# scheckmedia/centernet-uda

Hardware: AMD Instinct MI355X
Metric: images/sec CenterNet DLA-34 512x512 UDA step (entropy minimisation) (higher is better)
Workload: dtype f32; 1 GPU; configs[2]: DLA-34 + DCNv2, 512x512, per-GPU batch 16 source + 16 target, uda=entropy_minimization, Adam(lr 5e-5), random-init weights; global_batch=16, parallelism=dp1

## Files before the change

centernet-uda_amd/_ext.py:

```python
import torch

import hip_runtime as hr


def _shapes(input, weight, offset, mask, kh, kw, dg):
    if input.dim() != 4 or weight.dim() != 4:
        raise RuntimeError("dcn_v2: input and weight must be 4-D")
    B, C, H, W = input.shape
    Co, Ck, wkh, wkw = weight.shape
    if (wkh, wkw) != (kh, kw):
        raise RuntimeError("Input shape and kernel shape wont match: (%d x %d vs %d x %d)." % (kh, kw, wkh, wkw))
    if Ck != C:
        raise RuntimeError("Input shape and kernel channels wont match: (%d vs %d)." % (C, Ck))
    return B, C, H, W, Co


def _out_hw(H, W, kh, kw, sh, sw, ph, pw, dh, dw):
    return ((H + 2 * ph - (dh * (kh - 1) + 1)) // sh + 1, (W + 2 * pw - (dw * (kw - 1) + 1)) // sw + 1)


def _forward(who, input, weight, bias, offset, mask, om, geom, Ho, Wo, want_columns, act_slope, pack_token, pack_version,
             stats_box):
    B, C, H, W, Co, kh, kw = geom[:7]
    dg = geom[13]
    out = torch.empty((B, Co, Ho, Wo), dtype=torch.float32, device=input.device)
    cols = None
    if want_columns and W >= 2:
        cols = torch.empty((B, kh * kw * C, Ho * Wo), dtype=torch.float32, device=input.device)
    L = hr.lib()
    ws = hr.workspace(L.cnuda_dcn_v2_workspace_bytes(*geom), input.device)
    if dg == 1 and W >= 2:
        hr.prof_arm('dcn_fwd', B, C, H, W, Co, kh, kw, Ho, Wo)
    stats, blk, rows = None, 0, 0
    if stats_box is not None and act_slope < 0:
        rec = hr.stats_side_output(stats_box, L.cnuda_dcn_v2_stats_block, geom, Ho * Wo, input.device)
        if rec is not None:
            stats, blk, rows = rec[:3]
    tail = (*geom, hr.ptr(ws), ws.numel(), hr.stream())
    with hr.pack_stamp(pack_token, weight, pack_version):
        if om is not None:
            rc = L.cnuda_dcn_v2_forward_om(hr.ptr(input), hr.ptr(weight), hr.ptr(bias), hr.ptr(om), hr.ptr(out), hr.ptr(cols),
                                           hr.ptr(stats), blk, rows, float(act_slope), *tail)
        elif stats is not None:
            who += '_stats'
            rc = L.cnuda_dcn_v2_forward_stats(hr.ptr(input), hr.ptr(weight), hr.ptr(bias), hr.ptr(offset), hr.ptr(mask),
                                              hr.ptr(out), hr.ptr(cols), hr.ptr(stats), blk, rows, *tail)
        else:
            rc = L.cnuda_dcn_v2_forward_act(hr.ptr(input), hr.ptr(weight), hr.ptr(bias), hr.ptr(offset), hr.ptr(mask),
                                            hr.ptr(out), hr.ptr(cols), float(act_slope), *tail)
        hr.check(rc, who)
    return out, cols


def _backward(who, input, weight, bias, offset, mask, om, grad_output, geom, columns, grad_weight, grad_bias, grad_input):
    B, C, H, W, Co, kh, kw = geom[:7]
    g_in = grad_input if grad_input is not None else torch.empty_like(input)
    g_om = [torch.empty_like(om)] if om is not None else [torch.empty_like(offset), torch.empty_like(mask)]
    g_wb = [grad_weight if grad_weight is not None else torch.empty_like(weight),
            grad_bias if grad_bias is not None else torch.empty_like(bias)]
    L = hr.lib()
    ws = hr.workspace(L.cnuda_dcn_v2_workspace_bytes(*geom), input.device)
    if geom[13] == 1:
        hr.prof_arm('dcn_bwd', B, C, H, W, Co, kh, kw, grad_output.shape[2], grad_output.shape[3])
    fn = L.cnuda_dcn_v2_backward_acc if om is None else L.cnuda_dcn_v2_backward_om
    hr.check(fn(hr.ptr(input), hr.ptr(weight), hr.ptr(bias), *[hr.ptr(t) for t in ((offset, mask) if om is None else (om,))],
                hr.ptr(grad_output), hr.ptr(columns), hr.ptr(g_in), 1 if grad_input is not None else 0,
                *[hr.ptr(g) for g in g_om + g_wb], *geom, hr.ptr(ws), ws.numel(), hr.stream()), who)
    return [g_in] + g_om + g_wb


def dcn_v2_forward(input, weight, bias, offset, mask, kernel_h, kernel_w, stride_h, stride_w,
                   pad_h, pad_w, dilation_h, dilation_w, deformable_group, _want_columns=False, _act_slope=-1.0,
                   _pack_token=0, _pack_version=None, _stats_box=None):
    hr.require_gpu(input, weight, bias, offset, mask)
    input, weight, bias, offset, mask = [hr.f32c(t) for t in (input, weight, bias, offset, mask)]
    B, C, H, W, Co = _shapes(input, weight, offset, mask, kernel_h, kernel_w, deformable_group)
    Ho, Wo = _out_hw(H, W, kernel_h, kernel_w, stride_h, stride_w, pad_h, pad_w, dilation_h, dilation_w)
    T = kernel_h * kernel_w
    if tuple(offset.shape) != (B, 2 * T * deformable_group, Ho, Wo) or \
            tuple(mask.shape) != (B, T * deformable_group, Ho, Wo):
        raise RuntimeError("dcn_v2_forward: offset %s / mask %s do not match output %dx%d"
                           % (tuple(offset.shape), tuple(mask.shape), Ho, Wo))
    geom = (B, C, H, W, Co, kernel_h, kernel_w, stride_h, stride_w, pad_h, pad_w,
            dilation_h, dilation_w, deformable_group)
    out, cols = _forward('dcn_v2_forward', input, weight, bias, offset, mask, None, geom, Ho, Wo, _want_columns, _act_slope,
                         _pack_token, _pack_version, _stats_box)
    return (out, cols) if _want_columns else out


def dcn_v2_backward(input, weight, bias, offset, mask, grad_output, kernel_h, kernel_w, stride_h, stride_w,
                    pad_h, pad_w, dilation_h, dilation_w, deformable_group, _columns=None, _grad_weight=None,
                    _grad_bias=None, _grad_input=None):
    hr.require_gpu(input, weight, bias, offset, mask, grad_output)
    input, weight, bias, offset, mask, grad_output = [
        hr.f32c(t) for t in (input, weight, bias, offset, mask, grad_output)]
    B, C, H, W, Co = _shapes(input, weight, offset, mask, kernel_h, kernel_w, deformable_group)
    geom = (B, C, H, W, Co, kernel_h, kernel_w, stride_h, stride_w, pad_h, pad_w,
            dilation_h, dilation_w, deformable_group)
    return _backward('dcn_v2_backward', input, weight, bias, offset, mask, None, grad_output, geom, _columns, _grad_weight,
                     _grad_bias, _grad_input)


def dcn_v2_forward_om(input, weight, bias, om, kernel_h, kernel_w, stride_h, stride_w, pad_h, pad_w, dilation_h, dilation_w,
                      _want_columns=False, _pack_token=0, _stats_box=None, _act_slope=-1.0, _pack_version=None):
    hr.require_gpu(input, weight, bias, om)
    input, weight, bias, om = [hr.f32c(t) for t in (input, weight, bias, om)]
    B, C, H, W = input.shape
    Co = weight.shape[0]
    if weight.shape[1] != C or tuple(weight.shape[2:]) != (kernel_h, kernel_w):
        raise RuntimeError("dcn_v2_forward_om: weight %s does not match %d input channels / a %dx%d kernel"
                           % (tuple(weight.shape), C, kernel_h, kernel_w))
    Ho, Wo = _out_hw(H, W, kernel_h, kernel_w, stride_h, stride_w, pad_h, pad_w, dilation_h, dilation_w)
    T = kernel_h * kernel_w
    if tuple(om.shape) != (B, 3 * T, Ho, Wo):
        raise RuntimeError("dcn_v2_forward_om: om %s does not match [%d, %d, %d, %d]" % (tuple(om.shape), B, 3 * T, Ho, Wo))
    geom = (B, C, H, W, Co, kernel_h, kernel_w, stride_h, stride_w, pad_h, pad_w, dilation_h, dilation_w, 1)
    return _forward('dcn_v2_forward_om', input, weight, bias, None, None, om, geom, Ho, Wo, _want_columns, _act_slope,
                    _pack_token, _pack_version, _stats_box)


def dcn_v2_backward_om(input, weight, bias, om, grad_output, kernel_h, kernel_w, stride_h, stride_w, pad_h, pad_w,
                       dilation_h, dilation_w, _columns=None, _grad_weight=None, _grad_bias=None, _grad_input=None):
    hr.require_gpu(input, weight, bias, om, grad_output)
    input, weight, bias, om, grad_output = [hr.f32c(t) for t in (input, weight, bias, om, grad_output)]
    B, C, H, W = input.shape
    geom = (B, C, H, W, weight.shape[0], kernel_h, kernel_w, stride_h, stride_w, pad_h, pad_w, dilation_h, dilation_w, 1)
    return _backward('dcn_v2_backward_om', input, weight, bias, None, None, om, grad_output, geom, _columns, _grad_weight,
                     _grad_bias, _grad_input)


def _psroi_geom(input, rois, offset, no_trans, spatial_scale, output_dim, group_size, pooled_size, part_size,
                sample_per_part, trans_std):
    if input.dim() != 4:
        raise RuntimeError("dcn_v2_psroi_pooling: input must be 4-D")
    if rois.dim() != 2 or rois.shape[1] != 5:
        raise RuntimeError("dcn_v2_psroi_pooling: rois must be [N, 5] (batch index, x1, y1, x2, y2), got %s"
                           % (tuple(rois.shape),))
    B, C, H, W = input.shape
    N = rois.shape[0]
    if C != output_dim * group_size * group_size:
        raise RuntimeError("dcn_v2_psroi_pooling: input has %d channels, output_dim * group_size^2 = %d"
                           % (C, output_dim * group_size * group_size))
    if no_trans:
        num_classes = 1
    else:
        if offset.dim() != 4 or offset.shape[0] != N or offset.shape[1] % 2 or offset.shape[1] == 0 or \
                tuple(offset.shape[2:]) != (part_size, part_size):
            raise RuntimeError("dcn_v2_psroi_pooling: offset %s does not match [%d, 2 * num_classes, %d, %d]"
                               % (tuple(offset.shape), N, part_size, part_size))
        num_classes = offset.shape[1] // 2
        if output_dim % num_classes:
            raise RuntimeError("dcn_v2_psroi_pooling: output_dim %d is not a multiple of the offset's %d classes"
                               % (output_dim, num_classes))
    return (B, C, H, W, N, 1 if no_trans else 0, float(spatial_scale), int(output_dim), int(group_size),
            int(pooled_size), int(part_size), int(sample_per_part), float(trans_std), num_classes)


def dcn_v2_psroi_pooling_forward(input, rois, offset, no_trans, spatial_scale, output_dim, group_size, pooled_size,
                                 part_size, sample_per_part, trans_std):
    hr.require_gpu(input, rois, offset)
    input, rois = hr.f32c(input), hr.f32c(rois)
    geom = _psroi_geom(input, rois, offset, no_trans, spatial_scale, output_dim, group_size, pooled_size, part_size,
                       sample_per_part, trans_std)
    offset = None if no_trans else hr.f32c(offset)
    shape = (rois.shape[0], output_dim, pooled_size, pooled_size)
    out = torch.empty(shape, dtype=torch.float32, device=input.device)
    count = torch.empty(shape, dtype=torch.float32, device=input.device)
    hr.check(hr.lib().cnuda_dcn_v2_psroi_pooling_forward(hr.ptr(input), hr.ptr(rois), hr.ptr(offset), hr.ptr(out),
                                                         hr.ptr(count), *geom, hr.stream()),
             'dcn_v2_psroi_pooling_forward')
    return out, count


def dcn_v2_psroi_pooling_backward(grad_output, input, rois, offset, output_count, no_trans, spatial_scale, output_dim,
                                  group_size, pooled_size, part_size, sample_per_part, trans_std, _grad_input=None):
    hr.require_gpu(grad_output, input, rois, offset, output_count)
    grad_output, input, rois, output_count = [hr.f32c(t) for t in (grad_output, input, rois, output_count)]
    geom = _psroi_geom(input, rois, offset, no_trans, spatial_scale, output_dim, group_size, pooled_size, part_size,
                       sample_per_part, trans_std)
    shape = (rois.shape[0], output_dim, pooled_size, pooled_size)
    if tuple(grad_output.shape) != shape or tuple(output_count.shape) != shape:
        raise RuntimeError("dcn_v2_psroi_pooling_backward: grad_output %s / output_count %s do not match %s"
                           % (tuple(grad_output.shape), tuple(output_count.shape), shape))
    offset = None if no_trans else hr.f32c(offset)
    if _grad_input is not None and (_grad_input.shape != input.shape or _grad_input.dtype != torch.float32 or
                                    not _grad_input.is_contiguous() or not _grad_input.is_cuda):
        raise RuntimeError("dcn_v2_psroi_pooling_backward: _grad_input must be a contiguous fp32 GPU tensor like input")
    grad_input = _grad_input if _grad_input is not None else torch.empty_like(input)
    grad_offset = torch.empty(0, dtype=torch.float32, device=input.device) if no_trans else torch.empty_like(offset)
    L = hr.lib()
    ws = hr.workspace(L.cnuda_dcn_v2_psroi_pooling_workspace_bytes(geom[0], geom[4], geom[7], geom[9]), input.device)
    hr.check(L.cnuda_dcn_v2_psroi_pooling_backward(hr.ptr(grad_output), hr.ptr(input), hr.ptr(rois), hr.ptr(offset),
                                                   hr.ptr(output_count), hr.ptr(grad_input),
                                                   1 if _grad_input is not None else 0,
                                                   None if no_trans else hr.ptr(grad_offset), *geom, hr.ptr(ws),
                                                   ws.numel(), hr.stream()),
             'dcn_v2_psroi_pooling_backward')
    return grad_input, grad_offset
```

centernet-uda_amd/csrc/dcn.hip:

```cpp
#include <algorithm>
#include "igemm.cuh"
#include "igemm_host.h"

namespace cnuda {
namespace {

struct DcnGeom {
    int B, C, H, W, Co, kh, kw, sh, sw, ph, pw, dh, dw, dg, Ho, Wo;
    int off_bs, mask_bs, goff_bs, gmask_bs, gmask_logit;
};

struct Tap {
    int o00, o01, o10, o11;
    int h0, w0;
    float lh, lw, hh, hw;
    float mask;
    bool inside, c00, c01, c10, c11;
};

struct TapRaw { float dy, dx, mask; };
__device__ __forceinline__ TapRaw load_tap_raw(const DcnGeom& g, const float* __restrict__ off_b,
                                               const float* __restrict__ mask_b, int grp, int tap, int p) {
    const int T = g.kh * g.kw, HoWo = g.Ho * g.Wo;
    TapRaw r;
    r.dy = off_b[((size_t)grp * 2 * T + 2 * tap) * HoWo + p];
    r.dx = off_b[((size_t)grp * 2 * T + 2 * tap + 1) * HoWo + p];
    r.mask = mask_b[((size_t)grp * T + tap) * HoWo + p];
    return r;
}
__device__ __forceinline__ Tap tap_from_raw(const DcnGeom& g, const TapRaw& raw, int tap, int oy, int ox);
__device__ __forceinline__ Tap make_tap(const DcnGeom& g, const float* __restrict__ off_b,
                                        const float* __restrict__ mask_b, int grp, int tap, int oy, int ox) {
    return tap_from_raw(g, load_tap_raw(g, off_b, mask_b, grp, tap, oy * g.Wo + ox), tap, oy, ox);
}
__device__ __forceinline__ Tap tap_from_raw(const DcnGeom& g, const TapRaw& raw, int tap, int oy, int ox) {
    const int i = tap / g.kw, j = tap - i * g.kw;
    const float dy = raw.dy, dx = raw.dx;
    Tap t;
    t.mask = raw.mask;
    const float h = (float)(oy * g.sh - g.ph + i * g.dh) + dy;
    const float w = (float)(ox * g.sw - g.pw + j * g.dw) + dx;
    t.inside = (h > -1.0f) && (w > -1.0f) && (h < (float)g.H) && (w < (float)g.W);
    const float hf = floorf(h), wf = floorf(w);
    const int h0 = (int)hf, w0 = (int)wf;
    t.h0 = h0;
    t.w0 = w0;
    t.lh = h - hf;
    t.lw = w - wf;
    t.hh = 1.0f - t.lh;
    t.hw = 1.0f - t.lw;
    const bool top = h0 >= 0, bot = h0 + 1 <= g.H - 1, lef = w0 >= 0, rig = w0 + 1 <= g.W - 1;
    t.c00 = t.inside && top && lef;
    t.c01 = t.inside && top && rig;
    t.c10 = t.inside && bot && lef;
    t.c11 = t.inside && bot && rig;
    const int base = h0 * g.W + w0;
    t.o00 = t.c00 ? base : 0;
    t.o01 = t.c01 ? base + 1 : 0;
    t.o10 = t.c10 ? base + g.W : 0;
    t.o11 = t.c11 ? base + g.W + 1 : 0;
    return t;
}

__device__ __forceinline__ void tap_corners(const Tap& t, const float* __restrict__ plane, float& v00, float& v01,
                                            float& v10, float& v11) {
    v00 = t.c00 ? plane[t.o00] : 0.0f;
    v01 = t.c01 ? plane[t.o01] : 0.0f;
    v10 = t.c10 ? plane[t.o10] : 0.0f;
    v11 = t.c11 ? plane[t.o11] : 0.0f;
}
__device__ __forceinline__ float tap_sample(const Tap& t, float v00, float v01, float v10, float v11) {
    return t.hh * t.hw * v00 + t.hh * t.lw * v01 + t.lh * t.hw * v10 + t.lh * t.lw * v11;
}
struct __attribute__((packed, aligned(4))) Pair { float l, r; };

struct DcnFwdParams {
    DcnGeom g;
    const float *in, *off, *mask, *bias;
    float act_slope;
    float* out;
    float* col;
    float* stats;
    int stats_mp;
};

template <bool BUF>
struct DcnFwdLoaderT {
    using Params = DcnFwdParams;
    static const char* name() { return "DcnFwdLoader"; }
    static constexpr bool kHasSideOutput = true;
    const DcnGeom& g;
    const float *in_b, *off_b, *mask_b;
    buf_rsrc rin;
    float* col_base = nullptr;
    unsigned in_boff = 0, col_voff = IG_BUF_OOB;
    bool col_on = false;
    int oy, ox, K;
    bool valid;
    int cur;
    int ck0 = 0, ctap = 0, cc0 = 0;
    int qT, qB;
    float m00, m01, m10, m11;
    float* col_n;
    int col_stride;
    __device__ __forceinline__ void disable_col() { col_n = nullptr; col_on = false; }
    __device__ DcnFwdLoaderT(const Params& p, long long n, bool n_valid) : g(p.g), valid(n_valid), cur(-1) {
        const int HoWo = g.Ho * g.Wo;
        const int nn = n_valid ? (int)n : 0;
        const int b = nn / HoWo, pp = nn - b * HoWo;
        oy = pp / g.Wo;
        ox = pp - oy * g.Wo;
        const int T = g.kh * g.kw;
        in_b = p.in + (size_t)b * g.C * g.H * g.W;
        off_b = p.off + (size_t)b * g.off_bs;
        mask_b = p.mask + (size_t)b * g.mask_bs;
        K = T * g.C;
        col_n = (p.col && n_valid) ? p.col + (size_t)b * K * HoWo + pp : nullptr;
        col_stride = HoWo;
        if constexpr (BUF) {
            rin = ig_make_rsrc(p.in, (unsigned)((size_t)g.B * g.C * g.H * g.W * sizeof(float)));
            col_base = p.col;
            in_boff = (unsigned)(b * g.C * g.H * g.W) * (unsigned)sizeof(float);
            col_on = p.col != nullptr;
            col_voff = (p.col && n_valid) ? (unsigned)(b * K * HoWo + pp) * (unsigned)sizeof(float) : IG_BUF_OOB;
        }
    }
    __device__ __forceinline__ void set_tap(int tap) {
        const Tap t = make_tap(g, off_b, mask_b, 0, tap, oy, ox);
        const float mk = (valid && t.inside) ? t.mask : 0.0f;
        const float w00 = t.c00 ? t.hh * t.hw * mk : 0.0f, w01 = t.c01 ? t.hh * t.lw * mk : 0.0f;
        const float w10 = t.c10 ? t.lh * t.hw * mk : 0.0f, w11 = t.c11 ? t.lh * t.lw * mk : 0.0f;
        const bool inside = valid && t.inside;
        const int w0 = inside ? t.w0 : 0, h0 = inside ? t.h0 : 0;
        const int wa = w0 < 0 ? 0 : (w0 > g.W - 2 ? g.W - 2 : w0);
        const bool ledge = w0 < 0, redge = w0 > g.W - 2;
        m00 = ledge ? w01 : (redge ? 0.0f : w00);
        m01 = ledge ? 0.0f : (redge ? w00 : w01);
        m10 = ledge ? w11 : (redge ? 0.0f : w10);
        m11 = ledge ? 0.0f : (redge ? w10 : w11);
        const int ht = h0 < 0 ? 0 : h0, hb = h0 + 1 > g.H - 1 ? g.H - 1 : h0 + 1;
        qT = ht * g.W + wa;
        qB = hb * g.W + wa;
        cur = tap;
    }
    __device__ __forceinline__ float sample(const float* __restrict__ pl) const {
        const Pair a = *reinterpret_cast<const Pair*>(pl + qT), b = *reinterpret_cast<const Pair*>(pl + qB);
        return m00 * a.l + m01 * a.r + m10 * b.l + m11 * b.r;
    }
    struct Raw {
        Pair t[8], b[8];
        int k0;
        bool live, eager;
    };
    __device__ __forceinline__ void load_raw(int k0, int ksub, Raw& r) {
        const int HW = g.H * g.W;
        r.k0 = k0 + ksub;
        r.live = k0 < K;
        r.eager = g.C % IG_BK != 0;
        if (!r.eager) {
            if (!r.live) return;
            while (ck0 < k0) {
                ck0 += IG_BK;
                cc0 += IG_BK;
                if (cc0 >= g.C) { cc0 -= g.C; ++ctap; }
            }
            const int tap = ctap, c0 = cc0 + ksub;
            if (tap != cur) set_tap(tap);
            if constexpr (BUF) {
                const unsigned vT = in_boff + (unsigned)qT * 4u, vB = in_boff + (unsigned)qB * 4u;
                const int c0s = cc0 + __builtin_amdgcn_readfirstlane(ksub);
#pragma unroll
                for (int j = 0; j < 8; ++j) {
                    const unsigned soff = (unsigned)((c0s + 2 * j) * HW) * 4u;
                    r.t[j] = __builtin_bit_cast(Pair, __builtin_amdgcn_raw_buffer_load_b64(rin, (int)vT, (int)soff, 0));
                    r.b[j] = __builtin_bit_cast(Pair, __builtin_amdgcn_raw_buffer_load_b64(rin, (int)vB, (int)soff, 0));
                }
                return;
            }
            const float* plane = in_b + (size_t)c0 * HW;
#pragma unroll
            for (int j = 0; j < 8; ++j) {
                const float* pl = plane + (size_t)(2 * j) * HW;
                r.t[j] = *reinterpret_cast<const Pair*>(pl + qT);
                r.b[j] = *reinterpret_cast<const Pair*>(pl + qB);
            }
            return;
        }
#pragma unroll
        for (int j = 0; j < 8; ++j) {
            const int k = k0 + ksub + 2 * j;
            float v = 0.0f;
            if (k < K) {
                const int tap = k / g.C, c = k - tap * g.C;
                if (tap != cur) set_tap(tap);
                v = sample(in_b + (size_t)c * HW);
            }
            r.t[j].l = v;
        }
    }
    __device__ __forceinline__ void finish(const Raw& r, float (&v)[8]) {
        if (!r.eager) {
            if (!r.live) {
#pragma unroll
                for (int j = 0; j < 8; ++j) v[j] = 0.0f;
                return;
            }
#pragma unroll
            for (int j = 0; j < 8; ++j) v[j] = m00 * r.t[j].l + m01 * r.t[j].r + m10 * r.b[j].l + m11 * r.b[j].r;
            if constexpr (BUF) {
                if (col_on && col_voff != IG_BUF_OOB) {
                    const int k0s = __builtin_amdgcn_readfirstlane(r.k0);
                    const char* cbase = reinterpret_cast<const char*>(col_base);
                    unsigned voff = col_voff;
                    asm volatile("" : "+v"(voff));
#pragma unroll
                    for (int j = 0; j < 8; ++j) {
                        const size_t row = (size_t)(unsigned)((k0s + 2 * j) * col_stride) * 4u;
                        unsigned long long rbase = reinterpret_cast<unsigned long long>(cbase) + row;
                        asm volatile("" : "+s"(rbase));
                        *reinterpret_cast<__attribute__((address_space(1))) float*>(rbase + (unsigned long long)voff) = v[j];
                    }
                }
                return;
            }
            if (col_n) {
                float* cp = col_n + (size_t)r.k0 * col_stride;
                const size_t step = (size_t)2 * col_stride;
#pragma unroll
                for (int j = 0; j < 8; ++j) cp[j * step] = v[j];
            }
            return;
        }
#pragma unroll
        for (int j = 0; j < 8; ++j) {
            const int k = r.k0 + 2 * j;
            v[j] = r.t[j].l;
            if (col_n && k < K) col_n[(size_t)k * col_stride] = v[j];
        }
    }
    struct Out {
        float* base;
        int HoWo;
        __device__ Out(const Params& p, long long n) {
            HoWo = p.g.Ho * p.g.Wo;
            const int ni = (int)n, b = ni / HoWo, pp = ni - b * HoWo;
            base = p.out + (size_t)b * p.g.Co * HoWo + pp;
        }
        __device__ __forceinline__ void store(const Params& p, int m, float v) {
            v += p.bias[m];
            if (p.act_slope >= 0.0f && v < 0.0f) v *= p.act_slope;
            base[(size_t)m * HoWo] = v;
        }
        static constexpr bool kVec4 = true;
        __device__ static bool vec4_ok(const Params& p) { return ((p.g.Ho * p.g.Wo) & 3) == 0; }
        __device__ __forceinline__ void store4(const Params& p, int m, f32x4 v) {
            v += p.bias[m];
            if (p.act_slope >= 0.0f) {
#pragma unroll
                for (int e = 0; e < 4; ++e) if (v[e] < 0.0f) v[e] *= p.act_slope;
            }
            *reinterpret_cast<f32x4*>(base + (size_t)m * HoWo) = v;
        }
    };
};

using DcnFwdLoader = DcnFwdLoaderT<false>;
using DcnFwdBufLoader = DcnFwdLoaderT<true>;

constexpr int DW_MARGIN = 3;
typedef __attribute__((address_space(3))) volatile unsigned char lds_vu8;
template <int TC> struct DwTile {
    static constexpr int TR = IG_BN / TC, NR = TR + 2 + 2 * DW_MARGIN, RS = TC + 8, PL = NR * RS;
    static constexpr int CPR = TC / 4 + 2, CPP = NR * CPR, CELLS = 16 * CPP;
    static constexpr int NCELL = (CELLS + IG_THREADS - 1) / IG_THREADS;
    static constexpr int SHIFT = TC == 32 ? 5 : 4;
};
template <int TC> constexpr size_t dcnw_lds_floats(int bm) { return (size_t)16 * DwTile<TC>::PL + 2 * IG_KC * bm; }

template <int BM, int TC>
__global__ __launch_bounds__(IG_THREADS, 3) void dcnw_fwd_kernel(DcnFwdParams p, const float* __restrict__ A, int Mp, int Kp,
                                                                 int n_tiles, int tiles_x) {
    using Q = DwTile<TC>;
    constexpr int TM = BM / 32, PL = Q::PL, RS = Q::RS;
    extern __shared__ __attribute__((aligned(16))) float smem[];
    const DcnGeom& g = p.g;
    const int W = g.W, H = g.H, HW = g.H * g.W;
    float* const Hs = smem;
    float* const Asb = smem + 16 * PL;
    const int tid = threadIdx.x, lane = tid & 63, wid = tid >> 6;
    int tile = xcd_remap(blockIdx.x, n_tiles);
    const int tile_id = tile;
    const int tx = tile % tiles_x; tile /= tiles_x;
    const int tiles_y = H / Q::TR;
    const int ty = tile % tiles_y, b = tile / tiles_y;
    const int y0 = ty * Q::TR, x0 = tx * TC;
    const int yw0 = y0 - 1 - DW_MARGIN;
    const int pxl = wid * 32 + (lane & 31), kl = lane >> 5;
    const int py = y0 + (pxl >> Q::SHIFT), px = x0 + (pxl & (TC - 1)), pp = py * W + px;

    const buf_rsrc rs = ig_make_rsrc(p.in, (unsigned)((size_t)g.B * g.C * HW * sizeof(float)));
    auto cell = [&](int i, unsigned& voff, int& loff) {
        int salt = 0;
        asm volatile("" : "+v"(salt));
        const int e = tid + i * IG_THREADS + salt;
        const int c = e / Q::CPP, rem = e - c * Q::CPP;
        const int row = rem / Q::CPR, q4 = rem - row * Q::CPR;
        const int iy = yw0 + row, ix = x0 - 4 + 4 * q4;
        loff = e < Q::CELLS ? c * PL + row * RS + 4 * q4 : -1;
        voff = (e < Q::CELLS && iy >= 0 && iy < H && ix >= 0 && ix < W)
                   ? (unsigned)(((b * g.C + c) * HW + iy * W + ix) * (int)sizeof(float)) : IG_BUF_OOB;
    };

    int addr[9];
    float flh[9], flw[9], fmk[9];
    unsigned stray = 0;
    {
        const float* off_b = p.off + (size_t)b * g.off_bs + pp;
        const float* mask_b = p.mask + (size_t)b * g.mask_bs + pp;
        float dy[9], dx[9], mk[9];
#pragma unroll
        for (int t = 0; t < 9; ++t) {
            dy[t] = off_b[(size_t)(2 * t) * HW];
            dx[t] = off_b[(size_t)(2 * t + 1) * HW];
            mk[t] = mask_b[(size_t)t * HW];
        }
#pragma unroll
        for (int t = 0; t < 9; ++t) {
            const float h = (float)(py - 1 + t / 3) + dy[t], w = (float)(px - 1 + t % 3) + dx[t];
            const float hf = floorf(h), wf = floorf(w);
            const bool valid = h > -1.0f && w > -1.0f && h < (float)H && w < (float)W;
            const int h0 = valid ? (int)hf : 0, w0i = valid ? (int)wf : 0;
            const int wr = h0 - yw0, wc = w0i - x0 + 4;
            const bool inwin = valid && wr >= 0 && wr + 1 <= Q::NR - 1 && wc >= 0 && wc + 1 <= RS - 1;
            addr[t] = inwin ? wr * RS + wc : 0;
            flh[t] = h - hf;
            flw[t] = w - wf;
            fmk[t] = inwin ? mk[t] : 0.0f;
            if (valid && !inwin) stray |= 1u << t;
        }
    }
    const bool any_stray = __any(stray != 0);

    f32x16 acc[TM];
#pragma unroll
    for (int i = 0; i < TM; ++i)
#pragma unroll
        for (int r = 0; r < 16; ++r) acc[i][r] = 0.0f;

    f32x4 hreg[Q::NCELL];
    auto win_load = [&](int grp) {
        const unsigned soff = (unsigned)(grp * 16 * HW) * (unsigned)sizeof(float);
#pragma unroll
        for (int i = 0; i < Q::NCELL; ++i) {
            unsigned voff; int loff;
            cell(i, voff, loff);
            hreg[i] = ig_buf_load4(rs, voff, soff);
        }
    };
    auto win_store = [&]() {
#pragma unroll
        for (int i = 0; i < Q::NCELL; ++i) {
            unsigned voff; int loff;
            cell(i, voff, loff);
            if (loff >= 0) *reinterpret_cast<f32x4*>(Hs + loff) = hreg[i];
        }
    };
    f32x4 ra[ig_a_per<BM>()];
    const IgABuf<BM> abuf(A, Mp, Kp, 0, tid);
    const int nchunk = Kp / IG_KC, G = g.C >> 4;
    const bool col_on = p.col != nullptr;
    float* const col_l = col_on ? p.col + (size_t)b * 9 * g.C * HW + (size_t)kl * HW + pp : nullptr;

    win_load(0);
    abuf.load(0, ra);
    win_store();
    ig_store_a<BM>(Asb, tid, ra);
    if (1 < nchunk) abuf.load(IG_KC, ra);
    __syncthreads();
    int grp = 0;
    for (int c0 = 0; c0 < nchunk; c0 += 9, ++grp) {
        const bool more = grp + 1 < G;
        if (more) win_load(grp + 1);
#pragma unroll
        for (int t = 0; t < 9; ++t) {
            const int c = c0 + t;
            f32x4 ra2[ig_a_per<BM>()];
            if (c + 2 < nchunk) abuf.load((c + 2) * IG_KC, ra2);
            const float* As = Asb + (c & 1) * IG_KC * BM;
            const float* ap = As + kl * BM + (lane & 31);
            int a_t = addr[t];
            asm volatile("" : "+v"(a_t));
            const float* hb = Hs + kl * PL + a_t;
            const float lh = flh[t], lw = flw[t], hh = 1.0f - lh, hw = 1.0f - lw, mk = fmk[t];
            const float w00 = hh * hw * mk, w01 = hh * lw * mk, w10 = lh * hw * mk, w11 = lh * lw * mk;
            float v[IG_KC / 2], cr[IG_KC / 4][4];
            float* cp = nullptr;
            if (col_on) {
                unsigned long long rowoff = (unsigned long long)(unsigned)((t * g.C + grp * 16) * HW) * sizeof(float);
                asm volatile("" : "+s"(rowoff));
                cp = reinterpret_cast<float*>(reinterpret_cast<char*>(col_l) + rowoff);
            }
            auto read_half = [&](int h) {
#pragma unroll
                for (int s = 0; s < IG_KC / 4; ++s) {
                    const float* q = hb + 2 * (h * (IG_KC / 4) + s) * PL;
                    cr[s][0] = q[0]; cr[s][1] = q[1]; cr[s][2] = q[RS]; cr[s][3] = q[RS + 1];
                }
            };
            auto blend_half = [&](int h) {
#pragma unroll
                for (int s = 0; s < IG_KC / 4; ++s) {
                    float x = w00 * cr[s][0];
                    x = fmaf(w01, cr[s][1], x);
                    x = fmaf(w10, cr[s][2], x);
                    v[h * (IG_KC / 4) + s] = fmaf(w11, cr[s][3], x);
                }
                if (col_on) {
#pragma unroll
                    for (int s = 0; s < IG_KC / 4; ++s) cp[(size_t)(2 * (h * (IG_KC / 4) + s)) * HW] = v[h * (IG_KC / 4) + s];
                }
            };
            auto mma_half = [&](int h) {
#pragma unroll
                for (int s = h * (IG_KC / 4); s < (h + 1) * (IG_KC / 4); ++s) {
#pragma unroll
                    for (int i = 0; i < TM; ++i)
                        acc[i] = __builtin_amdgcn_mfma_f32_32x32x2f32(ap[2 * s * BM + i * 32], v[s], acc[i], 0, 0, 0);
                }
            };
            read_half(0);
            blend_half(0);
            read_half(1);
            __builtin_amdgcn_sched_barrier(0);
            mma_half(0);
            __builtin_amdgcn_sched_barrier(0);
            blend_half(1);
            mma_half(1);
            if (c + 1 < nchunk) ig_store_a<BM>(Asb + ((c + 1) & 1) * IG_KC * BM, tid, ra);
#pragma unroll
            for (int i = 0; i < ig_a_per<BM>(); ++i) ra[i] = ra2[i];
            __syncthreads();
            __builtin_amdgcn_sched_barrier(0);
        }
        if (any_stray) {
#pragma unroll 1
            for (int t0 = 0; t0 < 9; ++t0) {
                int t = t0;
                asm volatile("" : "+s"(t));
                if (!__any((stray >> t) & 1u)) continue;
                float sv[IG_KC / 2];
#pragma unroll
                for (int s = 0; s < IG_KC / 2; ++s) sv[s] = 0.0f;
                if ((stray >> t) & 1u) {
                    const float* off_b = p.off + (size_t)b * g.off_bs + pp;
                    const int tr = t / 3;
                    const float sh_ = (float)(py - 1 + tr) + off_b[(size_t)(2 * t) * HW];
                    const float sw_ = (float)(px - 1 + t - 3 * tr) + off_b[(size_t)(2 * t + 1) * HW];
                    const float smk = p.mask[(size_t)b * g.mask_bs + (size_t)t * HW + pp];
                    const float shf = floorf(sh_), swf = floorf(sw_);
                    const int sh0 = (int)shf, sw0 = (int)swf;
                    const float slh = sh_ - shf, slw = sw_ - swf, shh = 1.0f - slh, shw = 1.0f - slw;
                    const bool top = sh0 >= 0, bot = sh0 + 1 <= H - 1, lef = sw0 >= 0, rig = sw0 + 1 <= W - 1;
                    const float g00 = (top && lef) ? shh * shw * smk : 0.0f, g01 = (top && rig) ? shh * slw * smk : 0.0f;
                    const float g10 = (bot && lef) ? slh * shw * smk : 0.0f, g11 = (bot && rig) ? slh * slw * smk : 0.0f;
                    const int cy0 = top ? sh0 : 0, cy1 = bot ? sh0 + 1 : H - 1, cx0 = lef ? sw0 : 0, cx1 = rig ? sw0 + 1 : W - 1;
                    const float* in_c = p.in + ((size_t)b * g.C + grp * 16 + kl) * HW;
                    const int o00 = cy0 * W + cx0, o01 = cy0 * W + cx1, o10 = cy1 * W + cx0, o11 = cy1 * W + cx1;
#pragma unroll
                    for (int s = 0; s < IG_KC / 2; ++s) {
                        const float* pl = in_c + (size_t)(2 * s) * HW;
                        float x = g00 * pl[o00];
                        x = fmaf(g01, pl[o01], x);
                        x = fmaf(g10, pl[o10], x);
                        sv[s] = fmaf(g11, pl[o11], x);
                    }
                    if (col_on) {
                        float* cp = col_l + (size_t)(t * g.C + grp * 16) * HW;
#pragma unroll
                        for (int s = 0; s < IG_KC / 2; ++s) cp[(size_t)(2 * s) * HW] = sv[s];
                    }
                }
                const float* ag = A + (size_t)((c0 + t) * IG_KC + kl) * Mp + (lane & 31);
#pragma unroll
                for (int s = 0; s < IG_KC / 2; ++s) {
#pragma unroll
                    for (int i = 0; i < TM; ++i)
                        acc[i] = __builtin_amdgcn_mfma_f32_32x32x2f32(ag[(size_t)(2 * s) * Mp + i * 32], sv[s], acc[i], 0, 0, 0);
                }
            }
        }
        if (more) {
            win_store();
            __syncthreads();
        }
    }
    float* stage = smem + wid * IG_EPI_WAVE;
    const int col = lane & 31, cg = lane & 7, rsub = lane >> 3;
    const int epl = wid * 32 + 4 * cg;
    float* const obase = p.out + (size_t)b * g.Co * HW + (size_t)(y0 + (epl >> Q::SHIFT)) * W + x0 + (epl & (TC - 1));
#pragma unroll
    for (int i = 0; i < TM; ++i) {
#pragma unroll
        for (int r = 0; r < 16; ++r) stage[mfma_row(r, lane) * IG_EPI_LD + col] = acc[i][r];
        asm volatile("s_waitcnt lgkmcnt(0)" ::: "memory");
#pragma unroll
        for (int it = 0; it < 4; ++it) {
            const int row = it * 8 + rsub;
            f32x4 v4 = *reinterpret_cast<const f32x4*>(stage + row * IG_EPI_LD + 4 * cg);
            const int m = i * 32 + row;
            if (m < g.Co) {
                v4 += p.bias[m];
                if (p.act_slope >= 0.0f) {
#pragma unroll
                    for (int e = 0; e < 4; ++e) if (v4[e] < 0.0f) v4[e] *= p.act_slope;
                }
                *reinterpret_cast<f32x4*>(obase + (size_t)m * HW) = v4;
            }
            if (p.stats) {
                float s1 = (v4[0] + v4[1]) + (v4[2] + v4[3]);
                float s2 = (v4[0] * v4[0] + v4[1] * v4[1]) + (v4[2] * v4[2] + v4[3] * v4[3]);
                auto row8 = [](float v) {
                    v += __builtin_bit_cast(float, __builtin_amdgcn_update_dpp(0, __builtin_bit_cast(int, v), 0xB1, 0xf, 0xf, false));
                    v += __builtin_bit_cast(float, __builtin_amdgcn_update_dpp(0, __builtin_bit_cast(int, v), 0x4E, 0xf, 0xf, false));
                    v += __builtin_bit_cast(float, __builtin_amdgcn_update_dpp(0, __builtin_bit_cast(int, v), 0x141, 0xf, 0xf, false));
                    return v;
                };
                s1 = row8(s1);
                s2 = row8(s2);
                if (cg == 0)
                    reinterpret_cast<float2*>(p.stats)[((size_t)tile_id * 4 + wid) * p.stats_mp + m] = make_float2(s1, s2);
            }
        }
        asm volatile("s_waitcnt lgkmcnt(0)" ::: "memory");
    }
}

struct DcnSampleParams {
    DcnGeom g;
    const float *in, *off, *mask;
    float* col;
};
__global__ __launch_bounds__(1024) void dcn_sample_kernel(DcnSampleParams p, int tiles_per_image) {
    const DcnGeom& g = p.g;
    const int T = g.kh * g.kw, HoWo = g.Ho * g.Wo, HW = g.H * g.W;
    const int b = blockIdx.x / tiles_per_image, tile = blockIdx.x - b * tiles_per_image;
    const int px = tile * 64 + threadIdx.x;
    if (px >= HoWo) return;
    const int oy = px / g.Wo, ox = px - oy * g.Wo;
    const float* in_b = p.in + (size_t)b * g.C * HW;
    for (int tap = threadIdx.y; tap < T; tap += blockDim.y) {
        const Tap t = make_tap(g, p.off + (size_t)b * g.off_bs, p.mask + (size_t)b * g.mask_bs, 0, tap, oy, ox);
        const float mk = t.inside ? t.mask : 0.0f;
        const float w00 = t.c00 ? t.hh * t.hw * mk : 0.0f, w01 = t.c01 ? t.hh * t.lw * mk : 0.0f;
        const float w10 = t.c10 ? t.lh * t.hw * mk : 0.0f, w11 = t.c11 ? t.lh * t.lw * mk : 0.0f;
        float* dst = p.col + ((size_t)b * T + tap) * g.C * HoWo + px;
        const bool paired = g.W >= 2;
        const bool ledge = t.w0 < 0, redge = t.w0 > g.W - 2;
        const int wa = ledge ? 0 : (redge ? g.W - 2 : t.w0);
        const int ht = t.h0 < 0 ? 0 : t.h0, hb = t.h0 + 1 > g.H - 1 ? g.H - 1 : t.h0 + 1;
        const int qT = t.inside ? ht * g.W + wa : 0, qB = t.inside ? hb * g.W + wa : 0;
        for (int c0 = 0; c0 < g.C; c0 += 8) {
            float e00[8], e01[8], e10[8], e11[8];
            if (paired) {
                Pair pt[8], pb[8];
#pragma unroll
                for (int u = 0; u < 8; ++u) {
                    const float* plane = in_b + (size_t)(c0 + u < g.C ? c0 + u : g.C - 1) * HW;
                    pt[u] = *reinterpret_cast<const Pair*>(plane + qT);
                    pb[u] = *reinterpret_cast<const Pair*>(plane + qB);
                }
#pragma unroll
                for (int u = 0; u < 8; ++u) {
                    e00[u] = redge ? pt[u].r : pt[u].l; e01[u] = ledge ? pt[u].l : pt[u].r;
                    e10[u] = redge ? pb[u].r : pb[u].l; e11[u] = ledge ? pb[u].l : pb[u].r;
                }
            } else {
#pragma unroll
                for (int u = 0; u < 8; ++u) {
                    const float* plane = in_b + (size_t)(c0 + u < g.C ? c0 + u : g.C - 1) * HW;
                    e00[u] = plane[t.o00]; e01[u] = plane[t.o01]; e10[u] = plane[t.o10]; e11[u] = plane[t.o11];
                }
            }
#pragma unroll
            for (int u = 0; u < 8; ++u)
                if (c0 + u < g.C)
                    dst[(size_t)(c0 + u) * HoWo] = w00 * e00[u] + w01 * e01[u] + w10 * e10[u] + w11 * e11[u];
        }
    }
}

struct DcnColsParams {
    DcnGeom g;
    const float *col, *bias;
    float act_slope;
    float* out;
    float* stats;
    int stats_mp;
};
struct DcnColsLoader {
    using Params = DcnColsParams;
    static const char* name() { return "DcnColsLoader"; }
    static constexpr bool kHasSideOutput = false;
    const float* base;
    int K, HoWo;
    bool valid;
    __device__ DcnColsLoader(const Params& p, long long n, bool n_valid) : valid(n_valid) {
        HoWo = p.g.Ho * p.g.Wo;
        K = p.g.kh * p.g.kw * p.g.C;
        const int nn = n_valid ? (int)n : 0;
        const int b = nn / HoWo, pp = nn - b * HoWo;
        base = p.col + (size_t)b * K * HoWo + pp;
    }
    __device__ __forceinline__ void load(int k0, int ksub, float (&v)[8]) {
#pragma unroll
        for (int j = 0; j < 8; ++j) {
            const int k = k0 + ksub + 2 * j;
            v[j] = (valid && k < K) ? base[(size_t)k * HoWo] : 0.0f;
        }
    }
    struct Out {
        float* base;
        int HoWo;
        __device__ Out(const Params& p, long long n) {
            HoWo = p.g.Ho * p.g.Wo;
            const int ni = (int)n, b = ni / HoWo, pp = ni - b * HoWo;
            base = p.out + (size_t)b * p.g.Co * HoWo + pp;
        }
        __device__ __forceinline__ void store(const Params& p, int m, float v) {
            v += p.bias[m];
            if (p.act_slope >= 0.0f && v < 0.0f) v *= p.act_slope;
            base[(size_t)m * HoWo] = v;
        }
// ... 349 lines not shown
}

struct DcnPrepParams {
    DcnGeom g;
    const float *w, *off, *mask;
    float* wt;
    DcnGeo* geo;
    int wt_blocks;
    float* zero;
    long long zero_quads;
    int zero_first;
};
__global__ __launch_bounds__(256) void dcn_prep_kernel(DcnPrepParams p) {
    const DcnGeom& g = p.g;
    if (p.zero && (int)blockIdx.x >= p.zero_first) {
        const long long nb = (long long)gridDim.x - p.zero_first;
        float4* z = reinterpret_cast<float4*>(p.zero);
        for (long long i = ((long long)blockIdx.x - p.zero_first) * 256 + threadIdx.x; i < p.zero_quads; i += nb * 256)
            z[i] = make_float4(0.f, 0.f, 0.f, 0.f);
        return;
    }
    const int T = g.kh * g.kw;
    if ((int)blockIdx.x < p.wt_blocks) {
        const long long total = (long long)g.Co * g.C * T;
        for (long long i = (long long)blockIdx.x * 256 + threadIdx.x; i < total; i += (long long)p.wt_blocks * 256) {
            const int o = (int)(i % g.Co);
            const long long r = i / g.Co;
            const int c = (int)(r % g.C), tap = (int)(r / g.C);
            p.wt[i] = p.w[((size_t)o * g.C + c) * T + tap];
        }
        return;
    }
    if (!p.geo) return;
    const int HoWo = g.Ho * g.Wo;
    const long long total = (long long)g.B * T * HoWo;
    const long long nb = (long long)(p.zero ? p.zero_first : (int)gridDim.x) - p.wt_blocks;
    for (long long i = ((long long)blockIdx.x - p.wt_blocks) * 256 + threadIdx.x; i < total; i += nb * 256) {
        const int px = (int)(i % HoWo);
        const long long r = i / HoWo;
        const int tap = (int)(r % T), b = (int)(r / T);
        const int oy = px / g.Wo, ox = px - oy * g.Wo;
        p.geo[i] = dcn_geo_pack(make_tap(g, p.off + (size_t)b * g.off_bs, p.mask + (size_t)b * g.mask_bs, 0, tap, oy, ox));
    }
}

struct DcnBwdDataParams {
    DcnGeom g;
    const float *in, *dcol;
    const DcnGeo* geo;
    float *gin, *goff, *gmask;
    DcnWalkTile tile;
    int nsplit;
};
template <bool QUADS>
__global__ __launch_bounds__(512, 6) void dcn_bwd_data_kernel(DcnBwdDataParams p, int n_wg) {
    extern __shared__ __align__(16) float win[];
    const DcnGeom& g = p.g;
    const int T = g.kh * g.kw, HoWo = g.Ho * g.Wo, HW = g.H * g.W;
    const int tid = threadIdx.x & 255, lane = tid & 63, wid = __builtin_amdgcn_readfirstlane(tid >> 6);
    int id = xcd_remap(blockIdx.x, n_wg);
    const int part = id % p.nsplit; id /= p.nsplit;
    const DcnWalkTile& tile = p.tile;
    const int tx = id % tile.tiles_x; id /= tile.tiles_x;
    const int ty = id % tile.tiles_y;
    const int b = id / tile.tiles_y;
    const int y0 = ty * tile.TR, x0 = tx * tile.TC;
    const DcnGeo* geo_b = p.geo + (size_t)b * T * HoWo;
    const float* dcol_b = p.dcol + (size_t)b * T * g.C * HoWo;
    auto pixel_of = [&](int grp, bool& valid) {
        const int i = grp * 64 + lane;
        const int oy = y0 + (i >> tile.tc_shift), ox = x0 + (i & (tile.TC - 1));
        valid = oy < g.Ho && ox < g.Wo;
        return valid ? oy * g.Wo + ox : 0;
    };
#ifdef DCN_ABLATE
    if ((DCN_ABLATE == 1) == (threadIdx.x >= 256)) return;
#endif
    if (threadIdx.x >= 256) {
        bool valid;
        const int px = pixel_of(wid, valid);
        if (!valid) return;
        const float* in_b = p.in + (size_t)b * g.C * HW;
#pragma unroll 1
        for (int tap = part; tap < T; tap += p.nsplit) {
            const DcnGeoTap t = dcn_geo_unpack(geo_b[(size_t)tap * HoWo + px]);
            const float* dc = dcol_b + (size_t)tap * g.C * HoWo + (QUADS ? (size_t)px * 4 : (size_t)px);
            DcnCoordSums s{0.f, 0.f, 0.f};
            if (t.inside) s = dcn_coord_tap<QUADS>(g, t, in_b, dc, HoWo);
            dcn_coord_store(g, p.gmask, p.goff, b, tap, px, HoWo, t.mask, s);
        }
        return;
    }
    const DcnScatterCtx x = dcn_scatter_ctx(win, tile, g, y0, x0, wid, tid);
    float* gin_b = p.gin + (size_t)b * g.C * HW;
    const int cg_end = (part + 1) * tile.ncg / p.nsplit;
#pragma unroll 1
    for (int cg = part * tile.ncg / p.nsplit; cg < cg_end; ++cg)
        dcn_scatter_group<QUADS>(x, g, geo_b, dcol_b, gin_b, cg * CI_CG + wid * 4, lane);
}

struct DcnWParams {
    DcnGeom g;
    const float *in, *off, *mask, *gout;
};
struct DcnWLoader {
    using Params = DcnWParams;
    const Params& p;
    IgPixelCursor c;
    __device__ DcnWLoader(const Params& pp, long long n, long long n_end) : p(pp) {
        c.init(n, n_end, p.g.Ho * p.g.Wo, p.g.Wo);
    }
    __device__ __forceinline__ void advance() { c.advance(p.g.Ho * p.g.Wo, p.g.Wo); }
    template <int NV, int STEP>
    __device__ __forceinline__ void load_g(int m0, int msub, float (&v)[NV]) {
        const DcnGeom& g = p.g;
        const int HoWo = g.Ho * g.Wo;
        const float* base = p.gout + (size_t)c.b_ * g.Co * HoWo + c.pp_;
#pragma unroll
        for (int i = 0; i < NV; ++i) {
            const int m = m0 + msub + STEP * i;
            v[i] = (c.valid_ && m < g.Co) ? base[(size_t)m * HoWo] : 0.0f;
        }
    }
    template <int NV, int STEP>
    __device__ __forceinline__ void load_b(int j0, int jsub, float (&v)[NV]) {
        const DcnGeom& g = p.g;
        const int HW = g.H * g.W, T = g.kh * g.kw, K = T * g.C;
        const float* in_b = p.in + (size_t)c.b_ * g.C * HW;
        const float* off_b = p.off + (size_t)c.b_ * g.off_bs;
        const float* mask_b = p.mask + (size_t)c.b_ * g.mask_bs;
        int cur = -1;
        Tap t;
#pragma unroll
        for (int i = 0; i < NV; ++i) {
            const int k = j0 + jsub + STEP * i;
            float r = 0.0f;
            if (c.valid_ && k < K) {
                const int tap = k / g.C, ch = k - tap * g.C;
                if (tap != cur) { t = make_tap(g, off_b, mask_b, 0, tap, c.oy_, c.ox_); cur = tap; }
                if (t.inside) {
                    float v00, v01, v10, v11;
                    tap_corners(t, in_b + (size_t)ch * HW, v00, v01, v10, v11);
                    r = tap_sample(t, v00, v01, v10, v11) * t.mask;
                }
            }
            v[i] = r;
        }
    }
};

struct DcnColWParams {
    DcnGeom g;
    const float *col, *gout;
};
struct DcnColWLoader {
    using Params = DcnColWParams;
    const Params& p;
    IgPixelCursor c;
    __device__ DcnColWLoader(const Params& pp, long long n, long long n_end) : p(pp) {
        c.init(n, n_end, p.g.Ho * p.g.Wo, p.g.Wo);
    }
    __device__ __forceinline__ void advance() { c.advance(p.g.Ho * p.g.Wo, p.g.Wo); }
    template <int NV, int STEP>
    __device__ __forceinline__ void load_g(int m0, int msub, float (&v)[NV]) {
        const DcnGeom& g = p.g;
        const int HoWo = g.Ho * g.Wo;
        const float* base = p.gout + (size_t)c.b_ * g.Co * HoWo + c.pp_;
#pragma unroll
        for (int i = 0; i < NV; ++i) {
            const int m = m0 + msub + STEP * i;
            v[i] = (c.valid_ && m < g.Co) ? base[(size_t)m * HoWo] : 0.0f;
        }
    }
    template <int NV, int STEP>
    __device__ __forceinline__ void load_b(int j0, int jsub, float (&v)[NV]) {
        const DcnGeom& g = p.g;
        const int HoWo = g.Ho * g.Wo, K = g.kh * g.kw * g.C;
        const float* base = p.col + (size_t)c.b_ * K * HoWo + c.pp_;
#pragma unroll
        for (int i = 0; i < NV; ++i) {
            const int k = j0 + jsub + STEP * i;
            v[i] = (c.valid_ && k < K) ? base[(size_t)k * HoWo] : 0.0f;
        }
    }
};

struct DcnColWBufLoader {
    using Params = DcnColWParams;
    const Params& p;
    buf_rsrc rg, rc;
    IgPixelCursor c;
    unsigned gimg, cimg;
    __device__ DcnColWBufLoader(const Params& pp, long long n, long long n_end) : p(pp) {
        const DcnGeom& g = p.g;
        const size_t px = (size_t)g.B * g.Ho * g.Wo;
        rg = ig_make_rsrc(p.gout, (unsigned)(px * g.Co * sizeof(float)));
        rc = ig_make_rsrc(p.col, (unsigned)(px * g.kh * g.kw * g.C * sizeof(float)));
        c.init(n, n_end, g.Ho * g.Wo, g.Wo);
        gimg = (unsigned)(c.b_ * g.Co * g.Ho * g.Wo) * 4u;
        cimg = (unsigned)(c.b_ * g.kh * g.kw * g.C * g.Ho * g.Wo) * 4u;
    }
    __device__ __forceinline__ void advance() {
        const DcnGeom& g = p.g;
        c.advance(g.Ho * g.Wo, g.Wo);
        if (c.crossed_) {
            gimg += (unsigned)(c.crossed_ * g.Co * g.Ho * g.Wo) * 4u;
            cimg += (unsigned)(c.crossed_ * g.kh * g.kw * g.C * g.Ho * g.Wo) * 4u;
        }
    }
    template <int NV, int STEP>
    __device__ __forceinline__ void load_g(int m0, int msub, float (&v)[NV]) {
        ig_buf_rows<NV, STEP>(rg, c, gimg, p.g.Ho * p.g.Wo, m0, msub, v);
    }
    template <int NV, int STEP>
    __device__ __forceinline__ void load_b(int j0, int jsub, float (&v)[NV]) {
        ig_buf_rows<NV, STEP>(rc, c, cimg, p.g.Ho * p.g.Wo, j0, jsub, v);
    }
};

struct DcnNaiveParams {
    DcnGeom g;
    const float *in, *weight, *bias, *off, *mask, *gout;
    float *out, *gin, *goff, *gmask, *gw;
};

__global__ void dcn_naive_fwd_kernel(DcnNaiveParams p) {
    const DcnGeom& g = p.g;
    const int T = g.kh * g.kw, HoWo = g.Ho * g.Wo, HW = g.H * g.W, cpg = g.C / g.dg;
    const long long total = (long long)g.B * g.Co * HoWo;
    for (long long i = (long long)blockIdx.x * blockDim.x + threadIdx.x; i < total;
         i += (long long)gridDim.x * blockDim.x) {
        const int pp = (int)(i % HoWo), o = (int)((i / HoWo) % g.Co), b = (int)(i / ((long long)HoWo * g.Co));
        const int oy = pp / g.Wo, ox = pp - oy * g.Wo;
        float s = p.bias[o];
        for (int grp = 0; grp < g.dg; ++grp)
            for (int tap = 0; tap < T; ++tap) {
                const Tap t = make_tap(g, p.off + (size_t)b * g.off_bs,
                                       p.mask + (size_t)b * g.mask_bs, grp, tap, oy, ox);
                if (!t.inside) continue;
                for (int cc = 0; cc < cpg; ++cc) {
                    const int c = grp * cpg + cc;
                    float v00, v01, v10, v11;
                    tap_corners(t, p.in + ((size_t)b * g.C + c) * HW, v00, v01, v10, v11);
                    s += p.weight[((size_t)o * g.C + c) * T + tap] * (tap_sample(t, v00, v01, v10, v11) * t.mask);
                }
            }
        p.out[i] = s;
    }
}

__global__ void dcn_naive_bwd_kernel(DcnNaiveParams p) {
    const DcnGeom& g = p.g;
    const int T = g.kh * g.kw, HoWo = g.Ho * g.Wo, HW = g.H * g.W, cpg = g.C / g.dg;
    const long long total = (long long)g.B * g.C * T * HoWo;
    for (long long i = (long long)blockIdx.x * blockDim.x + threadIdx.x; i < total;
         i += (long long)gridDim.x * blockDim.x) {
        const int pp = (int)(i % HoWo), tap = (int)((i / HoWo) % T), c = (int)((i / ((long long)HoWo * T)) % g.C);
        const int b = (int)(i / ((long long)HoWo * T * g.C));
        const int oy = pp / g.Wo, ox = pp - oy * g.Wo, grp = c / cpg;
        const Tap t = make_tap(g, p.off + (size_t)b * g.off_bs, p.mask + (size_t)b * g.mask_bs, grp,
                               tap, oy, ox);
        if (!t.inside) continue;
        float v00, v01, v10, v11;
        tap_corners(t, p.in + ((size_t)b * g.C + c) * HW, v00, v01, v10, v11);
        const float smp = tap_sample(t, v00, v01, v10, v11);
        const float* go = p.gout + (size_t)b * g.Co * HoWo + pp;
        float d = 0.0f;
        for (int o = 0; o < g.Co; ++o) {
            const float gv = go[(size_t)o * HoWo];
            d += p.weight[((size_t)o * g.C + c) * T + tap] * gv;
            atomicAdd(p.gw + ((size_t)o * g.C + c) * T + tap, gv * (smp * t.mask));
        }
        const float dm = d * t.mask;
        atomicAdd(p.gmask + ((size_t)(b * g.dg + grp) * T + tap) * HoWo + pp, d * smp);
        atomicAdd(p.goff + ((size_t)(b * g.dg + grp) * 2 * T + 2 * tap) * HoWo + pp,
                  (-t.hw * v00 - t.lw * v01 + t.hw * v10 + t.lw * v11) * dm);
        atomicAdd(p.goff + ((size_t)(b * g.dg + grp) * 2 * T + 2 * tap + 1) * HoWo + pp,
                  (-t.hh * v00 + t.hh * v01 - t.lh * v10 + t.lh * v11) * dm);
        float* gplane = p.gin + ((size_t)b * g.C + c) * HW;
        if (t.c00) atomicAdd(gplane + t.o00, t.hh * t.hw * dm);
        if (t.c01) atomicAdd(gplane + t.o01, t.hh * t.lw * dm);
        if (t.c10) atomicAdd(gplane + t.o10, t.lh * t.hw * dm);
        if (t.c11) atomicAdd(gplane + t.o11, t.lh * t.lw * dm);
    }
}

int fill_geom(DcnGeom& g, int B, int C, int H, int W, int Co, int kh, int kw, int sh, int sw, int ph, int pw, int dh,
              int dw, int dg, const char* who) {
    CNUDA_REQUIRE(B > 0 && C > 0 && H > 0 && W > 0 && Co > 0, "%s: empty tensor", who);
    CNUDA_REQUIRE(kh > 0 && kw > 0 && sh > 0 && sw > 0 && dh > 0 && dw > 0 && ph >= 0 && pw >= 0,
                  "%s: bad kernel geometry", who);
    CNUDA_REQUIRE(dg > 0 && C % dg == 0, "%s: channels (%d) not divisible by deformable_group (%d)", who, C, dg);
    g = DcnGeom{B, C, H, W, Co, kh, kw, sh, sw, ph, pw, dh, dw, dg,
                (H + 2 * ph - (dh * (kh - 1) + 1)) / sh + 1, (W + 2 * pw - (dw * (kw - 1) + 1)) / sw + 1, 0, 0, 0, 0, 0};
    CNUDA_REQUIRE(g.Ho > 0 && g.Wo > 0, "%s: kernel larger than padded input", who);
    CNUDA_REQUIRE((long long)dg * 3 * kh * kw * g.Ho * g.Wo < (1ll << 31), "%s: offset planes of an image exceed 2^31 elements", who);
    g.off_bs = g.goff_bs = dg * 2 * kh * kw * g.Ho * g.Wo;
    g.mask_bs = g.gmask_bs = dg * kh * kw * g.Ho * g.Wo;
    return 0;
}

constexpr int kDcnMinTiles = 512;
int dcn_pick_bm(int M, long long N) {
    int bm = M > 64 ? 128 : (M > 32 ? 64 : 32);
    const long long n_tiles = (N + IG_BN - 1) / IG_BN;
    while (bm > 32 && n_tiles * ((M + bm - 1) / bm) < kDcnMinTiles) bm >>= 1;
    return bm;
}

constexpr int kFusedMinTilesDefault = 512;
int g_fused_min_tiles = kFusedMinTilesDefault;
int g_scatter_margin = 0;
int g_walk_tc = 0;
int g_offset_regime = 0;


int dcnw_tile_cols(int W) { return W % 32 == 0 ? 32 : 16; }
bool dcnw_takes(const DcnGeom& g) {
    static const bool dcnw_on = !(getenv("CNUDA_DCNW") && getenv("CNUDA_DCNW")[0] == '0');
    return dcnw_on && (g_offset_regime & 2) == 0 && matrix_mode() == 0 && g.kh == 3 && g.kw == 3 && g.sh == 1 && g.sw == 1 && g.ph == 1 && g.pw == 1 &&
           g.dh == 1 && g.dw == 1 && g.dg == 1 && g.C % 16 == 0 && g.Co <= 64 &&
           g.W % 16 == 0 && g.H % (IG_BN / dcnw_tile_cols(g.W)) == 0 &&
           (size_t)g.B * g.C * g.H * g.W * sizeof(float) < IG_BUF_OOB;
}

#ifndef DCN_COLS_WS
#define DCN_COLS_WS 1
#endif
#ifndef DCN_COLW_WS
#define DCN_COLW_WS 1
#endif
enum class DcnFwdPath { Naive, Composed, Window, SampleThenGemm, Gather };
struct DcnPlan {
    DcnFwdPath fwd;
    bool fwd_buf;
    bool fwd_ws;
    bool colw_buf, colw_ws;
    bool dcol_quads;
    int T, K, Kp, bm, Mp;
    WgradShape wg;
    long long N;
    size_t fwd_bytes, bwd_bytes;
    bool fwd_two_kernels;
    size_t gemm_bytes;
    DcnWalkTile tile;
    size_t col2im_lds;
    bool fused_consumers;
    int fused_split;
};
DcnPlan make_plan(const DcnGeom& g) {
    DcnPlan q;
    q.T = g.kh * g.kw;
    q.K = q.T * g.C;
    q.Kp = round_up(q.K, IG_KC);
    q.N = (long long)g.B * g.Ho * g.Wo;
    q.bm = dcn_pick_bm(g.Co, q.N);
    q.Mp = round_up(g.Co, q.bm);
    q.wg = make_wgrad_shape(g.Co, q.K, q.N, WG_BM, round_up(q.K, WG_BJ) % 128 == 0 ? 128 : WG_BJ, WG_BP);
    q.fwd_two_kernels = q.Mp / q.bm > 1;
    q.fwd_bytes = carve_bytes((size_t)q.Kp * q.Mp, 4) + 256 +
                  (q.fwd_two_kernels ? carve_bytes((size_t)g.B * q.K * g.Ho * g.Wo, 4) : 0);
    if (g.Co <= 64) {
        const size_t wb = carve_bytes((size_t)q.Kp * 64, 4) + 256;
        if (wb > q.fwd_bytes) q.fwd_bytes = wb;
    }
    q.gemm_bytes = cnuda_conv2d_workspace_bytes(g.B, g.Co, g.Ho, g.Wo, q.T * g.C, 1, 1, 1, 1, 0, 0);
    q.bwd_bytes = carve_bytes((size_t)q.wg.Z * q.wg.Mpw * q.wg.Jp, 4) +
                  carve_bytes(std::max((size_t)g.Co * g.B, (size_t)q.wg.Z * q.wg.Mpw), 4) +
                  carve_bytes((size_t)12 * g.C * (g.Co < 64 ? 64 : g.Co), 4) +
                  carve_bytes((size_t)g.B * q.T * g.C * g.Ho * g.Wo, 4) +
                  carve_bytes((size_t)g.B * q.T * g.Ho * g.Wo, sizeof(DcnGeo)) + carve_bytes(q.gemm_bytes, 1) + 256;
    DcnWalkTile& w = q.tile;
    w.TC = 64;
    while (w.TC > 16 && w.TC / 2 >= g.Wo) w.TC >>= 1;
    if (w.TC == 64 && round_up(g.Wo, 32) < round_up(g.Wo, 64)) w.TC = 32;
    if (g_walk_tc == 16 || g_walk_tc == 32 || g_walk_tc == 64) w.TC = g_walk_tc;
    w.TR = 256 / w.TC;
    w.tc_shift = w.TC == 64 ? 6 : (w.TC == 32 ? 5 : 4);
    w.tiles_y = ceil_div(g.Ho, w.TR);
    w.tiles_x = ceil_div(g.Wo, w.TC);
    w.ncg = ceil_div(g.C, CI_CG);
    w.margin = g_scatter_margin > 0 ? g_scatter_margin : ((g_offset_regime & 1) ? 4 : CI_MARGIN);
    const int wr = (w.TR - 1) * g.sh + (g.kh - 1) * g.dh + 2 * w.margin + 1;
    const int wc = (w.TC - 1) * g.sw + (g.kw - 1) * g.dw + 2 * w.margin + 1;
    w.WSZmax = wr * wc;
    w.claim_sz = ((wr + 1) * (wc + 1) + 15) / 16 * 16;
    if ((size_t)CI_CG * w.WSZmax * 4 + 4096 + 4 * (size_t)w.claim_sz > (w.margin > CI_MARGIN ? 80 : 53) * 1024) { w.WSZmax = 0; w.claim_sz = 16; }
    q.col2im_lds = ((size_t)CI_CG * w.WSZmax + 4 * 256) * sizeof(float) + 4 * (size_t)w.claim_sz;
    q.fused_consumers = w.WSZmax > 0 && g.W >= 2 && (long long)g.B * w.tiles_y * w.tiles_x >= g_fused_min_tiles;
    q.fused_split = 4;
    if (q.fused_split > w.ncg) q.fused_split = w.ncg;

    const size_t HoWo = (size_t)g.Ho * g.Wo;
    q.fwd = (g.dg > 1 && g.W >= 2) ? DcnFwdPath::Composed
          : (g.dg != 1 || g.W < 2) ? DcnFwdPath::Naive
          : dcnw_takes(g) ? DcnFwdPath::Window
          : q.fwd_two_kernels ? DcnFwdPath::SampleThenGemm : DcnFwdPath::Gather;
    q.fwd_buf = buffer_addressing() && g.C % IG_BK == 0 && (size_t)g.B * g.C * g.H * g.W * sizeof(float) < IG_BUF_OOB &&
                (size_t)g.B * q.K * HoWo * sizeof(float) < IG_BUF_OOB;
    q.fwd_ws = DCN_COLS_WS && q.fwd_buf && q.bm >= 64 && wave_specialised() && matrix_mode() == 0;
    q.colw_buf = buffer_addressing() && (size_t)g.B * q.K * HoWo * sizeof(float) < IG_BUF_OOB &&
                 (size_t)g.B * g.Co * HoWo * sizeof(float) < IG_BUF_OOB && HoWo < (1 << 23);
    q.colw_ws = DCN_COLW_WS && q.colw_buf && wave_specialised() && matrix_mode() == 0;
    static const bool quads_on = !(getenv("CNUDA_DCOL_QUADS") && getenv("CNUDA_DCOL_QUADS")[0] == '0');
    q.dcol_quads = quads_on && g.C % 4 == 0 && HoWo < (1 << 26) &&
                   cnuda_conv2d_rowquads_supported(g.B, g.Co, g.Ho, g.Wo, q.T * g.C, 1, 1, 1, 1, 0, 0);
    return q;
}

int plan_stats_block(const DcnGeom& g, const DcnPlan& q, int* rows) {
    if (q.fwd == DcnFwdPath::Naive || q.fwd == DcnFwdPath::Composed || ((g.Ho * g.Wo) & 3) != 0) return 0;
    if (q.fwd == DcnFwdPath::Window) { if (rows) *rows = 64; return 32; }
    if (rows) *rows = q.Mp;
    return q.bm == 32 ? 32 : 64;
}

struct DcnCall {
    DcnGeom g;
    const float *input, *weight, *bias, *offset, *mask;
    void* workspace;
    size_t workspace_bytes;
    cnuda_stream_t stream;
};
struct DcnFwdCall : DcnCall {
    float *output, *columns, *stats;
    float act_slope;
};
struct DcnBwdCall : DcnCall {
    const float *grad_output, *columns;
    float *grad_input, *grad_offset, *grad_mask, *grad_weight, *grad_bias;
    int accumulate_input;
};

template <class F>
auto with_quads(bool quads, F&& f) {
    return quads ? f(std::true_type{}) : f(std::false_type{});
}

template <class Loader, bool WS = false, class P>
bool launch_dcn_fwd(const DcnPlan& q, const P& p, const float* A, int Cout, hipStream_t st) {
    const int n_tiles = ceil_div(q.N, IG_BN), m_tiles = q.Mp / q.bm;
    const dim3 grid(n_tiles * m_tiles);
    if constexpr (WS)
        return with_tile<64, 128>(q.bm, [&](auto BM) {
            CNUDA_LAUNCH((igemm_fwd_ws_kernel<BM(), Loader>), grid, dim3(2 * IG_THREADS), 0, st, p, A, q.Mp, q.Kp, Cout, q.N, n_tiles, m_tiles);
        });
    else
        return with_tile<32, 64, 128>(q.bm, [&](auto BM) {
            CNUDA_LAUNCH((igemm_fwd_kernel<BM(), Loader>), grid, dim3(IG_THREADS), 0, st, p, A, q.Mp, q.Kp, Cout, q.N, n_tiles, m_tiles);
        });
}

}
}

using namespace cnuda;

extern "C" int cnuda_dcn_set_scatter_margin(int margin) {
    const int prev = g_scatter_margin;
    g_scatter_margin = margin < 1 ? 0 : (margin > 8 ? 8 : margin);
    return prev;
}
extern "C" int cnuda_dcn_set_walk_tile(int tile_cols) {
    const int prev = g_walk_tc;
    g_walk_tc = tile_cols;
    return prev;
}
extern "C" int cnuda_dcn_set_offset_regime(int regime) {
    const int prev = g_offset_regime;
    g_offset_regime = regime & 3;
    return prev;
}

namespace cnuda {
namespace {
__global__ __launch_bounds__(256) void dcn_offset_census_kernel(const float* __restrict__ offset, long long n_pairs, long long HW,
                                                                unsigned* __restrict__ counts) {
    unsigned c2 = 0, c3 = 0;
    for (long long i = (long long)blockIdx.x * 256 + threadIdx.x; i < n_pairs; i += (long long)gridDim.x * 256) {
        const long long plane = i / HW, px = i - plane * HW;
        const float dy = fabsf(offset[(2 * plane) * HW + px]), dx = fabsf(offset[(2 * plane + 1) * HW + px]);
        const float d = dy > dx ? dy : dx;
        c2 += d >= 2.0f;
        c3 += d >= 3.0f;
    }
    __shared__ unsigned s2, s3;
    if (threadIdx.x == 0) { s2 = 0; s3 = 0; }
    __syncthreads();
    if (c2) atomicAdd(&s2, c2);
    if (c3) atomicAdd(&s3, c3);
    __syncthreads();
    if (threadIdx.x == 0) {
        if (s2) atomicAdd(counts, s2);
        if (s3) atomicAdd(counts + 1, s3);
    }
}
}
}
extern "C" int cnuda_dcn_offset_census(const float* offset, int B, int taps, long long HW, unsigned* counts,
                                       cnuda_stream_t stream) {
    CNUDA_REQUIRE(offset && counts && B > 0 && taps > 0 && HW > 0, "cnuda_dcn_offset_census: bad arguments");
    const long long n = (long long)B * taps * HW;
    CNUDA_LAUNCH(cnuda::dcn_offset_census_kernel, dim3(stream_grid(n, 256)), dim3(256), 0, (hipStream_t)stream, offset, n, HW,
                 counts);
    return check_launch("cnuda_dcn_offset_census");
}
extern "C" int cnuda_dcn_set_fused_min_tiles(int min_tiles) {
    const int prev = g_fused_min_tiles;
    g_fused_min_tiles = min_tiles < 1 ? kFusedMinTilesDefault : min_tiles;
    return prev;
}

extern "C" size_t cnuda_dcn_v2_workspace_bytes(int B, int C, int H, int W, int Cout, int kh, int kw, int sh, int sw,
                                               int ph, int pw, int dh, int dw, int dg) {
    DcnGeom g;
    if (fill_geom(g, B, C, H, W, Cout, kh, kw, sh, sw, ph, pw, dh, dw, dg, "cnuda_dcn_v2_workspace_bytes")) return 0;
    const DcnPlan q = make_plan(g);
    if (q.fwd == DcnFwdPath::Composed) {
        const int Cg = C / dg, T = kh * kw;
        const size_t inner = cnuda_dcn_v2_workspace_bytes(B, Cg, H, W, Cout, kh, kw, sh, sw, ph, pw, dh, dw, 1);
        return 2 * carve_bytes((size_t)B * Cg * H * W, 4) + 2 * carve_bytes((size_t)Cout * Cg * T, 4) +
               carve_bytes((size_t)B * Cout * g.Ho * g.Wo, 4) + 2 * carve_bytes((size_t)Cout, 4) + carve_bytes(inner, 1) + 512;
    }
    return q.fwd_bytes > q.bwd_bytes ? q.fwd_bytes : q.bwd_bytes;
}

extern "C" int cnuda_dcn_v2_forward(const float* input, const float* weight, const float* bias, const float* offset,
                                    const float* mask, float* output, int B, int C, int H, int W, int Cout, int kh,
                                    int kw, int sh, int sw, int ph, int pw, int dh, int dw, int dg, void* workspace,
                                    size_t workspace_bytes, cnuda_stream_t stream) {
    return cnuda_dcn_v2_forward_cols(input, weight, bias, offset, mask, output, nullptr, B, C, H, W, Cout, kh, kw, sh,
                                     sw, ph, pw, dh, dw, dg, workspace, workspace_bytes, stream);
}

extern "C" int cnuda_dcn_v2_forward_cols(const float* input, const float* weight, const float* bias,
                                         const float* offset, const float* mask, float* output, float* columns, int B,
                                         int C, int H, int W, int Cout, int kh, int kw, int sh, int sw, int ph, int pw,
                                         int dh, int dw, int dg, void* workspace, size_t workspace_bytes,
                                         cnuda_stream_t stream) {
    return cnuda_dcn_v2_forward_act(input, weight, bias, offset, mask, output, columns, -1.0f, B, C, H, W, Cout, kh, kw,
                                    sh, sw, ph, pw, dh, dw, dg, workspace, workspace_bytes, stream);
}

extern "C" int cnuda_dcn_v2_stats_block(int B, int C, int H, int W, int Cout, int kh, int kw, int sh, int sw, int ph, int pw,
                                        int dh, int dw, int dg, int* rows) {
    DcnGeom g;
    if (fill_geom(g, B, C, H, W, Cout, kh, kw, sh, sw, ph, pw, dh, dw, dg, "cnuda_dcn_v2_stats_block")) return 0;
    return plan_stats_block(g, make_plan(g), rows);
}

static int dcn_forward_impl(const DcnFwdCall& c, const DcnPlan& q) {
    const DcnGeom& g = c.g;
    CNUDA_REQUIRE(c.input && c.weight && c.bias && c.offset && c.mask && c.output, "cnuda_dcn_v2_forward: null pointer");
    CNUDA_REQUIRE(!c.columns || g.W >= 2, "cnuda_dcn_v2_forward_cols: columns output needs width >= 2");
    hipStream_t st = (hipStream_t)c.stream;
    CNUDA_REQUIRE(c.act_slope < 0.0f || (g.dg == 1 && g.W >= 2), "cnuda_dcn_v2_forward_act: fused activation needs deformable_group == 1 and width >= 2");
    if (q.fwd == DcnFwdPath::Composed) {
        const int Cg = g.C / g.dg, T = q.T, HoWo = g.Ho * g.Wo;
        const long long HW = (long long)g.H * g.W;
        const size_t inner = cnuda_dcn_v2_workspace_bytes(g.B, Cg, g.H, g.W, g.Co, g.kh, g.kw, g.sh, g.sw, g.ph, g.pw, g.dh, g.dw, 1);
        Carver cv(c.workspace, c.workspace_bytes);
        float* xg = cv.take<float>((size_t)g.B * Cg * HW);
        float* wg = cv.take<float>((size_t)g.Co * Cg * T);
        float* tmp = cv.take<float>((size_t)g.B * g.Co * HoWo);
        float* zero = cv.take<float>((size_t)g.Co);
        void* iws = cv.take<char>(inner);
        CNUDA_REQUIRE(c.workspace && cv.cur <= cv.end, "cnuda_dcn_v2_forward: workspace too small");
        if (hipMemsetAsync(zero, 0, (size_t)g.Co * sizeof(float), st) != hipSuccess) return check_launch("cnuda_dcn_v2_forward(dg>1)");
        DcnFwdCall gc = c;
        gc.g.C = Cg; gc.g.dg = 1;
        gc.input = xg; gc.weight = wg;
        gc.workspace = iws; gc.workspace_bytes = inner;
        const DcnPlan gq = make_plan(gc.g);
        const PackStampSuspend uncached;
        for (int grp = 0; grp < g.dg; ++grp) {
            if (int rc = cnuda_copy_channels(c.input, xg, g.B, Cg, HW, g.C, grp * Cg, Cg, 0, c.stream)) return rc;
            if (int rc = cnuda_copy_channels(c.weight, wg, g.Co, Cg, T, g.C, grp * Cg, Cg, 0, c.stream)) return rc;
            gc.bias = grp == 0 ? c.bias : zero;
            gc.offset = c.offset + (size_t)grp * 2 * T * HoWo;
            gc.mask = c.mask + (size_t)grp * T * HoWo;
            gc.output = grp == 0 ? c.output : tmp;
            gc.columns = c.columns ? c.columns + (size_t)grp * g.B * T * Cg * HoWo : nullptr;
            if (int rc = dcn_forward_impl(gc, gq)) return rc;
            if (grp > 0)
                if (int rc = cnuda_add(c.output, tmp, c.output, (long long)g.B * g.Co * HoWo, c.stream)) return rc;
        }
        return check_launch("cnuda_dcn_v2_forward(dg>1)");
    }
    if (q.fwd == DcnFwdPath::Naive) {
        DcnNaiveParams p{g, c.input, c.weight, c.bias, c.offset, c.mask, nullptr, c.output, nullptr, nullptr, nullptr, nullptr};
        CNUDA_LAUNCH(dcn_naive_fwd_kernel, dim3(stream_grid((long long)g.B * g.Co * g.Ho * g.Wo, 256)), dim3(256),
                           0, st, p);
        return check_launch("cnuda_dcn_v2_forward(dg>1)");
    }
    CNUDA_REQUIRE(q.N < (1ll << 31) - IG_BN, "cnuda_dcn_v2_forward: more than 2^31 pixels per call");
    CNUDA_REQUIRE(c.workspace && c.workspace_bytes >= q.fwd_bytes, "cnuda_dcn_v2_forward: workspace too small");
    Carver cv(c.workspace, c.workspace_bytes);
    if (q.fwd == DcnFwdPath::Window) {
        const int bm = 64;
        const float* Aw = launch_pack(c.weight, cv.take<float>((size_t)q.Kp * bm), (size_t)q.Kp * bm * sizeof(float), g.Co, g.C,
                                      q.T, PACK_HALO_FWD, q.Kp, bm, 0, st);
        DcnFwdParams p{g, c.input, c.offset, c.mask, c.bias, c.act_slope, c.output, c.columns, c.stats, 64};
        ProfScope prof(st);
        prof.name("dcnw_fwd_kernel<%d>%s", bm, c.columns ? " (+ column side output)" : "");
        const int tiles_x = g.W / dcnw_tile_cols(g.W), n_tiles = (int)(q.N / IG_BN);
        bool lds_ok = true;
        const bool found = with_tiles<Tile<64, 32>, Tile<64, 16>>(bm, dcnw_tile_cols(g.W), [&](auto BM, auto TC) {
            const size_t fl = dcnw_lds_floats<TC()>(BM());
            const size_t lds = (fl < (size_t)4 * IG_EPI_WAVE ? (size_t)4 * IG_EPI_WAVE : fl) * sizeof(float);
            lds_ok = raise_dynamic_lds(reinterpret_cast<const void*>(&dcnw_fwd_kernel<BM(), TC()>), lds);
            if (lds_ok) CNUDA_LAUNCH((dcnw_fwd_kernel<BM(), TC()>), dim3(n_tiles), dim3(IG_THREADS), lds, st, p, Aw, bm, q.Kp, n_tiles, tiles_x);
        });
        CNUDA_REQUIRE(lds_ok, "cnuda_dcn_v2_forward: dynamic LDS");
        CNUDA_REQUIRE(found, "cnuda_dcn_v2_forward: no dcnw_fwd_kernel instance for %d-column tiles", dcnw_tile_cols(g.W));
        return check_launch("cnuda_dcn_v2_forward(window)");
    }
    const float* A = launch_pack(c.weight, cv.take<float>((size_t)q.Kp * q.Mp), (size_t)q.Kp * q.Mp * sizeof(float), g.Co,
                                 g.C, q.T, PACK_FWD, q.Kp, q.Mp, 0, st);
    if (q.fwd == DcnFwdPath::SampleThenGemm) {
        float* cols = c.columns ? c.columns : cv.take<float>((size_t)g.B * q.K * g.Ho * g.Wo);
        ProfScope prof(st);
        prof.name("dcn_sample_kernel + igemm_fwd_kernel<%d, DcnColsLoader>", q.bm);
        {
            DcnSampleParams sp{g, c.input, c.offset, c.mask, cols};
            const int tiles = ceil_div(g.Ho * g.Wo, 64), tw = q.T < 16 ? q.T : 16;
            CNUDA_LAUNCH(dcn_sample_kernel, dim3(g.B * tiles), dim3(64, tw), 0, st, sp, tiles);
        }
        DcnColsParams p{g, cols, c.bias, c.act_slope, c.output, c.stats, q.Mp};
        const bool found = q.fwd_ws    ? launch_dcn_fwd<DcnColsBufLoader, true>(q, p, A, g.Co, st)
                           : q.fwd_buf ? launch_dcn_fwd<DcnColsBufLoader>(q, p, A, g.Co, st)
                                       : launch_dcn_fwd<DcnColsLoader>(q, p, A, g.Co, st);
        CNUDA_REQUIRE(found, "cnuda_dcn_v2_forward: no GEMM instance for a %d-row tile", q.bm);
        return check_launch("cnuda_dcn_v2_forward(columns + GEMM)");
    }
    DcnFwdParams p{g, c.input, c.offset, c.mask, c.bias, c.act_slope, c.output, c.columns, c.stats, q.Mp};
    ProfScope prof(st);
    prof.name("igemm_fwd_kernel<%d, DcnFwdLoader>%s", q.bm, c.columns ? " (+ column side output)" : "");
    const bool found = q.fwd_buf ? launch_dcn_fwd<DcnFwdBufLoader>(q, p, A, g.Co, st) : launch_dcn_fwd<DcnFwdLoader>(q, p, A, g.Co, st);
    CNUDA_REQUIRE(found, "cnuda_dcn_v2_forward: no GEMM instance for a %d-row tile", q.bm);
    return check_launch("cnuda_dcn_v2_forward");
}

extern "C" int cnuda_dcn_v2_forward_act(const float* input, const float* weight, const float* bias,
                                        const float* offset, const float* mask, float* output, float* columns,
                                        float act_slope, int B, int C, int H, int W, int Cout, int kh, int kw, int sh,
                                        int sw, int ph, int pw, int dh, int dw, int dg, void* workspace,
                                        size_t workspace_bytes, cnuda_stream_t stream) {
    DcnFwdCall c{};
    if (int rc = fill_geom(c.g, B, C, H, W, Cout, kh, kw, sh, sw, ph, pw, dh, dw, dg, "cnuda_dcn_v2_forward")) return rc;
    c.input = input; c.weight = weight; c.bias = bias; c.offset = offset; c.mask = mask;
    c.output = output; c.columns = columns; c.act_slope = act_slope;
    c.workspace = workspace; c.workspace_bytes = workspace_bytes; c.stream = stream;
    return dcn_forward_impl(c, make_plan(c.g));
}

extern "C" int cnuda_dcn_v2_forward_stats(const float* input, const float* weight, const float* bias,
                                          const float* offset, const float* mask, float* output, float* columns,
                                          float* stats, int stats_block, int stats_rows, int B, int C, int H, int W,
                                          int Cout, int kh, int kw, int sh,
                                          int sw, int ph, int pw, int dh, int dw, int dg, void* workspace,
                                          size_t workspace_bytes, cnuda_stream_t stream) {
    DcnFwdCall c{};
    if (int rc = fill_geom(c.g, B, C, H, W, Cout, kh, kw, sh, sw, ph, pw, dh, dw, dg, "cnuda_dcn_v2_forward")) return rc;
    const DcnPlan q = make_plan(c.g);
    if (stats) {
        int rows = 0;
        const int blk = plan_stats_block(c.g, q, &rows);
        CNUDA_REQUIRE(blk != 0, "cnuda_dcn_v2_forward_stats: no statistics for this call (cnuda_dcn_v2_stats_block says which)");
        CNUDA_REQUIRE(blk == stats_block && rows == stats_rows,
                      "cnuda_dcn_v2_forward_stats: the statistics buffer was sized for blocks of %d pixels x %d rows, this call "
                      "writes %d x %d (did the offset regime change between cnuda_dcn_v2_stats_block and the call?)",
                      stats_block, stats_rows, blk, rows);
    }
    c.input = input; c.weight = weight; c.bias = bias; c.offset = offset; c.mask = mask;
    c.output = output; c.columns = columns; c.stats = stats; c.act_slope = -1.0f;
    c.workspace = workspace; c.workspace_bytes = workspace_bytes; c.stream = stream;
    return dcn_forward_impl(c, q);
}

extern "C" int cnuda_dcn_v2_forward_om(const float* input, const float* weight, const float* bias, const float* om,
                                       float* output, float* columns, float* stats, int stats_block, int stats_rows,
                                       float act_slope, int B,
                                       int C, int H, int W, int Cout, int kh, int kw, int sh, int sw, int ph, int pw, int dh,
                                       int dw, int dg, void* workspace, size_t workspace_bytes, cnuda_stream_t stream) {
    CNUDA_REQUIRE(om && dg == 1 && W >= 2, "cnuda_dcn_v2_forward_om: needs deformable_group == 1 and width >= 2");
    DcnFwdCall c{};
    if (int rc = fill_geom(c.g, B, C, H, W, Cout, kh, kw, sh, sw, ph, pw, dh, dw, dg, "cnuda_dcn_v2_forward_om")) return rc;
    const DcnPlan q = make_plan(c.g);
    if (stats) {
        int rows = 0;
        const int blk = plan_stats_block(c.g, q, &rows);
        CNUDA_REQUIRE(blk != 0 && blk == stats_block && rows == stats_rows,
                      "cnuda_dcn_v2_forward_om: the statistics buffer was sized for blocks of %d pixels x %d rows, this call "
                      "writes %d x %d", stats_block, stats_rows, blk, rows);
    }
    CNUDA_REQUIRE(!stats || act_slope < 0.0f, "cnuda_dcn_v2_forward_om: statistics are those of the output before an activation");
    c.g.off_bs = c.g.mask_bs = 3 * q.T * c.g.Ho * c.g.Wo;
    c.input = input; c.weight = weight; c.bias = bias; c.offset = om; c.mask = om + (size_t)2 * q.T * c.g.Ho * c.g.Wo;
    c.output = output; c.columns = columns; c.stats = stats; c.act_slope = act_slope;
    c.workspace = workspace; c.workspace_bytes = workspace_bytes; c.stream = stream;
    return dcn_forward_impl(c, q);
}

static int dcn_backward_impl(const DcnBwdCall& c, const DcnPlan& q) {
    const DcnGeom& g = c.g;
    CNUDA_REQUIRE(!c.columns || g.W >= 2, "cnuda_dcn_v2_backward_cols: columns input needs width >= 2");
    CNUDA_REQUIRE(c.input && c.weight && c.offset && c.mask && c.grad_output && c.grad_input && c.grad_offset && c.grad_mask &&
                      c.grad_weight && c.grad_bias,
                  "cnuda_dcn_v2_backward: null pointer");
    hipStream_t st = (hipStream_t)c.stream;
    const int T = q.T, HoWo = g.Ho * g.Wo;
    if (q.fwd == DcnFwdPath::Composed) {
        const int Cg = g.C / g.dg;
        const long long HW = (long long)g.H * g.W;
        const size_t inner = cnuda_dcn_v2_workspace_bytes(g.B, Cg, g.H, g.W, g.Co, g.kh, g.kw, g.sh, g.sw, g.ph, g.pw, g.dh, g.dw, 1);
        Carver cv(c.workspace, c.workspace_bytes);
        float* xg = cv.take<float>((size_t)g.B * Cg * HW);
        float* wg = cv.take<float>((size_t)g.Co * Cg * T);
        float* ging = cv.take<float>((size_t)g.B * Cg * HW);
        float* gwg = cv.take<float>((size_t)g.Co * Cg * T);
        float* gbt = cv.take<float>((size_t)g.Co);
        void* iws = cv.take<char>(inner);
        CNUDA_REQUIRE(c.workspace && cv.cur <= cv.end, "cnuda_dcn_v2_backward: workspace too small");
        DcnBwdCall gc = c;
        gc.g.C = Cg; gc.g.dg = 1;
        gc.input = xg; gc.weight = wg; gc.grad_input = ging; gc.grad_weight = gwg;
        gc.workspace = iws; gc.workspace_bytes = inner;
        const DcnPlan gq = make_plan(gc.g);
        const PackStampSuspend uncached;
        for (int grp = 0; grp < g.dg; ++grp) {
            if (int rc = cnuda_copy_channels(c.input, xg, g.B, Cg, HW, g.C, grp * Cg, Cg, 0, c.stream)) return rc;
            if (int rc = cnuda_copy_channels(c.weight, wg, g.Co, Cg, T, g.C, grp * Cg, Cg, 0, c.stream)) return rc;
            if (c.accumulate_input)
                if (int rc = cnuda_copy_channels(c.grad_input, ging, g.B, Cg, HW, g.C, grp * Cg, Cg, 0, c.stream)) return rc;
            gc.offset = c.offset + (size_t)grp * 2 * T * HoWo;
            gc.mask = c.mask + (size_t)grp * T * HoWo;
            gc.columns = c.columns ? c.columns + (size_t)grp * g.B * T * Cg * HoWo : nullptr;
            gc.grad_offset = c.grad_offset + (size_t)grp * 2 * T * HoWo;
            gc.grad_mask = c.grad_mask + (size_t)grp * T * HoWo;
            gc.grad_bias = grp == 0 ? c.grad_bias : gbt;
            if (int rc = dcn_backward_impl(gc, gq)) return rc;
            if (int rc = cnuda_copy_channels(ging, c.grad_input, g.B, Cg, HW, Cg, 0, g.C, grp * Cg, c.stream)) return rc;
            if (int rc = cnuda_copy_channels(gwg, c.grad_weight, g.Co, Cg, T, Cg, 0, g.C, grp * Cg, c.stream)) return rc;
        }
        return check_launch("cnuda_dcn_v2_backward(dg>1)");
    }
    const long long gin_elems = (long long)g.B * g.C * g.H * g.W;
    const bool zero_in_prep = !c.accumulate_input && g.dg == 1 && (gin_elems & 3) == 0 && (reinterpret_cast<uintptr_t>(c.grad_input) & 15) == 0;
    if (!c.accumulate_input && !zero_in_prep &&
        hipMemsetAsync(c.grad_input, 0, (size_t)gin_elems * sizeof(float), st) != hipSuccess)
        return check_launch("cnuda_dcn_v2_backward(memset)");
    if (g.dg != 1) {
        launch_channel_sum(c.grad_output, c.grad_bias, g.B, g.Co, HoWo, st);
        (void)hipMemsetAsync(c.grad_offset, 0, (size_t)g.B * g.dg * 2 * T * HoWo * sizeof(float), st);
        (void)hipMemsetAsync(c.grad_mask, 0, (size_t)g.B * g.dg * T * HoWo * sizeof(float), st);
        (void)hipMemsetAsync(c.grad_weight, 0, (size_t)g.Co * g.C * T * sizeof(float), st);
        DcnNaiveParams p{g, c.input, c.weight, nullptr, c.offset, c.mask, c.grad_output, nullptr,
                         c.grad_input, c.grad_offset, c.grad_mask, c.grad_weight};
        CNUDA_LAUNCH(dcn_naive_bwd_kernel, dim3(stream_grid((long long)g.B * g.C * T * HoWo, 256)), dim3(256), 0, st,
                           p);
        return check_launch("cnuda_dcn_v2_backward(dg>1)");
    }
    CNUDA_REQUIRE(c.workspace && c.workspace_bytes >= q.bwd_bytes, "cnuda_dcn_v2_backward: workspace too small");
    Carver cv(c.workspace, c.workspace_bytes);
    ProfGroup prof;
    if (int rc = wgrad_then_reduce(
            q.wg, cv, std::max((size_t)g.Co * g.B, (size_t)q.wg.Z * q.wg.Mpw), c.grad_weight, c.grad_bias, g.Co, g.C, q.T, st, 4,
            "cnuda_dcn_v2_backward(weight)", "cnuda_dcn_v2_backward(weight reduce)", [&](ProfScope& wscope, float* slabs, float* bsl) -> int {
                bool found;
                if (c.columns) {
                    DcnColWParams p{g, c.columns, c.grad_output};
                    wscope.name(q.colw_ws ? "igemm_wgrad_ws_kernel<%s, 64, %d>" : "igemm_wgrad_kernel<%s, 64, %d>",
                                q.colw_buf ? "DcnColWBufLoader" : "DcnColWLoader", q.wg.bj);
                    found = q.colw_ws    ? launch_wgrad<DcnColWBufLoader, true, Tile<64, 64>, Tile<64, 128>>(q.wg, p, slabs, bsl, st)
                            : q.colw_buf ? launch_wgrad<DcnColWBufLoader, false, Tile<64, 64>, Tile<64, 128>>(q.wg, p, slabs, bsl, st)
                                         : launch_wgrad<DcnColWLoader, false, Tile<64, 64>, Tile<64, 128>>(q.wg, p, slabs, bsl, st);
                } else {
                    DcnWParams p{g, c.input, c.offset, c.mask, c.grad_output};
                    wscope.name("igemm_wgrad_kernel<DcnWLoader, 64, 64>");
                    WgradShape s = q.wg;  s.bj = WG_BJ;
                    found = launch_wgrad<DcnWLoader, false, Tile<64, 64>>(s, p, slabs, bsl, st);
                }
                CNUDA_REQUIRE(found, "cnuda_dcn_v2_backward: no weight-gradient instance for %d-column tiles", q.wg.bj);
                return 0;
            }))
        return rc;
    float* wt = cv.take<float>((size_t)12 * g.C * (g.Co < 64 ? 64 : g.Co));
    float* dcol = cv.take<float>((size_t)g.B * q.T * g.C * HoWo);
    DcnGeo* geo = cv.take<DcnGeo>((size_t)g.B * q.T * HoWo);
    void* gemm_ws = cv.take<char>(q.gemm_bytes);
    {
        {
            const int wt_blocks = stream_grid((long long)q.T * g.C * g.Co, 256);
            const int geo_blocks = q.fused_consumers ? stream_grid((long long)g.B * q.T * HoWo, 256) : 0;
            const int zero_blocks = zero_in_prep ? stream_grid(gin_elems / 4, 256) : 0;
            DcnPrepParams pp{g, c.weight, c.offset, c.mask, wt, q.fused_consumers ? geo : nullptr, wt_blocks,
                             zero_in_prep ? c.grad_input : nullptr, gin_elems / 4, wt_blocks + geo_blocks};
            CNUDA_LAUNCH(dcn_prep_kernel, dim3(wt_blocks + geo_blocks + zero_blocks), dim3(256), 0, st, pp);
        }
        const bool quads = q.dcol_quads;
        if (int rc = quads ? cnuda_conv2d_forward_rowquads(c.grad_output, wt, dcol, g.B, g.Co, g.Ho, g.Wo, q.T * g.C, 1, 1, 1, 1, 0, 0,
                                                           gemm_ws, q.gemm_bytes, c.stream)
                           : cnuda_conv2d_forward(c.grad_output, wt, nullptr, dcol, g.B, g.Co, g.Ho, g.Wo, q.T * g.C, 1, 1, 1, 1, 0,
                                                  0, -1.0f, gemm_ws, q.gemm_bytes, c.stream))
            return rc;
        if (q.fused_consumers) {
            DcnBwdDataParams p{g, c.input, dcol, geo, c.grad_input, c.grad_offset, c.grad_mask, q.tile, q.fused_split};
            const int n_wg = g.B * q.tile.tiles_y * q.tile.tiles_x * q.fused_split;
            ProfScope scope(st, 3);
            scope.name("dcn_bwd_data_kernel");
            if (int rc = with_quads(quads, [&](auto Q) -> int {
                    CNUDA_REQUIRE(raise_dynamic_lds(reinterpret_cast<const void*>(&dcn_bwd_data_kernel<Q()>), q.col2im_lds),
                                  "cnuda_dcn_v2_backward: dynamic LDS");
                    CNUDA_LAUNCH((dcn_bwd_data_kernel<Q()>), dim3(n_wg), dim3(512), q.col2im_lds, st, p, n_wg);
                    return 0;
                }))
                return rc;
        } else {
            {
                DcnCoordParams p{g, c.input, c.offset, c.mask, dcol, c.grad_offset, c.grad_mask, geo};
                const int tiles = ceil_div(HoWo, 64), tw = q.T < 16 ? q.T : 16;
                ProfScope scope(st, 1);
                scope.name("dcn_coord_grad_kernel");
                with_quads(quads, [&](auto Q) {
                    CNUDA_LAUNCH((dcn_coord_grad_kernel<Q()>), dim3(g.B * tiles), dim3(64, tw), 0, st, p, tiles);
                });
            }
            {
                DcnCol2imParams p{g, dcol, geo, c.grad_input, q.tile};
                const int n_wg = g.B * q.tile.tiles_y * q.tile.tiles_x * q.tile.ncg;
                ProfScope scope(st, 2);
                scope.name("dcn_col2im_kernel");
                if (int rc = with_quads(quads, [&](auto Q) -> int {
                        CNUDA_REQUIRE(raise_dynamic_lds(reinterpret_cast<const void*>(&dcn_col2im_kernel<Q()>), q.col2im_lds),
                                      "cnuda_dcn_v2_backward: dynamic LDS");
                        CNUDA_LAUNCH((dcn_col2im_kernel<Q()>), dim3(n_wg), dim3(256), q.col2im_lds, st, p, n_wg);
                        return 0;
                    }))
                    return rc;
            }
        }
        if (int rc = check_launch("cnuda_dcn_v2_backward(data)")) return rc;
    }
    return check_launch("cnuda_dcn_v2_backward");
}

extern "C" int cnuda_dcn_v2_backward(const float* input, const float* weight, const float* bias, const float* offset,
                                     const float* mask, const float* grad_output, float* grad_input,
                                     float* grad_offset, float* grad_mask, float* grad_weight, float* grad_bias, int B,
                                     int C, int H, int W, int Cout, int kh, int kw, int sh, int sw, int ph, int pw,
                                     int dh, int dw, int dg, void* workspace, size_t workspace_bytes,
                                     cnuda_stream_t stream) {
    return cnuda_dcn_v2_backward_cols(input, weight, bias, offset, mask, grad_output, nullptr, grad_input, grad_offset,
                                      grad_mask, grad_weight, grad_bias, B, C, H, W, Cout, kh, kw, sh, sw, ph, pw, dh,
                                      dw, dg, workspace, workspace_bytes, stream);
}

extern "C" int cnuda_dcn_v2_backward_cols(const float* input, const float* weight, const float* bias,
                                          const float* offset, const float* mask, const float* grad_output,
                                          const float* columns, float* grad_input, float* grad_offset,
                                          float* grad_mask, float* grad_weight, float* grad_bias, int B, int C, int H,
                                          int W, int Cout, int kh, int kw, int sh, int sw, int ph, int pw, int dh,
                                          int dw, int dg, void* workspace, size_t workspace_bytes,
                                          cnuda_stream_t stream) {
    return cnuda_dcn_v2_backward_acc(input, weight, bias, offset, mask, grad_output, columns, grad_input, 0, grad_offset,
                                     grad_mask, grad_weight, grad_bias, B, C, H, W, Cout, kh, kw, sh, sw, ph, pw, dh, dw, dg,
                                     workspace, workspace_bytes, stream);
}

extern "C" int cnuda_dcn_v2_backward_acc(const float* input, const float* weight, const float* bias,
                                         const float* offset, const float* mask, const float* grad_output,
                                         const float* columns, float* grad_input, int accumulate_input,
                                         float* grad_offset, float* grad_mask, float* grad_weight, float* grad_bias, int B,
                                         int C, int H, int W, int Cout, int kh, int kw, int sh, int sw, int ph, int pw,
                                         int dh, int dw, int dg, void* workspace, size_t workspace_bytes,
                                         cnuda_stream_t stream) {
    DcnBwdCall c{};
    if (int rc = fill_geom(c.g, B, C, H, W, Cout, kh, kw, sh, sw, ph, pw, dh, dw, dg, "cnuda_dcn_v2_backward")) return rc;
    c.input = input; c.weight = weight; c.bias = bias; c.offset = offset; c.mask = mask;
    c.grad_output = grad_output; c.columns = columns; c.grad_input = grad_input; c.accumulate_input = accumulate_input;
    c.grad_offset = grad_offset; c.grad_mask = grad_mask; c.grad_weight = grad_weight; c.grad_bias = grad_bias;
    c.workspace = workspace; c.workspace_bytes = workspace_bytes; c.stream = stream;
    return dcn_backward_impl(c, make_plan(c.g));
}

extern "C" int cnuda_dcn_v2_backward_om(const float* input, const float* weight, const float* bias, const float* om,
                                        const float* grad_output, const float* columns, float* grad_input,
                                        int accumulate_input, float* grad_om, float* grad_weight, float* grad_bias, int B,
                                        int C, int H, int W, int Cout, int kh, int kw, int sh, int sw, int ph, int pw, int dh,
                                        int dw, int dg, void* workspace, size_t workspace_bytes, cnuda_stream_t stream) {
    CNUDA_REQUIRE(om && grad_om && dg == 1 && W >= 2, "cnuda_dcn_v2_backward_om: needs deformable_group == 1 and width >= 2");
    DcnBwdCall c{};
    if (int rc = fill_geom(c.g, B, C, H, W, Cout, kh, kw, sh, sw, ph, pw, dh, dw, dg, "cnuda_dcn_v2_backward_om")) return rc;
    DcnGeom& g = c.g;
    const size_t mo = (size_t)2 * kh * kw * g.Ho * g.Wo;
    g.off_bs = g.mask_bs = g.goff_bs = g.gmask_bs = 3 * kh * kw * g.Ho * g.Wo;
    g.gmask_logit = 1;
    c.input = input; c.weight = weight; c.bias = bias; c.offset = om; c.mask = om + mo;
    c.grad_output = grad_output; c.columns = columns; c.grad_input = grad_input; c.accumulate_input = accumulate_input;
    c.grad_offset = grad_om; c.grad_mask = grad_om + mo; c.grad_weight = grad_weight; c.grad_bias = grad_bias;
    c.workspace = workspace; c.workspace_bytes = workspace_bytes; c.stream = stream;
    return dcn_backward_impl(c, make_plan(c.g));
}
```

centernet-uda_amd/csrc/igemm.cuh:

```cuda
#pragma once
#include <type_traits>
#include <utility>
#include "common.h"
#include "igemm_host.h"

namespace cnuda {

using f32x16 = __attribute__((ext_vector_type(16))) float;

constexpr int IG_BN = 128;
constexpr int IG_BK = 16;
constexpr int IG_KC = 16;
constexpr int IG_THREADS = 256;

template <int BM> struct IgTile;
template <> struct IgTile<128> { static constexpr int WM = 2, WN = 2, TM = 2, TN = 2; };
template <> struct IgTile<64>  { static constexpr int WM = 2, WN = 2, TM = 1, TN = 2; };
template <> struct IgTile<32>  { static constexpr int WM = 1, WN = 4, TM = 1, TN = 1; };

__device__ __forceinline__ int xcd_remap(int bid, int nwg) {
    constexpr int NX = 8;
    const int per = nwg / NX, rem = nwg % NX;
    const int x = bid % NX, q = bid / NX;
    const int start = x * per + (x < rem ? x : rem);
// ... 576 lines not shown
        }
    }
#pragma unroll
    for (int j = 0; j < T::TN; ++j) {
        const long long n = n0 + wn_off + j * 32 + (lane & 31);
        if (n >= N) continue;
        typename Loader::Out out(p, n);
#pragma unroll
        for (int i = 0; i < T::TM; ++i)
#pragma unroll
            for (int r = 0; r < 16; ++r) {
                const int m = m0 + wm_off + i * 32 + mfma_row(r, lane);
                if (m < M) out.store(p, m, acc[i][j][r]);
            }
    }
}

template <int BM, class Loader, int KC = IG_KC>
__global__ __launch_bounds__(2 * IG_THREADS, (BM == 128 ? 2 : 1)) void igemm_fwd_ws_kernel(
    typename Loader::Params p, const float* __restrict__ A, int Mp, int Kp, int M, long long N,
    int n_tiles, int m_tiles) {
    igemm_fwd_ws_body<BM, Loader, KC>(p, A, Mp, Kp, M, N, n_tiles, m_tiles);
}
template <int BM, class Loader, int KC = IG_KC>
__global__ __launch_bounds__(2 * IG_THREADS, (BM == 128 ? 2 : 1)) void igemm_fwd_ws_splitk_kernel(
    typename Loader::Params p, const float* __restrict__ A, int Mp, int Kp, int M, long long N,
    int n_tiles, int m_tiles, float* __restrict__ slab, int split_k) {
    igemm_fwd_ws_body<BM, Loader, KC, true>(p, A, Mp, Kp, M, N, n_tiles, m_tiles, slab, split_k);
}

template <int BMT, int LDA, class Loader, int KP>
__device__ __forceinline__ void ig_shortk_tile(const typename Loader::Params& p, float* __restrict__ As,
                                               const float* __restrict__ Bs, int m0, long long n0, int lane, int wid, int M,
                                               long long N) {
    using T = IgTile<BMT>;
    const int wm_off = (wid / T::WN) * (T::TM * 32), wn_off = (wid % T::WN) * (T::TN * 32);
    f32x16 acc[T::TM][T::TN];
    ig_zero(acc);
#pragma unroll
    for (int c = 0; c < KP / IG_KC; ++c)
        ig_mma_chunk<BMT, IG_KC, LDA>(As + c * IG_KC * LDA, Bs + c * IG_KC * IG_BN, acc, wm_off, wn_off, lane);
    if constexpr (IgHasQuads<typename Loader::Out>::value) {
        ig_epilogue_quads<BMT, Loader>(p, acc, m0, n0, wm_off, wn_off, lane, M, N);
        return;
    }
    __syncthreads();
    if constexpr (Loader::Out::kVec4) {
        if (Loader::Out::vec4_ok(p)) {
            ig_epilogue_vec4<BMT, Loader>(p, As + wid * IG_EPI_WAVE, acc, m0, n0, wm_off, wn_off, lane, M, N);
            return;
        }
    }
#pragma unroll
    for (int j = 0; j < T::TN; ++j) {
        const long long n = n0 + wn_off + j * 32 + (lane & 31);
        if (n >= N) continue;
        typename Loader::Out out(p, n);
#pragma unroll
        for (int i = 0; i < T::TM; ++i)
#pragma unroll
            for (int r = 0; r < 16; ++r) {
                const int m = m0 + wm_off + i * 32 + mfma_row(r, lane);
                if (m < M) out.store(p, m, acc[i][j][r]);
            }
    }
}

template <int BM, class Loader, int KP>
__global__ __launch_bounds__(IG_THREADS, 2) void igemm_fwd_shortk_kernel(
    typename Loader::Params p, const float* __restrict__ A, int Mp, int Kp, int M, long long N, int n_tiles, int m_tiles) {
    static_assert(KP % IG_KC == 0 && KP * BM >= 4 * IG_EPI_WAVE, "the A buffer holds the epilogue staging tiles");
    __shared__ __attribute__((aligned(16))) float As[KP * BM];
    __shared__ __attribute__((aligned(16))) float Bs[KP * IG_BN];
    const int tid = threadIdx.x, lane = tid & 63, wid = tid >> 6;
    const long long n0 = (long long)xcd_remap(blockIdx.x, n_tiles) * IG_BN;
    {
        const int nl = tid & (IG_BN - 1), ksub = tid >> 7;
        Loader ld(p, n0 + nl, n0 + nl < N);
        float rb[KP / IG_BK][8];
#pragma unroll
        for (int c = 0; c < KP / IG_BK; ++c) ld.load(c * IG_BK, ksub, rb[c]);
#pragma unroll
        for (int c = 0; c < KP / IG_BK; ++c)
#pragma unroll
            for (int j = 0; j < 8; ++j) Bs[(c * IG_BK + ksub + 2 * j) * IG_BN + nl] = rb[c][j];
    }
    constexpr int CELLS = KP * BM / 4, PER = CELLS / IG_THREADS;
    static_assert(CELLS % IG_THREADS == 0, "whole 16-byte cells per thread");
    const buf_rsrc ra = ig_make_rsrc(A, (unsigned)((size_t)Kp * Mp * sizeof(float)));
    f32x4 cell[PER];
    auto load_a = [&](int mt) {
#pragma unroll
        for (int i = 0; i < PER; ++i) {
            const int e = tid + i * IG_THREADS, kk = e / (BM / 4), m = (e % (BM / 4)) * 4;
            cell[i] = ig_buf_load4(ra, kk < Kp ? (unsigned)((kk * Mp + m) * (int)sizeof(float)) : IG_BUF_OOB,
                                   (unsigned)(mt * BM) * (unsigned)sizeof(float));
        }
    };
    load_a(0);
    for (int mt = 0; mt < m_tiles; ++mt) {
        const int m0 = mt * BM;
        __syncthreads();
#pragma unroll
        for (int i = 0; i < PER; ++i) reinterpret_cast<f32x4*>(As)[tid + i * IG_THREADS] = cell[i];
        __syncthreads();
        if (mt + 1 < m_tiles) load_a(mt + 1);
        if constexpr (BM == 128) {
            if (M - m0 <= 64) {
                ig_shortk_tile<64, BM, Loader, KP>(p, As, Bs, m0, n0, lane, wid, M, N);
                continue;
            }
        }
        ig_shortk_tile<BM, BM, Loader, KP>(p, As, Bs, m0, n0, lane, wid, M, N);
    }
}

constexpr int WG_BM = 64, WG_BJ = 64, WG_BP = 32;

struct IgPixelCursor {
    int left_;
    int b_, pp_, oy_, ox_;
    int crossed_;
    bool valid_;
    __device__ __forceinline__ void init(long long n, long long n_end, int HoWo, int Wo) {
        const long long d = n_end - n;
        left_ = d > 0x7fffffffll ? 0x7fffffff : (d < 0 ? 0 : (int)d);
        valid_ = left_ > 0;
        const long long nn = valid_ ? n : 0;
        b_ = (int)(nn / HoWo);
        pp_ = (int)(nn - (long long)b_ * HoWo);
        oy_ = pp_ / Wo;
        ox_ = pp_ - oy_ * Wo;
        crossed_ = 0;
    }
    __device__ __forceinline__ void advance(int HoWo, int Wo) {
        left_ = left_ > WG_BP ? left_ - WG_BP : 0;
        valid_ = left_ > 0;
        pp_ += WG_BP;
        ox_ += WG_BP;
        crossed_ = 0;
        while (ox_ >= Wo) { ox_ -= Wo; ++oy_; }
        while (pp_ >= HoWo) { pp_ -= HoWo; ++b_; ++crossed_; oy_ = pp_ / Wo; ox_ = pp_ - oy_ * Wo; }
    }
};
__device__ __forceinline__ int ig_mad24(int a, int b, int c) { return __mul24(a, b) + c; }
template <int NV, int STEP>
__device__ __forceinline__ void ig_buf_rows(buf_rsrc rs, const IgPixelCursor& c, unsigned image_base, int HoWo, int row0,
                                            int sub, float (&v)[NV]) {
    const unsigned voff = c.valid_ ? image_base + (unsigned)ig_mad24(sub, HoWo, c.pp_) * 4u : IG_BUF_OOB;
#pragma unroll
    for (int i = 0; i < NV; ++i) v[i] = ig_buf_load(rs, voff, (unsigned)((row0 + STEP * i) * HoWo) * (unsigned)sizeof(float));
}

template <int NG, int STEP>
__device__ __forceinline__ void ig_wgrad_store_bias(float (&bs)[NG], float* __restrict__ dst, int pl, int sub) {
    static_assert(WG_BP == 32, "a row group's pixel lanes are one half of a wave");
#pragma unroll
    for (int i = 0; i < NG; ++i) {
        float v = bs[i];
#pragma unroll
        for (int d = 16; d >= 1; d >>= 1) v += __shfl_xor(v, d, 64);
        if (pl == 0) dst[sub + STEP * i] = v;
    }
}

template <int BM, int BJ>
struct IgWgradTile {
    static constexpr int GLD = BM + 1, BLD = BJ + 1;
    static constexpr int STEP = IG_THREADS / WG_BP;
    static constexpr int TM = (BM == 128 && BJ == 128) ? 2 : 1, TJ = (BM / 32) * (BJ / 32) / 4 / TM;
    static constexpr int WJ = BJ / 32 / TJ, NG = BM / STEP, NB = BJ / STEP;
    static_assert((BM / 32 / TM) * WJ == 4, "four waves tile the block");
};

template <class WLoader, int BM, int BJ>
struct IgWgradStager {
    using W = IgWgradTile<BM, BJ>;
    const int pl, sub, m0, j0;
    WLoader ld;
    const bool do_bias;
    float rg[W::NG], rb[W::NB], bs[W::NG];
    __device__ __forceinline__ IgWgradStager(const typename WLoader::Params& p, long long n_begin, long long n_end, int m0_,
                                             int j0_, int tid, bool do_bias_)
        : pl(tid % WG_BP), sub(tid / WG_BP), m0(m0_), j0(j0_), ld(p, n_begin + pl, n_end), do_bias(do_bias_) {
#pragma unroll
        for (int i = 0; i < W::NG; ++i) bs[i] = 0.0f;
    }
    __device__ __forceinline__ void load() {
        ld.template load_g<W::NG, W::STEP>(m0, sub, rg);
        ld.template load_b<W::NB, W::STEP>(j0, sub, rb);
    }
    __device__ __forceinline__ void advance_load() { ld.advance(); load(); }
    __device__ __forceinline__ void store(float* Gs, float* Bs) {
#pragma unroll
        for (int i = 0; i < W::NG; ++i) Gs[pl * W::GLD + sub + W::STEP * i] = rg[i];
#pragma unroll
        for (int i = 0; i < W::NB; ++i) Bs[pl * W::BLD + sub + W::STEP * i] = rb[i];
        if (do_bias) {
#pragma unroll
            for (int i = 0; i < W::NG; ++i) bs[i] += rg[i];
        }
    }
    __device__ __forceinline__ void store_bias(float* __restrict__ bslab, int Mp) {
        if (do_bias) ig_wgrad_store_bias<W::NG, W::STEP>(bs, bslab + (size_t)blockIdx.z * Mp + m0, pl, sub);
    }
};

template <int BM, int BJ>
__device__ __forceinline__ void ig_wgrad_mma_chunk(const float* Gs, const float* Bs,
                                                   f32x16 (&acc)[IgWgradTile<BM, BJ>::TM][IgWgradTile<BM, BJ>::TJ],
                                                   int wm_off, int wj_off, int lane) {
    using W = IgWgradTile<BM, BJ>;
    constexpr int TM = W::TM, TJ = W::TJ, GLD = W::GLD, BLD = W::BLD;
    const int kl = lane >> 5, il = lane & 31;
    const float* gp = Gs + kl * GLD + wm_off + il;
    const float* bp = Bs + kl * BLD + wj_off + il;
    float a[2][2][TM], b[2][2][TJ];
    auto frag = [&](int kk, float (&fa)[2][TM], float (&fb)[2][TJ]) {
#pragma unroll
        for (int i = 0; i < TM; ++i) { fa[0][i] = gp[kk * GLD + i * 32]; fa[1][i] = gp[(kk + 2) * GLD + i * 32]; }
#pragma unroll
        for (int t = 0; t < TJ; ++t) { fb[0][t] = bp[kk * BLD + t * 32]; fb[1][t] = bp[(kk + 2) * BLD + t * 32]; }
    };
    auto mma = [&](const float (&fa)[2][TM], const float (&fb)[2][TJ]) {
#pragma unroll
        for (int h = 0; h < 2; ++h)
#pragma unroll
            for (int i = 0; i < TM; ++i)
#pragma unroll
                for (int t = 0; t < TJ; ++t)
                    acc[i][t] = __builtin_amdgcn_mfma_f32_32x32x2f32(fa[h][i], fb[h][t], acc[i][t], 0, 0, 0);
    };
    frag(0, a[0], b[0]);
#pragma unroll
    for (int kk = 0; kk < WG_BP; kk += 8) {
        frag(kk + 4, a[1], b[1]);
        __builtin_amdgcn_sched_barrier(0);
        mma(a[0], b[0]);
        __builtin_amdgcn_sched_barrier(0);
        if (kk + 8 < WG_BP) frag(kk + 8, a[0], b[0]);
        __builtin_amdgcn_sched_barrier(0);
        mma(a[1], b[1]);
        __builtin_amdgcn_sched_barrier(0);
    }
}

template <int BM, int BJ>
__device__ __forceinline__ void ig_wgrad_store_slab(float* __restrict__ slabs,
                                                    const f32x16 (&acc)[IgWgradTile<BM, BJ>::TM][IgWgradTile<BM, BJ>::TJ],
                                                    int Mp, int Jp, int m0, int j0, int wm_off, int wj_off, int lane) {
    using W = IgWgradTile<BM, BJ>;
    float* slab = slabs + (size_t)blockIdx.z * Mp * Jp;
#pragma unroll
    for (int i = 0; i < W::TM; ++i)
#pragma unroll
        for (int t = 0; t < W::TJ; ++t)
#pragma unroll
            for (int r = 0; r < 16; ++r) {
                const int m = m0 + wm_off + i * 32 + mfma_row(r, lane);
                const int j = j0 + wj_off + t * 32 + (lane & 31);
                slab[(size_t)m * Jp + j] = acc[i][t][r];
            }
}

template <class WLoader, int BM, int BJ>
__global__ __launch_bounds__(IG_THREADS) void igemm_wgrad_kernel(
    typename WLoader::Params p, float* __restrict__ slabs, int Mp, int Jp, long long N, long long pix_per_split,
    float* __restrict__ bslab) {
    using W = IgWgradTile<BM, BJ>;
    __shared__ float Gs[2][WG_BP * W::GLD];
    __shared__ float Bs[2][WG_BP * W::BLD];
    const int tid = threadIdx.x, lane = tid & 63, wid = tid >> 6;
    const int j0 = blockIdx.x * BJ, m0 = blockIdx.y * BM;
    const long long n_begin = (long long)blockIdx.z * pix_per_split;
    long long n_end = n_begin + pix_per_split;
    if (n_end > N) n_end = N;
    const int wm_off = (wid / W::WJ) * 32 * W::TM, wj_off = (wid % W::WJ) * 32 * W::TJ;
    IgWgradStager<WLoader, BM, BJ> stg(p, n_begin, n_end, m0, j0, tid, bslab != nullptr && blockIdx.x == 0);
    f32x16 acc[W::TM][W::TJ];
    ig_zero(acc);
    stg.load();
    stg.store(Gs[0], Bs[0]);
    if (n_begin + WG_BP < n_end) stg.advance_load();
    __syncthreads();
    int cur = 0;
    for (long long nb = n_begin; nb < n_end; nb += WG_BP) {
        ig_wgrad_mma_chunk<BM, BJ>(Gs[cur], Bs[cur], acc, wm_off, wj_off, lane);
        if (nb + WG_BP < n_end) {
            stg.store(Gs[cur ^ 1], Bs[cur ^ 1]);
            if (nb + 2 * WG_BP < n_end) stg.advance_load();
        }
        __syncthreads();
        cur ^= 1;
    }
    ig_wgrad_store_slab<BM, BJ>(slabs, acc, Mp, Jp, m0, j0, wm_off, wj_off, lane);
    stg.store_bias(bslab, Mp);
}

template <class WLoader, int BM, int BJ>
__global__ __launch_bounds__(2 * IG_THREADS) void igemm_wgrad_ws_kernel(
    typename WLoader::Params p, float* __restrict__ slabs, int Mp, int Jp, long long N, long long pix_per_split,
    float* __restrict__ bslab) {
    using W = IgWgradTile<BM, BJ>;
    __shared__ float Gs[2][WG_BP * W::GLD];
    __shared__ float Bs[2][WG_BP * W::BLD];
    const bool producer = threadIdx.x >= IG_THREADS;
    const int tid = threadIdx.x & (IG_THREADS - 1), lane = tid & 63, wid = tid >> 6;
    const int j0 = blockIdx.x * BJ, m0 = blockIdx.y * BM;
    const long long n_begin = (long long)blockIdx.z * pix_per_split;
    long long n_end = n_begin + pix_per_split;
    if (n_end > N) n_end = N;
    if (producer) {
        IgWgradStager<WLoader, BM, BJ> stg(p, n_begin, n_end, m0, j0, tid, bslab != nullptr && blockIdx.x == 0);
        const int nchunk = (int)((n_end - n_begin + WG_BP - 1) / WG_BP);
        stg.load();
        stg.store(Gs[0], Bs[0]);
        if (1 < nchunk) stg.advance_load();
        __syncthreads();
        int cur = 0;
        for (int c = 0; c < nchunk; ++c) {
            if (c + 1 < nchunk) {
                stg.store(Gs[cur ^ 1], Bs[cur ^ 1]);
                if (c + 2 < nchunk) stg.advance_load();
            }
            __syncthreads();
            cur ^= 1;
        }
        stg.store_bias(bslab, Mp);
        return;
    }
    const int wm_off = (wid / W::WJ) * 32 * W::TM, wj_off = (wid % W::WJ) * 32 * W::TJ;
    f32x16 acc[W::TM][W::TJ];
    ig_zero(acc);
    __syncthreads();
    int cur = 0;
    for (long long nb = n_begin; nb < n_end; nb += WG_BP) {
        ig_wgrad_mma_chunk<BM, BJ>(Gs[cur], Bs[cur], acc, wm_off, wj_off, lane);
        __syncthreads();
        cur ^= 1;
    }
    ig_wgrad_store_slab<BM, BJ>(slabs, acc, Mp, Jp, m0, j0, wm_off, wj_off, lane);
}

template <class Loader, bool WS, class... Tiles, class P>
bool launch_wgrad(const WgradShape& s, const P& p, float* slabs, float* bsl, hipStream_t st) {
    const dim3 grid(s.Jp / s.bj, s.Mpw / s.bm, s.Z), blk((WS ? 2 : 1) * IG_THREADS);
    return with_tiles<Tiles...>(s.bm, s.bj, [&](auto BM, auto BJ) {
        if constexpr (WS)
            CNUDA_LAUNCH((igemm_wgrad_ws_kernel<Loader, BM(), BJ()>), grid, blk, 0, st, p, slabs, s.Mpw, s.Jp, s.N, s.pix_per_split, bsl);
        else
// ... 20 lines not shown
```

centernet-uda_amd/hip_runtime/__init__.py:

```python
import ctypes
import os
import threading
import weakref

import torch

_PKG_ROOT = os.path.dirname(os.path.dirname(os.path.abspath(__file__)))
LIB_PATH = os.path.join(_PKG_ROOT, 'libcenternet_uda_hip.so')
ABI_VERSION = 2

_lib = None
_lock = threading.Lock()
_workspaces = {}

c_int, c_size_t, c_void_p, c_float = ctypes.c_int, ctypes.c_size_t, ctypes.c_void_p, ctypes.c_float


def lib():
    global _lib
    if _lib is None:
        with _lock:
            if _lib is None:
                if not os.path.exists(LIB_PATH):
                    raise RuntimeError(
                        "%s not found: build it with `make -C centernet-uda_amd/csrc` "
                        "(or __graft_entry__.build()); there is no CPU/eager fallback" % LIB_PATH)
                l = ctypes.CDLL(LIB_PATH)
                l.cnuda_last_error.restype = ctypes.c_char_p
                l.cnuda_abi_version.restype = c_int
                if l.cnuda_abi_version() != ABI_VERSION:
                    raise RuntimeError("libcenternet_uda_hip.so ABI %d != expected %d"
                                       % (l.cnuda_abi_version(), ABI_VERSION))
                for name in dir(_Sig):
                    if name.startswith('cnuda_'):
                        restype, argtypes = getattr(_Sig, name)
                        fn = getattr(l, name)
                        fn.restype, fn.argtypes = restype, argtypes
                _lib = l
    return _lib


_I = c_int
_P = c_void_p


_LL = ctypes.c_longlong
_F = c_float
_D = ctypes.c_double
_WS = [_P, c_size_t, _P]


class _Sig:
    cnuda_decode_workspace_bytes = (c_size_t, [_I] * 5)
    cnuda_decode_set_max_bands = (_I, [_I])
    cnuda_decode_set_stage2_threads = (_I, [_I])
    cnuda_decode_detection = (_I, [_P] * 5 + [_I] * 8 + _WS)
    cnuda_nms = (_I, [_P, _P] + [_I] * 5 + [_P])
    cnuda_dcn_v2_workspace_bytes = (c_size_t, [_I] * 14)
    cnuda_dcn_v2_forward = (_I, [_P] * 6 + [_I] * 14 + _WS)
    cnuda_dcn_v2_backward = (_I, [_P] * 11 + [_I] * 14 + _WS)
    cnuda_dcn_v2_forward_cols = (_I, [_P] * 7 + [_I] * 14 + _WS)
    cnuda_dcn_v2_forward_act = (_I, [_P] * 7 + [_F] + [_I] * 14 + _WS)
    cnuda_dcn_v2_forward_stats = (_I, [_P] * 8 + [_I] * 16 + _WS)
    cnuda_dcn_v2_stats_block = (_I, [_I] * 14 + [_P])
    cnuda_dcn_v2_forward_om = (_I, [_P] * 7 + [_I] * 2 + [_F] + [_I] * 14 + _WS)
    cnuda_dcn_v2_backward_om = (_I, [_P] * 7 + [_I] + [_P] * 3 + [_I] * 14 + _WS)
    cnuda_dcn_v2_backward_cols = (_I, [_P] * 12 + [_I] * 14 + _WS)
    cnuda_dcn_v2_backward_acc = (_I, [_P] * 8 + [_I] + [_P] * 4 + [_I] * 14 + _WS)
    cnuda_dcn_v2_psroi_pooling_workspace_bytes = (c_size_t, [_I] * 4)
    cnuda_dcn_v2_psroi_pooling_forward = (_I, [_P] * 5 + [_I] * 6 + [_F] + [_I] * 5 + [_F, _I, _P])
    cnuda_dcn_v2_psroi_pooling_backward = (_I, [_P] * 6 + [_I, _P] + [_I] * 6 + [_F] + [_I] * 5 + [_F, _I] + _WS)
    cnuda_eval_workspace_bytes = (c_size_t, [_I, _I])
    cnuda_eval_box_spans = (_I, [_P, _I, _I, _I, _P, _P] + _WS)
    cnuda_eval_iou_rotated = (_I, [_P, _I, _I, _I, _LL, _P, _P, _I, _P] + _WS)
    cnuda_eval_iou_axis = (_I, [_P, _P, _P, _I, _I, _I, _LL, _P, _P])
    cnuda_eval_match = (_I, [_P, _P, _I, _P, _P, _I, _I, _LL, _P, _I, _P, _P, _P, _P])
    cnuda_eval_match_flagged = (_I, [_P, _P, _I, _P, _P, _P, _I, _I, _LL, _P, _I, _P, _P, _P, _P])
    cnuda_eval_oks = (_I, [_P] * 6 + [_I, _P, _I, _I, _I, _LL, _P, _P, _P, _P])
    cnuda_conv2d_workspace_bytes = (c_size_t, [_I] * 11)
    cnuda_conv2d_forward = (_I, [_P] * 4 + [_I] * 11 + [_F] + _WS)
    cnuda_conv2d_forward_res = (_I, [_P] * 5 + [_I] * 11 + [_F] + _WS)
    cnuda_conv2d_rowsig_supported = (_I, [_I] * 11)
    cnuda_conv2d_forward_rowsig = (_I, [_P] * 4 + [_I] * 12 + _WS)
    cnuda_conv2d_rowquads_supported = (_I, [_I] * 11)
    cnuda_conv2d_cat_supported = (_I, [_P, _I, _I, _I, _I, _I])
    cnuda_conv2d_cat_forward = (_I, [_P, _P, _I, _P, _P, _P, _P, _F, _I, _I, _I, _I] + _WS)
    cnuda_conv2d_cat_backward_data = (_I, [_P, _P, _P, _P, _P, _P, _I, _I, _I, _I, _I] + _WS)
    cnuda_conv2d_cat_backward_weight = (_I, [_P, _P, _I, _P, _P, _I, _I, _I, _I] + _WS)
    cnuda_conv2d_forward_rowquads = (_I, [_P] * 3 + [_I] * 11 + _WS)
    cnuda_conv2d_backward_data = (_I, [_P] * 3 + [_I] * 11 + _WS)
    cnuda_conv2d_backward_data_add = (_I, [_P] * 5 + [_I] * 11 + _WS)
    cnuda_conv2d_stats_block = (_I, [_I] * 11 + [_P, _P])
    cnuda_conv2d_forward_stats = (_I, [_P] * 6 + [_I] * 11 + [_F] + _WS)
    cnuda_bn_train_forward_stats = (_I, [_P, _P, _LL, _I] + [_P] * 9 + [_F, _F, _I, _I, _I, _LL, _I] + _WS)
    cnuda_conv2d_backward_weight = (_I, [_P] * 4 + [_I] * 11 + _WS)
    cnuda_conv2d_norm_input_supported = (_I, [_I] * 11)
    cnuda_conv2d_forward_norm_input = (_I, [_P] * 5 + [_I] + [_P] * 4 + [_I] * 11 + [_F] + _WS)
    cnuda_conv2d_backward_weight_norm_input = (_I, [_P] * 5 + [_I] + [_P] * 3 + [_I] * 11 + _WS)
    cnuda_bn_workspace_bytes = (c_size_t, [_I, _I, _LL])
    cnuda_bn_train_forward = (_I, [_P] * 10 + [_F, _F, _I, _I, _I, _LL, _I] + _WS)
    cnuda_bn_eval_forward = (_I, [_P] * 7 + [_F, _I, _I, _I, _LL, _P])
    cnuda_bn_backward = (_I, [_P] * 11 + [_I, _I, _I, _LL, _I] + _WS)
    cnuda_maxpool2d_forward = (_I, [_P] * 2 + [_I] * 5 + [_P])
    cnuda_maxpool2d_backward = (_I, [_P] * 3 + [_I] * 5 + [_P])
    cnuda_maxpool2d_backward_acc = (_I, [_P] * 3 + [_I] * 6 + [_P])
    cnuda_maxpool2d_window_forward = (_I, [_P] * 2 + [_I] * 7 + [_P])
    cnuda_maxpool2d_window_backward = (_I, [_P] * 3 + [_I] * 7 + [_P])
    cnuda_dwconvt2d_forward = (_I, [_P] * 3 + [_I] * 7 + [_P])
    cnuda_dwconvt2d_add_forward = (_I, [_P] * 4 + [_I] * 7 + [_P])
    cnuda_dwconvt2d_workspace_bytes = (c_size_t, [_I] * 3)
    cnuda_dwconvt2d_backward = (_I, [_P] * 5 + [_I] * 7 + _WS)
    cnuda_dwconv2d_workspace_bytes = (c_size_t, [_I] * 3)
    cnuda_dwconv2d_forward = (_I, [_P] * 3 + [_I] * 7 + [_P])
    cnuda_dwconv2d_backward = (_I, [_P] * 5 + [_I] * 7 + _WS)
    cnuda_dwconv2d_same_workspace_bytes = (c_size_t, [_I] * 3)
    cnuda_dwconv2d_same_forward = (_I, [_P] * 3 + [_I] * 10 + [_P])
    cnuda_dwconv2d_same_backward = (_I, [_P] * 5 + [_I] * 10 + _WS)
    cnuda_swish_forward = (_I, [_P] * 2 + [_LL, _P])
    cnuda_swish_backward = (_I, [_P] * 3 + [_LL, _P])
    cnuda_se_workspace_bytes = (c_size_t, [_I] * 3)
    cnuda_se_forward = (_I, [_P] * 9 + [_I] * 3 + [_LL, _P])
    cnuda_se_backward = (_I, [_P] * 12 + [_I] * 3 + [_LL] + _WS)
    cnuda_drop_connect_add = (_I, [_P] * 4 + [_I, _LL, _P])
    cnuda_pad_right_bottom = (_I, [_P] * 2 + [_LL] + [_I] * 4 + [_P])
    cnuda_add = (_I, [_P] * 3 + [_LL, _P])
    cnuda_act_backward = (_I, [_P] * 3 + [_LL, _F, _P])
    cnuda_conv1x1_backward_data_act = (_I, [_P] * 4 + [_I] * 3 + [_LL, _F, _P])
    cnuda_head_backward_sparse_supported = (_I, [_I] * 13)
    cnuda_head_backward_sparse_workspace_bytes = (c_size_t, [_I] * 9)
    cnuda_head_backward_sparse = (_I, [_P] * 12 + [_I] * 9 + [_F] + _WS)
    cnuda_copy_channels = (_I, [_P, _P, _I, _I, _LL, _I, _I, _I, _I, _P])
    cnuda_split_offset_mask = (_I, [_P] * 3 + [_I, _I, _LL, _P])
    cnuda_split_offset_mask_backward = (_I, [_P] * 4 + [_I, _I, _LL, _P])
    cnuda_loss_workspace_bytes = (c_size_t, [])
    cnuda_focal_loss_forward = (_I, [_P] * 4 + [_LL, _F] + _WS)
    cnuda_focal_loss_backward = (_I, [_P] * 5 + [_LL, _F, _P])
    cnuda_reg_l1_forward = (_I, [_P] * 5 + [_I, _I, _I, _LL, _I, _F, _F, _P])
    cnuda_reg_l1_backward = (_I, [_P] * 7 + [_I, _I, _I, _LL, _I, _F, _F, _P])
    cnuda_kps_l1_forward = (_I, [_P] * 6 + [_I, _I, _I, _LL, _I, _I, _F, _F, _P])
    cnuda_kps_l1_backward = (_I, [_P] * 8 + [_I, _I, _I, _LL, _I, _I, _F, _F, _P])
    cnuda_decode_keypoints = (_I, [_P] * 4 + [_I] * 5 + [_P])
    cnuda_softmax_loss_forward = (_I, [_P, _P, _I, _I, _LL, _I] + _WS)
    cnuda_softmax_loss_backward = (_I, [_P] * 3 + [_I, _I, _LL, _I, _P])
    cnuda_entropy_map_forward = (_I, [_P, _P, _I, _I, _LL, _P])
    cnuda_entropy_map_backward = (_I, [_P] * 3 + [_I, _I, _LL, _P])
    cnuda_entropy_eta_loss_forward = (_I, [_P, _P, _I, _I, _LL, _F] + _WS)
    cnuda_entropy_eta_loss_backward = (_I, [_P] * 3 + [_I, _I, _LL, _F, _P])
    cnuda_argmax_histogram = (_I, [_P, _P, _I, _I, _LL, _P])
    cnuda_iw_max_square_forward = (_I, [_P, _P, _F, _P, _P, _I, _I, _LL] + _WS)
    cnuda_iw_max_square_backward = (_I, [_P] * 4 + [_I, _I, _LL, _P])
    cnuda_bce_const_forward = (_I, [_P, _F, _P, _LL, _P])
    cnuda_bce_const_backward = (_I, [_P, _F, _P, _P, _LL, _P])
    cnuda_sigmoid_clamp_ = (_I, [_P, _P, _LL, _P])
    cnuda_gather_feat = (_I, [_P] * 3 + [_I, _I, _I, _LL, _P])
    cnuda_encode_targets = (_I, [_P] * 10 + [_I] * 5 + [_P])
    cnuda_encode_targets_modes = (_I, [_P] * 17 + [_I] * 6 + [_P])
    cnuda_prepare_input = (_I, [_P, _P, _I, _I, _I] + [_F] * 6 + [_P])
    cnuda_augment_color = (_I, [_P] * 3 + [_I] * 3 + [_P])
    cnuda_augment_warp = (_I, [_P] * 8 + [ctypes.c_ulonglong] + [_I] * 5 + [_P])
    cnuda_augment_points = (_I, [_P] * 3 + [_I] + [_P] * 2 + [_I] * 2 + [_P])
    cnuda_render_detections = (_I, [_P] * 6 + [_I] * 8 + [_F] * 6 + [_P])
    cnuda_meter_update = (_I, [_P, _I, _D, _P, _P, _P, _P])
    cnuda_mirror_input = (_I, [_P, _P, _LL, _I, _I, _P])
    cnuda_tta_merge = (_I, [_P] * 9 + [_I] * 6 + [_P])
    cnuda_project_detections = (_I, [_P] * 9 + [_I] * 4 + [_F, _F, _I, _I, _P])
    cnuda_predict_workspace_bytes = (c_size_t, [_I, _I])
    cnuda_soft_nms_merge = (_I, [_P] * 10 + [_I] * 5 + [_F] + _WS)
    cnuda_fda_workspace_bytes = (c_size_t, [_I] * 4)
    cnuda_fda_source_to_target = (_I, [_P] * 4 + [_I] * 4 + _WS)
    cnuda_adam_step = (_I, [_P] * 4 + [_LL] + [_F] * 5 + [_I, _P])
    cnuda_sgd_step = (_I, [_P] * 3 + [_LL] + [_D] * 4 + [_I] * 3 + [_P])
    cnuda_adamw_step = (_I, [_P] * 5 + [_LL] + [_D] * 5 + [_I] * 3 + [_P])
    cnuda_rmsprop_step = (_I, [_P] * 5 + [_LL] + [_D] * 5 + [_I, _P])
    cnuda_set_matrix_mode = (_I, [_I])
    cnuda_get_matrix_mode = (_I, [])
    cnuda_pack_cache_attach = (_I, [_P, c_size_t])
    cnuda_pack_stamp = (_I, [ctypes.c_ulonglong, ctypes.c_ulonglong])
    cnuda_pack_refresh = (_I, [_P, ctypes.c_size_t, ctypes.c_ulonglong, ctypes.c_ulonglong, _P, ctypes.c_size_t, _P])
    cnuda_pack_refresh_ranges = (_I, [_P, _P, _I, ctypes.c_ulonglong, ctypes.c_ulonglong, _P, ctypes.c_size_t, _P])
    cnuda_ema_update = (_I, [_P, _I, ctypes.c_uint, _F, _F, _P])
    cnuda_pseudo_labels = (_I, [_P] * 6 + [_I] * 6 + [_F, _P])
    cnuda_pack_cache_used = (c_size_t, [])
    cnuda_pack_cache_fills = (ctypes.c_ulonglong, [])
    cnuda_pack_cache_resets = (ctypes.c_ulonglong, [])
    cnuda_prof_enable = (_I, [_I])
    cnuda_prof_arm = (_I, [_I])
    cnuda_prof_collect = (_I, [_P, _P, _P, _I])
    cnuda_prof_name_len = (_I, [])
    cnuda_launch_log_enable = (_I, [_I])
    cnuda_launch_log_collect = (_I, [ctypes.c_char_p, c_size_t])
    cnuda_dcn_set_fused_min_tiles = (_I, [_I])
    cnuda_dcn_set_scatter_margin = (_I, [_I])
    cnuda_dcn_set_offset_regime = (_I, [_I])
    cnuda_dcn_set_walk_tile = (_I, [_I])
    cnuda_dcn_offset_census = (_I, [_P, _I, _I, _LL, _P, _P])
    cnuda_conv_set_halo_policy = (_I, [_I, _I])
    cnuda_conv_set_splitk_policy = (_I, [_I])


_PARAM_EPOCH = 0


def bump_param_epoch(rewritten=None):
    global _PARAM_EPOCH
    if rewritten is not None and not isinstance(rewritten, torch.Tensor):
        several = [t for t in rewritten if t is not None]
        if len(several) > 1:
            return _bump_several(several)
        rewritten = several[0] if several else None
    if _HELD is not None:
        _HELD.append(rewritten)
        return
    old = _PARAM_EPOCH
    _PARAM_EPOCH += 1
    if rewritten is not None and rewritten.is_cuda and _PACK['arena'] is not None and not _PACK['off']:
        if _PACK.get('table') is None or _PACK['table'].device != rewritten.device:
            _PACK['table'] = torch.empty(1 << 18, dtype=torch.uint8, device=rewritten.device)
# ... 163 lines not shown


def _stream_handle():
    if _raw_stream is not None and _cur_device is not None:
        return _raw_stream(_cur_device())
    return torch.cuda.current_stream().cuda_stream


def stream():
    return c_void_p(_stream_handle())


def require_gpu(*tensors):
    for t in tensors:
        if t is not None and not t.is_cuda:
            raise RuntimeError("centernet-uda_amd ops run on MI355X only: got a %s tensor "
                               "(there is no CPU fallback; the CPU oracle lives in oracle/ for tests)"
                               % t.device)


def f32c(t):
    if t.dtype != torch.float32:
        raise RuntimeError("expected float32, got %s" % t.dtype)
    if getattr(t, '_cnuda_deferred_bn', None) is not None:
        raise RuntimeError("this tensor is the unwritten output of a deferred BatchNorm (apply on load): only ops.conv2d "
                           "may consume it; build the BatchNorm without defer_apply for other consumers")
    return t if t.is_contiguous() else t.contiguous()


def workspace(nbytes, device):
    key = (device.index if device.index is not None else torch.cuda.current_device(), _stream_handle())
    buf = _workspaces.get(key)
    if buf is None or buf.numel() < nbytes:
        buf = torch.empty(max(int(nbytes), 1 << 20), dtype=torch.uint8, device=device)
        _workspaces[key] = buf
    return buf


def stats_side_output(box, query, geom, HoWo, device, per_image=False):
    rows, bpi = ctypes.c_int(0), ctypes.c_int(0)
    blk = query(*geom, ctypes.byref(rows), *([ctypes.byref(bpi)] if per_image else []))
    if not blk:
        return None
    nblk = geom[0] * bpi.value if bpi.value else (geom[0] * HoWo + 127) // 128 * (128 // blk)
    stats = torch.empty((nblk, rows.value, 2), dtype=torch.float32, device=device)
    box.append((stats, 0 if bpi.value else blk, rows.value, bpi.value))
    return box[-1]


class _Prof:
    enabled = False
    table = []
    shapes = []
    cap = 0


def set_matrix_mode(mode):
    check(lib().cnuda_set_matrix_mode(int(mode)), 'set_matrix_mode')


def get_matrix_mode():
    return int(lib().cnuda_get_matrix_mode())


def prof_arm(kind, B, C, H, W, Co, kh, kw, Ho, Wo):
    if not _Prof.enabled or len(_Prof.table) >= _Prof.cap:
        return
    flops = 2.0 * B * Ho * Wo * Co * C * kh * kw
    if kind == 'dcn_bwd':
        T, px = kh * kw, B * Ho * Wo
        coord_bytes = 4.0 * px * (T * C + 3 * T + 3 * T + 4 * T) + 4.0 * B * C * H * W
        col2im_bytes = 4.0 * px * T * C + 16.0 * px * T * ((C + 15) // 16) + 4.0 * B * C * H * W
        fused_bytes = 4.0 * px * T * C + 16.0 * px * T + 12.0 * px * T + 8.0 * B * C * H * W
        _Prof.table.append([(flops, 0.0), (0.0, coord_bytes), (0.0, col2im_bytes), (0.0, fused_bytes), (flops, 0.0)])
    elif kind in ('conv_fwd', 'conv_dgrad', 'conv_wgrad', 'dcn_fwd'):
        nbytes = 4.0 * B * (C * H * W + Co * Ho * Wo)
        if kind == 'dcn_fwd':
            nbytes += 4.0 * B * Ho * Wo * (3 * kh * kw + kh * kw * C)
        _Prof.table.append([(flops, nbytes)])
    else:
        raise ValueError(kind)
    _Prof.shapes.append((kind, B, C, H, W, Co, kh, kw, Ho, Wo))
    lib().cnuda_prof_arm(len(_Prof.table) - 1)


def prof_begin(max_records=16384):
    check(lib().cnuda_prof_enable(int(max_records)), 'prof_enable')
    _Prof.enabled, _Prof.table, _Prof.shapes, _Prof.cap = True, [], [], int(max_records)


def prof_end(by_shape=False):
    n = sum(len(e) for e in _Prof.table)
    L = lib()
    nl = int(L.cnuda_prof_name_len())
    tags = (ctypes.c_int * max(n, 1))()
    ms = (ctypes.c_float * max(n, 1))()
    names = ctypes.create_string_buffer(max(n, 1) * nl)
    got = L.cnuda_prof_collect(tags, ms, names, n)
    out = {}
    for i in range(got):
        flops, nbytes = _Prof.table[tags[i] & 0xffffff][tags[i] >> 24]
        name = names.raw[i * nl:(i + 1) * nl].split(b'\0', 1)[0].decode() or 'unnamed launch'
        key = (name, _Prof.shapes[tags[i] & 0xffffff]) if by_shape else name
        d = out.setdefault(key, {'launches': 0, 'ms': 0.0, 'flops': 0.0, 'bytes': 0.0})
        d['launches'] += 1
        d['ms'] += float(ms[i])
        d['flops'] += flops
        d['bytes'] += nbytes
    _Prof.enabled, _Prof.table, _Prof.shapes = False, [], []
    lib().cnuda_prof_enable(0)
    return out


def launch_counts():
    L = lib()
    L.cnuda_launch_log_enable(1)
    buf = ctypes.create_string_buffer(1 << 18)
    n = L.cnuda_launch_log_collect(buf, len(buf))
    if n < 0:
        check(n, 'launch_log_collect')
    out = {}
    for line in buf.value.decode().split('\n'):
        if line:
            name, _, count = line.rpartition('\t')
            out[name] = int(count)
    return out


class launch_log:

    def __enter__(self):
        self.before = launch_counts()
        self.names, self.counts = [], {}
        return self

    def __exit__(self, *exc):
        after = launch_counts()
        self.counts = {k: v - self.before.get(k, 0) for k, v in after.items() if v > self.before.get(k, 0)}
        self.names = list(self.counts)


class dcn_fused_min_tiles:

    def __init__(self, n):
        self.n = int(n)

    def __enter__(self):
        self.prev = lib().cnuda_dcn_set_fused_min_tiles(self.n)

    def __exit__(self, *exc):
        lib().cnuda_dcn_set_fused_min_tiles(self.prev)


class splitk:

    def __init__(self, max_tiles):
        self.max_tiles = int(max_tiles)

    def __enter__(self):
        self.prev = lib().cnuda_conv_set_splitk_policy(self.max_tiles)

    def __exit__(self, *exc):
        lib().cnuda_conv_set_splitk_policy(self.prev)


class halo_conv:

    def __init__(self, level, min_tiles):
        self.level, self.min_tiles = int(level), int(min_tiles)

    def __enter__(self):
        prev = lib().cnuda_conv_set_halo_policy(-1, 0)
        self.prev = (prev & 0xff, prev >> 8)
        lib().cnuda_conv_set_halo_policy(self.level, self.min_tiles)

    def __exit__(self, *exc):
        lib().cnuda_conv_set_halo_policy(*self.prev)
```

centernet-uda_amd/libs/DCNv2/dcn_v2.py:

```python
import math
import os as _os

import torch
from torch import nn

import _ext as _backend
import hip_runtime as hr
from hip_runtime import nn as hnn
from hip_runtime import ops
from hip_runtime.arena import grad_sink
from hip_runtime.fanout import accumulate_in_place, claim, fork, slot_of


_KEEP_COLUMNS = _os.environ.get('CNUDA_DCN_KEEP_COLS', '1') != '0'
USE_OM = _os.environ.get('CNUDA_DCN_OM', '1') != '0'


def _pair(v):
    return tuple(v) if isinstance(v, (tuple, list)) else (v, v)


def _node_forward(ctx, fwd, input, sampling, weight, bias, geom, keep, pack_token, stats_box, regime):
    ctx.regime = int(regime)
    ctx.slot = slot_of(input)
    ctx.geom = geom
    keep = keep and any(ctx.needs_input_grad[:3 + len(sampling)]) and _KEEP_COLUMNS
    with _offset_regime(ctx.regime):
        out = fwd(input, weight, bias, *sampling, *geom, _want_columns=keep, _pack_token=pack_token, _stats_box=stats_box)
    out, cols = out if isinstance(out, tuple) else (out, None)
    ctx.save_for_backward(input, *sampling, weight, bias, cols)
    return out


def _node_backward(ctx, bwd, grad_output):
    input, *sampling, weight, bias, cols = ctx.saved_tensors
    sw, sb = grad_sink(weight), grad_sink(bias)
    acc = accumulate_in_place(ctx.slot)
    with _offset_regime(ctx.regime):
        g_in, *g_sampling, g_w, g_b = bwd(input, weight, bias, *sampling, grad_output, *ctx.geom, _columns=cols,
                                          _grad_weight=sw, _grad_bias=sb, _grad_input=acc)
    if acc is None:
        claim(ctx.slot, g_in)
    return g_in, g_sampling, (None if sw is not None else g_w), (None if sb is not None else g_b)


class _DeformConvFn(torch.autograd.Function):
    @staticmethod
    def forward(ctx, input, offset, mask, weight, bias, stride, padding, dilation, deformable_groups, pack_token=0,
                stats_box=None, regime=0):
        geom = tuple(weight.shape[2:]) + _pair(stride) + _pair(padding) + _pair(dilation) + (deformable_groups,)
        return _node_forward(ctx, _backend.dcn_v2_forward, input, (offset, mask), weight, bias, geom, input.shape[3] >= 2,
                             pack_token, stats_box, regime)

    @staticmethod
    @torch.autograd.function.once_differentiable
    def backward(ctx, grad_output):
        g_in, (g_off, g_mask), g_w, g_b = _node_backward(ctx, _backend.dcn_v2_backward, grad_output)
        return g_in, g_off, g_mask, g_w, g_b, None, None, None, None, None, None, None


class _DeformConvOmFn(torch.autograd.Function):

    @staticmethod
    def forward(ctx, input, om, weight, bias, stride, padding, dilation, pack_token=0, stats_box=None, regime=0):
        geom = tuple(weight.shape[2:]) + _pair(stride) + _pair(padding) + _pair(dilation)
        return _node_forward(ctx, _backend.dcn_v2_forward_om, input, (om,), weight, bias, geom, True, pack_token, stats_box,
                             regime)

    @staticmethod
    @torch.autograd.function.once_differentiable
    def backward(ctx, grad_output):
        g_in, (g_om,), g_w, g_b = _node_backward(ctx, _backend.dcn_v2_backward_om, grad_output)
        return g_in, g_om, g_w, g_b, None, None, None, None, None, None


class _offset_regime:

    def __init__(self, regime):
        self.regime = regime
        self.prev = 0

    def __enter__(self):
        self.prev = hr.lib().cnuda_dcn_set_offset_regime(self.regime)

    def __exit__(self, *exc):
        hr.lib().cnuda_dcn_set_offset_regime(self.prev)


def dcn_v2_conv(input, offset, mask, weight, bias, stride, padding, dilation, deformable_groups, pack_token=0,
                emit_stats=False, regime=0):
    return ops.with_bn_stats(emit_stats, lambda box: _DeformConvFn.apply(
        input, offset, mask, weight, bias, stride, padding, dilation, deformable_groups, pack_token, box, regime))


class DCNv2(nn.Module):
    def __init__(self, in_channels, out_channels, kernel_size, stride, padding, dilation=1,
                 deformable_groups=1):
        super().__init__()
        self.in_channels, self.out_channels = in_channels, out_channels
        self.kernel_size, self.stride = _pair(kernel_size), _pair(stride)
        self.padding, self.dilation = _pair(padding), _pair(dilation)
        self.deformable_groups = deformable_groups
        self.weight = nn.Parameter(torch.empty(out_channels, in_channels, *self.kernel_size))
        self.bias = nn.Parameter(torch.empty(out_channels))
        self._pack_token = hr.PackToken()
        self.reset_parameters()

    def reset_parameters(self):
        bound = 1.0 / math.sqrt(self.in_channels * self.kernel_size[0] * self.kernel_size[1])
        with torch.no_grad():
            self.weight.uniform_(-bound, bound)
            self.bias.zero_()

    def forward(self, input, offset, mask):
        taps = self.deformable_groups * self.kernel_size[0] * self.kernel_size[1]
        assert offset.shape[1] == 2 * taps and mask.shape[1] == taps
        return dcn_v2_conv(input, offset, mask, self.weight, self.bias, self.stride, self.padding,
                           self.dilation, self.deformable_groups, self._pack_token)


class DCN(DCNv2):

    def __init__(self, in_channels, out_channels, kernel_size, stride, padding, dilation=1,
                 deformable_groups=1):
        super().__init__(in_channels, out_channels, kernel_size, stride, padding, dilation, deformable_groups)
        taps = self.deformable_groups * self.kernel_size[0] * self.kernel_size[1]
        self.conv_offset_mask = hnn.Conv2d(in_channels, 3 * taps, self.kernel_size, self.stride,
                                           self.padding, bias=True)
        self.emit_stats = False
        self._regime, self._census_calls = 0, 0
        with torch.no_grad():
            self.conv_offset_mask.weight.zero_()
            self.conv_offset_mask.bias.zero_()

    def forward(self, input):
        input_om, input = fork(input, 2)
        taps = self.kernel_size[0] * self.kernel_size[1]
        cm = self.conv_offset_mask
        hooked = bool(cm._forward_hooks or cm._forward_pre_hooks or cm._backward_hooks)
        if self.deformable_groups == 1 and input.shape[3] >= 2 and USE_OM and not hooked:
            om = ops.conv2d_rowsig(input_om, cm.weight, cm.bias, cm.stride, cm.padding, 2 * taps, cm._pack_token)
            if om is not None:
                self._take_census(lambda: om.detach()[:, :2 * taps].contiguous())
                return ops.with_bn_stats(self.emit_stats and self.training, lambda box: _DeformConvOmFn.apply(
                    input, om, self.weight, self.bias, self.stride, self.padding, self.dilation, self._pack_token, box,
                    self._regime))
        om = cm(input_om)
        offset, mask = ops.split_offset_mask(om)
        if self.deformable_groups == 1:
            self._take_census(lambda: offset)
        return dcn_v2_conv(input, offset, mask, self.weight, self.bias, self.stride, self.padding,
                           self.dilation, self.deformable_groups, self._pack_token,
                           emit_stats=self.emit_stats and self.training, regime=self._regime)

    CENSUS_EVERY = 64
    CENSUS_SHARES = (0.015, 0.03)

    def _take_census(self, offsets):
        if self.training:
            self._census_calls += 1
            if self._census_calls % self.CENSUS_EVERY == 1:
                self._regime = self._census(offsets())

    def _census(self, offset):
        off = offset.detach()
        B, HW = off.shape[0], off.shape[2] * off.shape[3]
        taps = off.shape[1] // 2
        counts = torch.zeros(2, dtype=torch.int32, device=off.device)
        hr.check(hr.lib().cnuda_dcn_offset_census(hr.ptr(hr.f32c(off)), B, taps, HW, hr.ptr(counts), hr.stream()), 'census')
        n2, n3 = counts.tolist()
        total = float(B * taps * HW)
        return (1 if n2 > self.CENSUS_SHARES[0] * total else 0) | (2 if n3 > self.CENSUS_SHARES[1] * total else 0)


class _DCNv2Pooling(torch.autograd.Function):
    @staticmethod
    def forward(ctx, input, rois, offset, spatial_scale, pooled_size, output_dim, no_trans, group_size=1,
                part_size=None, sample_per_part=4, trans_std=.0):
        ctx.args = (int(no_trans), spatial_scale, output_dim, group_size, pooled_size,
                    pooled_size if part_size is None else part_size, sample_per_part, trans_std)
        output, output_count = _backend.dcn_v2_psroi_pooling_forward(input, rois, offset, *ctx.args)
        ctx.save_for_backward(input, rois, offset, output_count)
        return output

    @staticmethod
    @torch.autograd.function.once_differentiable
    def backward(ctx, grad_output):
        input, rois, offset, output_count = ctx.saved_tensors
        grad_input, grad_offset = _backend.dcn_v2_psroi_pooling_backward(grad_output, input, rois, offset, output_count,
                                                                         *ctx.args)
        return grad_input, None, grad_offset, None, None, None, None, None, None, None, None


# ... 57 lines not shown
```

include/centernet_uda_hip.h:

```cpp
#ifndef CENTERNET_UDA_HIP_H
#define CENTERNET_UDA_HIP_H

#include <stddef.h>
#include <stdint.h>

#ifdef __cplusplus
extern "C" {
#endif

#define CNUDA_ERR_INVALID_ARGUMENT (-1)
#define CNUDA_ABI_VERSION 2

typedef void* cnuda_stream_t;

int cnuda_abi_version(void);
const char* cnuda_last_error(void);

int cnuda_set_matrix_mode(int mode);
int cnuda_get_matrix_mode(void);

int cnuda_pack_cache_attach(void* arena, size_t bytes);
int cnuda_pack_stamp(unsigned long long token, unsigned long long version);
size_t cnuda_pack_cache_used(void);
unsigned long long cnuda_pack_cache_fills(void);
unsigned long long cnuda_pack_cache_resets(void);
int cnuda_pack_refresh(const void* params, size_t params_bytes, unsigned long long old_epoch,
                       unsigned long long new_epoch, void* table, size_t table_bytes, cnuda_stream_t stream);
int cnuda_pack_refresh_ranges(const void* const* params, const size_t* params_bytes, int ranges,
                              unsigned long long old_epoch, unsigned long long new_epoch, void* table,
                              size_t table_bytes, cnuda_stream_t stream);

int cnuda_prof_enable(int max_records);
int cnuda_prof_arm(int tag);
int cnuda_prof_collect(int* tags, float* ms, char* names, int cap);
int cnuda_prof_name_len(void);

int cnuda_launch_log_enable(int on);
int cnuda_launch_log_collect(char* names, size_t cap);
int cnuda_dcn_set_fused_min_tiles(int min_tiles);
int cnuda_dcn_set_scatter_margin(int margin);
int cnuda_dcn_set_walk_tile(int tile_cols);
int cnuda_dcn_set_offset_regime(int regime);
int cnuda_dcn_offset_census(const float* offset, int B, int taps, long long HW, unsigned* counts, cnuda_stream_t stream);
int cnuda_conv_set_halo_policy(int level, int min_tiles);
int cnuda_conv_set_splitk_policy(int max_tiles);

int cnuda_decode_set_max_bands(int max_bands);
int cnuda_decode_set_stage2_threads(int threads);
size_t cnuda_decode_workspace_bytes(int B, int C, int H, int W, int K);
int cnuda_decode_detection(const float* heat, const float* wh, const float* reg,
                           float* dets, int64_t* inds,
                           int B, int C, int H, int W, int K, int wh_ch, int rotated, int nms_size,
                           void* workspace, size_t workspace_bytes, cnuda_stream_t stream);
int cnuda_decode_keypoints(const float* kps, const float* reg, const int64_t* inds, float* out,
                           int B, int J, int K, int H, int W, cnuda_stream_t stream);
int cnuda_nms(const float* heat, float* out, int B, int C, int H, int W, int nms_size,
              cnuda_stream_t stream);

size_t cnuda_dcn_v2_workspace_bytes(int B, int C, int H, int W, int Cout, int kh, int kw,
                                    int sh, int sw, int ph, int pw, int dh, int dw, int dg);
int cnuda_dcn_v2_forward(const float* input, const float* weight, const float* bias,
                         const float* offset, const float* mask, float* output,
                         int B, int C, int H, int W, int Cout, int kh, int kw,
                         int sh, int sw, int ph, int pw, int dh, int dw, int dg,
                         void* workspace, size_t workspace_bytes, cnuda_stream_t stream);
int cnuda_dcn_v2_backward(const float* input, const float* weight, const float* bias,
                          const float* offset, const float* mask, const float* grad_output,
                          float* grad_input, float* grad_offset, float* grad_mask,
                          float* grad_weight, float* grad_bias,
                          int B, int C, int H, int W, int Cout, int kh, int kw,
                          int sh, int sw, int ph, int pw, int dh, int dw, int dg,
                          void* workspace, size_t workspace_bytes, cnuda_stream_t stream);

int cnuda_dcn_v2_forward_act(const float* input, const float* weight, const float* bias,
                             const float* offset, const float* mask, float* output, float* columns,
                             float act_slope,
                             int B, int C, int H, int W, int Cout, int kh, int kw,
                             int sh, int sw, int ph, int pw, int dh, int dw, int dg,
                             void* workspace, size_t workspace_bytes, cnuda_stream_t stream);
int cnuda_dcn_v2_stats_block(int B, int C, int H, int W, int Cout, int kh, int kw, int sh, int sw, int ph, int pw,
                             int dh, int dw, int dg, int* rows);
int cnuda_dcn_v2_forward_stats(const float* input, const float* weight, const float* bias, const float* offset,
                               const float* mask, float* output, float* columns, float* stats, int stats_block,
                               int stats_rows,
                               int B, int C, int H, int W, int Cout, int kh, int kw, int sh, int sw, int ph, int pw,
                               int dh, int dw, int dg, void* workspace, size_t workspace_bytes, cnuda_stream_t stream);

int cnuda_dcn_v2_forward_om(const float* input, const float* weight, const float* bias, const float* om, float* output,
                            float* columns, float* stats, int stats_block, int stats_rows,
                            float act_slope ,
                            int B, int C, int H, int W, int Cout, int kh, int kw, int sh, int sw, int ph, int pw,
                            int dh, int dw, int dg, void* workspace, size_t workspace_bytes, cnuda_stream_t stream);
int cnuda_dcn_v2_backward_om(const float* input, const float* weight, const float* bias, const float* om,
                             const float* grad_output, const float* columns, float* grad_input, int accumulate_input,
                             float* grad_om, float* grad_weight, float* grad_bias,
                             int B, int C, int H, int W, int Cout, int kh, int kw, int sh, int sw, int ph, int pw,
                             int dh, int dw, int dg, void* workspace, size_t workspace_bytes, cnuda_stream_t stream);

int cnuda_dcn_v2_forward_cols(const float* input, const float* weight, const float* bias,
                              const float* offset, const float* mask, float* output, float* columns,
                              int B, int C, int H, int W, int Cout, int kh, int kw,
                              int sh, int sw, int ph, int pw, int dh, int dw, int dg,
                              void* workspace, size_t workspace_bytes, cnuda_stream_t stream);
int cnuda_dcn_v2_backward_cols(const float* input, const float* weight, const float* bias,
                               const float* offset, const float* mask, const float* grad_output,
                               const float* columns,
                               float* grad_input, float* grad_offset, float* grad_mask,
                               float* grad_weight, float* grad_bias,
                               int B, int C, int H, int W, int Cout, int kh, int kw,
                               int sh, int sw, int ph, int pw, int dh, int dw, int dg,
                               void* workspace, size_t workspace_bytes, cnuda_stream_t stream);

int cnuda_dcn_v2_backward_acc(const float* input, const float* weight, const float* bias,
                              const float* offset, const float* mask, const float* grad_output,
                              const float* columns,
                              float* grad_input, int accumulate_input, float* grad_offset, float* grad_mask,
                              float* grad_weight, float* grad_bias,
                              int B, int C, int H, int W, int Cout, int kh, int kw,
                              int sh, int sw, int ph, int pw, int dh, int dw, int dg,
                              void* workspace, size_t workspace_bytes, cnuda_stream_t stream);

size_t cnuda_dcn_v2_psroi_pooling_workspace_bytes(int B, int num_rois, int output_dim, int pooled_size);
int cnuda_dcn_v2_psroi_pooling_forward(const float* input, const float* rois, const float* trans,
                                       float* output, float* output_count,
                                       int B, int channels, int H, int W, int num_rois, int no_trans,
                                       float spatial_scale, int output_dim, int group_size, int pooled_size,
                                       int part_size, int sample_per_part, float trans_std, int num_classes,
                                       cnuda_stream_t stream);
int cnuda_dcn_v2_psroi_pooling_backward(const float* grad_output, const float* input, const float* rois,
                                        const float* trans, const float* output_count,
                                        float* grad_input, int accumulate_input, float* grad_trans,
                                        int B, int channels, int H, int W, int num_rois, int no_trans,
                                        float spatial_scale, int output_dim, int group_size, int pooled_size,
                                        int part_size, int sample_per_part, float trans_std, int num_classes,
                                        void* workspace, size_t workspace_bytes, cnuda_stream_t stream);

size_t cnuda_eval_workspace_bytes(int num_boxes, int H);
int cnuda_eval_box_spans(const int* verts, int num_boxes, int H, int W, int* rows, double* area,
                         void* workspace, size_t workspace_bytes, cnuda_stream_t stream);
int cnuda_eval_iou_rotated(const int* groups, int num_groups, int num_det, int num_gt, long long num_pairs,
                           const int* rows, const double* area, int H, double* iou,
                           void* workspace, size_t workspace_bytes, cnuda_stream_t stream);
int cnuda_eval_iou_axis(const float* det_boxes, const float* gt_boxes, const int* groups, int num_groups,
                        int num_det, int num_gt, long long num_pairs, double* iou, cnuda_stream_t stream);
int cnuda_eval_match(const double* iou, const int* groups, int num_groups, const double* det_area,
                     const double* gt_area, int num_det, int num_gt, long long num_pairs,
                     const double* thresholds, int num_thresholds, const double* area_ranges,
                     unsigned* det_bits, unsigned char* gt_ignore, cnuda_stream_t stream);
int cnuda_eval_match_flagged(const double* iou, const int* groups, int num_groups, const double* det_area,
                             const double* gt_area, const unsigned char* gt_flags, int num_det, int num_gt,
                             long long num_pairs, const double* thresholds, int num_thresholds,
                             const double* area_ranges, unsigned* det_bits, unsigned char* gt_ignore,
                             cnuda_stream_t stream);
int cnuda_eval_oks(const float* det_kps, const float* gt_kps, const unsigned char* gt_vis, const double* gt_area,
                   const float* gt_box, const double* sigmas, int num_joints, const int* groups, int num_groups,
                   int num_det, int num_gt, long long num_pairs, double* oks, double* det_area,
                   unsigned char* gt_flags, cnuda_stream_t stream);

size_t cnuda_conv2d_workspace_bytes(int B, int C, int H, int W, int Cout, int kh, int kw,
                                    int sh, int sw, int ph, int pw);
int cnuda_conv2d_forward(const float* x, const float* weight, const float* bias, float* y,
                         int B, int C, int H, int W, int Cout, int kh, int kw,
                         int sh, int sw, int ph, int pw, float act_slope,
                         void* workspace, size_t workspace_bytes, cnuda_stream_t stream);
int cnuda_conv2d_forward_res(const float* x, const float* weight, const float* bias, const float* residual, float* y,
                             int B, int C, int H, int W, int Cout, int kh, int kw,
                             int sh, int sw, int ph, int pw, float act_slope,
                             void* workspace, size_t workspace_bytes, cnuda_stream_t stream);
int cnuda_conv2d_rowsig_supported(int B, int C, int H, int W, int Cout, int kh, int kw, int sh, int sw, int ph, int pw);
int cnuda_conv2d_forward_rowsig(const float* x, const float* weight, const float* bias, float* y, int sig_from,
                                int B, int C, int H, int W, int Cout, int kh, int kw, int sh, int sw, int ph, int pw,
                                void* workspace, size_t workspace_bytes, cnuda_stream_t stream);
int cnuda_conv2d_cat_supported(const int* cs, int n, int B, int H, int W, int Cout);
int cnuda_conv2d_cat_forward(const float* const* xs, const int* cs, int n, const float* weight, const float* bias ,
                             float* y, float* stats, float act_slope ,
                             int B, int H, int W, int Cout, void* workspace, size_t workspace_bytes, cnuda_stream_t stream);
int cnuda_conv2d_cat_backward_data(const float* grad_y, const float* weight, float* const* grad_xs, const float* const* adds,
                                   const float* const* add2s, const int* cs, int n, int B, int H, int W, int Cout,
                                   void* workspace, size_t workspace_bytes, cnuda_stream_t stream);
int cnuda_conv2d_cat_backward_weight(const float* const* xs, const int* cs, int n, const float* grad_y, float* grad_weight,
                                     int B, int H, int W, int Cout, void* workspace, size_t workspace_bytes,
                                     cnuda_stream_t stream);
int cnuda_conv2d_rowquads_supported(int B, int C, int H, int W, int Cout, int kh, int kw, int sh, int sw, int ph, int pw);
int cnuda_conv2d_forward_rowquads(const float* x, const float* weight, float* y,
                                  int B, int C, int H, int W, int Cout, int kh, int kw, int sh, int sw, int ph, int pw,
                                  void* workspace, size_t workspace_bytes, cnuda_stream_t stream);
int cnuda_conv2d_stats_block(int B, int C, int H, int W, int Cout, int kh, int kw, int sh, int sw, int ph, int pw, int* rows,
                             int* blocks_per_image );
int cnuda_conv2d_forward_stats(const float* x, const float* weight, const float* bias, const float* residual, float* y,
                               float* stats, int B, int C, int H, int W, int Cout, int kh, int kw,
                               int sh, int sw, int ph, int pw, float act_slope,
                               void* workspace, size_t workspace_bytes, cnuda_stream_t stream);
int cnuda_conv2d_backward_data(const float* grad_y, const float* weight, float* grad_x,
                               int B, int C, int H, int W, int Cout, int kh, int kw,
                               int sh, int sw, int ph, int pw,
                               void* workspace, size_t workspace_bytes, cnuda_stream_t stream);
int cnuda_conv2d_norm_input_supported(int B, int C, int H, int W, int Cout, int kh, int kw, int sh, int sw, int ph, int pw);
int cnuda_conv2d_forward_norm_input(const float* x, const float* mean, const float* invstd, const float* gamma,
                                    const float* beta, int imgs_per_group, const float* weight, const float* bias, float* y,
                                    float* stats, int B, int C, int H, int W, int Cout, int kh, int kw, int sh, int sw, int ph,
                                    int pw, float act_slope, void* workspace, size_t workspace_bytes, cnuda_stream_t stream);
int cnuda_conv2d_backward_weight_norm_input(const float* x, const float* mean, const float* invstd, const float* gamma,
                                            const float* beta, int imgs_per_group, const float* grad_y, float* grad_weight,
                                            float* grad_bias, int B, int C, int H, int W, int Cout, int kh, int kw, int sh,
                                            int sw, int ph, int pw, void* workspace, size_t workspace_bytes,
                                            cnuda_stream_t stream);
int cnuda_conv2d_backward_data_add(const float* grad_y, const float* weight, const float* addend, const float* addend2,
                                   float* grad_x,
                                   int B, int C, int H, int W, int Cout, int kh, int kw,
                                   int sh, int sw, int ph, int pw,
                                   void* workspace, size_t workspace_bytes, cnuda_stream_t stream);
int cnuda_conv2d_backward_weight(const float* x, const float* grad_y, float* grad_weight, float* grad_bias,
                                 int B, int C, int H, int W, int Cout, int kh, int kw,
                                 int sh, int sw, int ph, int pw,
                                 void* workspace, size_t workspace_bytes, cnuda_stream_t stream);

size_t cnuda_bn_workspace_bytes(int B, int C, long long HW);
int cnuda_bn_train_forward(const float* x, const float* gamma, const float* beta, const float* residual,
                           float* y, float* save_mean, float* save_invstd,
                           float* running_mean, float* running_var,
                           long long* num_batches_tracked ,
                           float momentum, float eps, int relu,
                           int B, int C, long long HW,
                           int groups ,
                           void* workspace, size_t workspace_bytes, cnuda_stream_t stream);
int cnuda_bn_train_forward_stats(const float* x, const float* stats, long long blocks_per_group, int rows, const float* gamma,
                                 const float* beta, const float* residual, float* y, float* save_mean, float* save_invstd,
                                 float* running_mean, float* running_var, long long* num_batches_tracked,
                                 float momentum, float eps, int relu, int B, int C, long long HW, int groups,
                                 void* workspace, size_t workspace_bytes, cnuda_stream_t stream);
int cnuda_bn_eval_forward(const float* x, const float* gamma, const float* beta,
                          const float* running_mean, const float* running_var, const float* residual,
                          float* y, float eps, int relu, int B, int C, long long HW, cnuda_stream_t stream);
int cnuda_bn_backward(const float* grad_y, const float* x, const float* y, const float* gamma,
                      const float* beta ,
                      const float* save_mean, const float* save_invstd,
                      float* grad_x, float* grad_residual, float* grad_gamma, float* grad_beta,
                      int relu, int B, int C, long long HW, int groups,
                      void* workspace, size_t workspace_bytes, cnuda_stream_t stream);

int cnuda_maxpool2d_forward(const float* x, float* y, int B, int C, int H, int W, int k, cnuda_stream_t stream);
int cnuda_maxpool2d_backward(const float* x, const float* grad_y, float* grad_x,
                             int B, int C, int H, int W, int k, cnuda_stream_t stream);
int cnuda_maxpool2d_backward_acc(const float* x, const float* grad_y, float* grad_x, int accumulate, int B, int C, int H, int W,
                                 int k, cnuda_stream_t stream);
int cnuda_maxpool2d_window_forward(const float* x, float* y, int B, int C, int H, int W, int k, int s, int p,
                                   cnuda_stream_t stream);
int cnuda_maxpool2d_window_backward(const float* x, const float* grad_y, float* grad_x,
                                    int B, int C, int H, int W, int k, int s, int p, cnuda_stream_t stream);
int cnuda_dwconvt2d_forward(const float* x, const float* w, float* y,
                            int B, int C, int H, int W, int k, int s, int p, cnuda_stream_t stream);
int cnuda_dwconvt2d_add_forward(const float* x, const float* w, const float* skip, float* y,
                                int B, int C, int H, int W, int k, int s, int p, cnuda_stream_t stream);
size_t cnuda_dwconvt2d_workspace_bytes(int B, int C, int k);
int cnuda_dwconvt2d_backward(const float* x, const float* w, const float* grad_y, float* grad_x, float* grad_w,
                             int B, int C, int H, int W, int k, int s, int p,
                             void* workspace, size_t workspace_bytes, cnuda_stream_t stream);
size_t cnuda_dwconv2d_workspace_bytes(int B, int C, int k);
int cnuda_dwconv2d_forward(const float* x, const float* w, float* y, int B, int C, int H, int W, int k, int s, int p,
                           cnuda_stream_t stream);
int cnuda_dwconv2d_backward(const float* x, const float* w, const float* grad_y, float* grad_x, float* grad_w,
                            int B, int C, int H, int W, int k, int s, int p,
                            void* workspace, size_t workspace_bytes, cnuda_stream_t stream);
int cnuda_add(const float* a, const float* b, float* out, long long n, cnuda_stream_t stream);
int cnuda_act_backward(const float* grad_y, const float* y, float* grad_x, long long n, float slope,
                       cnuda_stream_t stream);
int cnuda_conv1x1_backward_data_act(const float* grad_y, const float* weight, const float* hidden, float* grad_hidden,
                                    int B, int Co, int Ch, long long HW, float slope, cnuda_stream_t stream);
int cnuda_head_backward_sparse_supported(int B, int M, int C, int H, int W, int Ch, int Co, int kh, int kw, int sh, int sw,
                                         int ph, int pw);
size_t cnuda_head_backward_sparse_workspace_bytes(int B, int M, int C, int H, int W, int Ch, int Co, int kh, int kw);
int cnuda_head_backward_sparse(const float* grad_y, const long long* ind, const unsigned char* mask, const float* x,
                               const float* hidden, const float* w1, const float* w2, float* grad_x, float* grad_w1,
// ... 152 lines not shown
```

Before: 219.9 images/sec.

## Store DCN column side output in interleaved quads for vector writes and reads

Adds a quad-interleaved storage layout for the deformable-conv column buffer. The forward window kernel writes four channel values per pixel as one 16-byte vector store, and the weight-gradient stager reads them back as vector loads and remaps them to the original row order in shared memory. The aim is to replace strided scalar global stores and loads with coalesced vector accesses. The layout is threaded through the Python forward/backward contexts, and a runtime check rejects a mismatch if the offset regime changes between choosing the layout and launching the kernel.

```diff
diff --git a/centernet-uda_amd/_ext.py b/centernet-uda_amd/_ext.py
--- a/centernet-uda_amd/_ext.py
+++ b/centernet-uda_amd/_ext.py
@@ -20,7 +20,7 @@
 
 
 def _forward(who, input, weight, bias, offset, mask, om, geom, Ho, Wo, want_columns, act_slope, pack_token, pack_version,
-             stats_box):
+             stats_box, columns_quads=False):
     B, C, H, W, Co, kh, kw = geom[:7]
     dg = geom[13]
     out = torch.empty((B, Co, Ho, Wo), dtype=torch.float32, device=input.device)
@@ -28,6 +28,7 @@
     if want_columns and W >= 2:
         cols = torch.empty((B, kh * kw * C, Ho * Wo), dtype=torch.float32, device=input.device)
     L = hr.lib()
+    layout = L.cnuda_dcn_v2_columns_layout(*geom) if cols is not None and columns_quads else 0
     ws = hr.workspace(L.cnuda_dcn_v2_workspace_bytes(*geom), input.device)
     if dg == 1 and W >= 2:
         hr.prof_arm('dcn_fwd', B, C, H, W, Co, kh, kw, Ho, Wo)
@@ -37,7 +38,7 @@
         if rec is not None:
             stats, blk, rows = rec[:3]
     tail = (*geom, hr.ptr(ws), ws.numel(), hr.stream())
-    with hr.pack_stamp(pack_token, weight, pack_version):
+    with hr.pack_stamp(pack_token, weight, pack_version), hr.dcn_columns_layout(layout):
         if om is not None:
             rc = L.cnuda_dcn_v2_forward_om(hr.ptr(input), hr.ptr(weight), hr.ptr(bias), hr.ptr(om), hr.ptr(out), hr.ptr(cols),
                                            hr.ptr(stats), blk, rows, float(act_slope), *tail)
@@ -49,10 +50,11 @@
             rc = L.cnuda_dcn_v2_forward_act(hr.ptr(input), hr.ptr(weight), hr.ptr(bias), hr.ptr(offset), hr.ptr(mask),
                                             hr.ptr(out), hr.ptr(cols), float(act_slope), *tail)
         hr.check(rc, who)
-    return out, cols
-
-
-def _backward(who, input, weight, bias, offset, mask, om, grad_output, geom, columns, grad_weight, grad_bias, grad_input):
+    return out, cols, layout
+
+
+def _backward(who, input, weight, bias, offset, mask, om, grad_output, geom, columns, grad_weight, grad_bias, grad_input,
+              columns_layout=0):
     B, C, H, W, Co, kh, kw = geom[:7]
     g_in = grad_input if grad_input is not None else torch.empty_like(input)
     g_om = [torch.empty_like(om)] if om is not None else [torch.empty_like(offset), torch.empty_like(mask)]
@@ -63,15 +65,17 @@
     if geom[13] == 1:
         hr.prof_arm('dcn_bwd', B, C, H, W, Co, kh, kw, grad_output.shape[2], grad_output.shape[3])
     fn = L.cnuda_dcn_v2_backward_acc if om is None else L.cnuda_dcn_v2_backward_om
-    hr.check(fn(hr.ptr(input), hr.ptr(weight), hr.ptr(bias), *[hr.ptr(t) for t in ((offset, mask) if om is None else (om,))],
+    with hr.dcn_columns_layout(columns_layout if columns is not None else 0):
+        rc = fn(hr.ptr(input), hr.ptr(weight), hr.ptr(bias), *[hr.ptr(t) for t in ((offset, mask) if om is None else (om,))],
                 hr.ptr(grad_output), hr.ptr(columns), hr.ptr(g_in), 1 if grad_input is not None else 0,
-                *[hr.ptr(g) for g in g_om + g_wb], *geom, hr.ptr(ws), ws.numel(), hr.stream()), who)
+                *[hr.ptr(g) for g in g_om + g_wb], *geom, hr.ptr(ws), ws.numel(), hr.stream())
+    hr.check(rc, who)
     return [g_in] + g_om + g_wb
 
 
 def dcn_v2_forward(input, weight, bias, offset, mask, kernel_h, kernel_w, stride_h, stride_w,
                    pad_h, pad_w, dilation_h, dilation_w, deformable_group, _want_columns=False, _act_slope=-1.0,
-                   _pack_token=0, _pack_version=None, _stats_box=None):
+                   _pack_token=0, _pack_version=None, _stats_box=None, _columns_quads=False):
     hr.require_gpu(input, weight, bias, offset, mask)
     input, weight, bias, offset, mask = [hr.f32c(t) for t in (input, weight, bias, offset, mask)]
     B, C, H, W, Co = _shapes(input, weight, offset, mask, kernel_h, kernel_w, deformable_group)
@@ -83,14 +87,14 @@
                            % (tuple(offset.shape), tuple(mask.shape), Ho, Wo))
     geom = (B, C, H, W, Co, kernel_h, kernel_w, stride_h, stride_w, pad_h, pad_w,
             dilation_h, dilation_w, deformable_group)
-    out, cols = _forward('dcn_v2_forward', input, weight, bias, offset, mask, None, geom, Ho, Wo, _want_columns, _act_slope,
-                         _pack_token, _pack_version, _stats_box)
-    return (out, cols) if _want_columns else out
+    out, cols, layout = _forward('dcn_v2_forward', input, weight, bias, offset, mask, None, geom, Ho, Wo, _want_columns,
+                                 _act_slope, _pack_token, _pack_version, _stats_box, _columns_quads)
+    return (out, cols, layout) if _want_columns else out
 
 
 def dcn_v2_backward(input, weight, bias, offset, mask, grad_output, kernel_h, kernel_w, stride_h, stride_w,
                     pad_h, pad_w, dilation_h, dilation_w, deformable_group, _columns=None, _grad_weight=None,
-                    _grad_bias=None, _grad_input=None):
+                    _grad_bias=None, _grad_input=None, _columns_layout=0):
     hr.require_gpu(input, weight, bias, offset, mask, grad_output)
     input, weight, bias, offset, mask, grad_output = [
         hr.f32c(t) for t in (input, weight, bias, offset, mask, grad_output)]
@@ -98,11 +102,12 @@
     geom = (B, C, H, W, Co, kernel_h, kernel_w, stride_h, stride_w, pad_h, pad_w,
             dilation_h, dilation_w, deformable_group)
     return _backward('dcn_v2_backward', input, weight, bias, offset, mask, None, grad_output, geom, _columns, _grad_weight,
-                     _grad_bias, _grad_input)
+                     _grad_bias, _grad_input, _columns_layout)
 
 
 def dcn_v2_forward_om(input, weight, bias, om, kernel_h, kernel_w, stride_h, stride_w, pad_h, pad_w, dilation_h, dilation_w,
-                      _want_columns=False, _pack_token=0, _stats_box=None, _act_slope=-1.0, _pack_version=None):
+                      _want_columns=False, _pack_token=0, _stats_box=None, _act_slope=-1.0, _pack_version=None,
+                      _columns_quads=True):
     hr.require_gpu(input, weight, bias, om)
     input, weight, bias, om = [hr.f32c(t) for t in (input, weight, bias, om)]
     B, C, H, W = input.shape
@@ -116,17 +121,18 @@
         raise RuntimeError("dcn_v2_forward_om: om %s does not match [%d, %d, %d, %d]" % (tuple(om.shape), B, 3 * T, Ho, Wo))
     geom = (B, C, H, W, Co, kernel_h, kernel_w, stride_h, stride_w, pad_h, pad_w, dilation_h, dilation_w, 1)
     return _forward('dcn_v2_forward_om', input, weight, bias, None, None, om, geom, Ho, Wo, _want_columns, _act_slope,
-                    _pack_token, _pack_version, _stats_box)
+                    _pack_token, _pack_version, _stats_box, _columns_quads)
 
 
 def dcn_v2_backward_om(input, weight, bias, om, grad_output, kernel_h, kernel_w, stride_h, stride_w, pad_h, pad_w,
-                       dilation_h, dilation_w, _columns=None, _grad_weight=None, _grad_bias=None, _grad_input=None):
+                       dilation_h, dilation_w, _columns=None, _grad_weight=None, _grad_bias=None, _grad_input=None,
+                       _columns_layout=0):
     hr.require_gpu(input, weight, bias, om, grad_output)
     input, weight, bias, om, grad_output = [hr.f32c(t) for t in (input, weight, bias, om, grad_output)]
     B, C, H, W = input.shape
     geom = (B, C, H, W, weight.shape[0], kernel_h, kernel_w, stride_h, stride_w, pad_h, pad_w, dilation_h, dilation_w, 1)
     return _backward('dcn_v2_backward_om', input, weight, bias, None, None, om, grad_output, geom, _columns, _grad_weight,
-                     _grad_bias, _grad_input)
+                     _grad_bias, _grad_input, _columns_layout)
 
 
 def _psroi_geom(input, rois, offset, no_trans, spatial_scale, output_dim, group_size, pooled_size, part_size,
diff --git a/centernet-uda_amd/csrc/dcn.hip b/centernet-uda_amd/csrc/dcn.hip
--- a/centernet-uda_amd/csrc/dcn.hip
+++ b/centernet-uda_amd/csrc/dcn.hip
@@ -1,6 +1,7 @@
 #include <algorithm>
 #include "igemm.cuh"
 #include "igemm_host.h"
+#include "dcn_colmap.h"
 
 namespace cnuda {
 namespace {
@@ -82,6 +83,7 @@
     float* col;
     float* stats;
     int stats_mp;
+    int col_quads = 0;
 };
 
 template <bool BUF>
@@ -368,8 +370,10 @@
     f32x4 ra[ig_a_per<BM>()];
     const IgABuf<BM> abuf(A, Mp, Kp, 0, tid);
     const int nchunk = Kp / IG_KC, G = g.C >> 4;
-    const bool col_on = p.col != nullptr;
-    float* const col_l = col_on ? p.col + (size_t)b * 9 * g.C * HW + (size_t)kl * HW + pp : nullptr;
+    const bool col_on = p.col != nullptr, colq = col_on && p.col_quads != 0;
+    float* const col_l = !col_on ? nullptr
+                         : colq  ? p.col + (size_t)b * 9 * g.C * HW + (size_t)(4 * dcn_col_quad_of(kl)) * HW + 4 * pp
+                                 : p.col + (size_t)b * 9 * g.C * HW + (size_t)kl * HW + pp;
 
     win_load(0);
     abuf.load(0, ra);
@@ -416,8 +420,17 @@
                     v[h * (IG_KC / 4) + s] = fmaf(w11, cr[s][3], x);
                 }
                 if (col_on) {
-#pragma unroll
-                    for (int s = 0; s < IG_KC / 4; ++s) cp[(size_t)(2 * (h * (IG_KC / 4) + s)) * HW] = v[h * (IG_KC / 4) + s];
+                    if (colq) {
+                        static_assert(IG_KC / 4 == 4, "a blend_half is one quad");
+                        float q[4];
+#pragma unroll
+                        for (int s = 0; s < 4; ++s) { q[s] = v[4 * h + s]; asm("" : "+v"(q[s])); }
+                        const f32x4 q4 = {q[0], q[1], q[2], q[3]};
+                        *reinterpret_cast<f32x4*>(cp + (size_t)(4 * dcn_col_quad_of(8 * h)) * HW) = q4;
+                    } else {
+#pragma unroll
+                        for (int s = 0; s < IG_KC / 4; ++s) cp[(size_t)(2 * (h * (IG_KC / 4) + s)) * HW] = v[h * (IG_KC / 4) + s];
+                    }
                 }
             };
             auto mma_half = [&](int h) {
@@ -476,8 +489,16 @@
                     }
                     if (col_on) {
                         float* cp = col_l + (size_t)(t * g.C + grp * 16) * HW;
-#pragma unroll
-                        for (int s = 0; s < IG_KC / 2; ++s) cp[(size_t)(2 * s) * HW] = sv[s];
+                        if (colq) {
+#pragma unroll
+                            for (int h = 0; h < 2; ++h) {
+                                const f32x4 q4 = {sv[4 * h], sv[4 * h + 1], sv[4 * h + 2], sv[4 * h + 3]};
+                                *reinterpret_cast<f32x4*>(cp + (size_t)(4 * dcn_col_quad_of(8 * h)) * HW) = q4;
+                            }
+                        } else {
+#pragma unroll
+                            for (int s = 0; s < IG_KC / 2; ++s) cp[(size_t)(2 * s) * HW] = sv[s];
+                        }
                     }
                 }
                 const float* ag = A + (size_t)((c0 + t) * IG_KC + kl) * Mp + (lane & 31);
@@ -1133,13 +1154,33 @@
 struct DcnColWParams {
     DcnGeom g;
     const float *col, *gout;
-};
-struct DcnColWLoader {
+    int col_quads = 0;
+};
+struct DcnColQuadRows {
+    __device__ static __forceinline__ int b_quad_row_base(int sub) { return dcn_col_quad_row(sub, 0); }
+    __device__ static constexpr int b_quad_row_imm(int m, int e) { return dcn_col_quad_row(8 * m, e); }
+};
+struct DcnColWLoader : DcnColQuadRows {
     using Params = DcnColWParams;
     const Params& p;
     IgPixelCursor c;
     __device__ DcnColWLoader(const Params& pp, long long n, long long n_end) : p(pp) {
         c.init(n, n_end, p.g.Ho * p.g.Wo, p.g.Wo);
+    }
+    __device__ __forceinline__ bool b_quads() const { return p.col_quads != 0; }
+    template <int NQ>
+    __device__ __forceinline__ void load_bq(int j0, int sub, float (&v)[4 * NQ]) {
+        const DcnGeom& g = p.g;
+        const int HoWo = g.Ho * g.Wo, K = g.kh * g.kw * g.C;
+        const float* base = p.col + (size_t)c.b_ * K * HoWo + (size_t)4 * c.pp_;
+#pragma unroll
+        for (int m = 0; m < NQ; ++m) {
+            const int k = j0 + 4 * (sub + 8 * m);
+            f32x4 q = {0.0f, 0.0f, 0.0f, 0.0f};
+            if (c.valid_ && k < K) q = *reinterpret_cast<const f32x4*>(base + (size_t)k * HoWo);
+#pragma unroll
+            for (int e = 0; e < 4; ++e) v[4 * m + e] = q[e];
+        }
     }
     __device__ __forceinline__ void advance() { c.advance(p.g.Ho * p.g.Wo, p.g.Wo); }
     template <int NV, int STEP>
@@ -1166,7 +1207,7 @@
     }
 };
 
-struct DcnColWBufLoader {
+struct DcnColWBufLoader : DcnColQuadRows {
     using Params = DcnColWParams;
     const Params& p;
     buf_rsrc rg, rc;
@@ -1196,6 +1237,11 @@
     template <int NV, int STEP>
     __device__ __forceinline__ void load_b(int j0, int jsub, float (&v)[NV]) {
         ig_buf_rows<NV, STEP>(rc, c, cimg, p.g.Ho * p.g.Wo, j0, jsub, v);
+    }
+    __device__ __forceinline__ bool b_quads() const { return p.col_quads != 0; }
+    template <int NQ>
+    __device__ __forceinline__ void load_bq(int j0, int sub, float (&v)[4 * NQ]) {
+        ig_buf_quads<NQ>(rc, c, cimg, p.g.Ho * p.g.Wo, j0, sub, v);
     }
 };
 
@@ -1294,6 +1340,8 @@
 int g_scatter_margin = 0;
 int g_walk_tc = 0;
 int g_offset_regime = 0;
+int g_columns_layout = CNUDA_DCN_COLS_ROWS;
+int g_col_quads_policy = !(getenv("CNUDA_DCN_COL_QUADS") && getenv("CNUDA_DCN_COL_QUADS")[0] == '0');
 
 
 int dcnw_tile_cols(int W) { return W % 32 == 0 ? 32 : 16; }
@@ -1451,6 +1499,32 @@
     const int prev = g_offset_regime;
     g_offset_regime = regime & 3;
     return prev;
+}
+extern "C" int cnuda_dcn_set_columns_layout(int layout) {
+    const int prev = g_columns_layout;
+    g_columns_layout = layout == CNUDA_DCN_COLS_QUADS ? CNUDA_DCN_COLS_QUADS : CNUDA_DCN_COLS_ROWS;
+    return prev;
+}
+extern "C" int cnuda_dcn_set_col_quads_policy(int on) {
+    const int prev = g_col_quads_policy;
+    g_col_quads_policy = on != 0;
+    return prev;
+}
+extern "C" int cnuda_dcn_v2_columns_layout(int B, int C, int H, int W, int Cout, int kh, int kw, int sh, int sw, int ph, int pw,
+                                           int dh, int dw, int dg) {
+    DcnGeom g;
+    if (fill_geom(g, B, C, H, W, Cout, kh, kw, sh, sw, ph, pw, dh, dw, dg, "cnuda_dcn_v2_columns_layout")) return CNUDA_DCN_COLS_ROWS;
+    DcnPlan q = make_plan(g);
+    if (q.fwd == DcnFwdPath::Composed) {
+        g.C /= g.dg; g.dg = 1;
+        q = make_plan(g);
+    }
+    return g_col_quads_policy && q.fwd == DcnFwdPath::Window ? CNUDA_DCN_COLS_QUADS : CNUDA_DCN_COLS_ROWS;
+}
+extern "C" int cnuda_dcn_column_row(int C, int storage_row) {
+    if (C <= 0 || C % 16 != 0 || storage_row < 0 || storage_row >= 9 * C) return -1;
+    const int tap = storage_row / C, within = storage_row - tap * C;
+    return tap * C + dcn_col_quad_row(within >> 2, within & 3);
 }
 
 namespace cnuda {
@@ -1577,11 +1651,15 @@
     CNUDA_REQUIRE(q.N < (1ll << 31) - IG_BN, "cnuda_dcn_v2_forward: more than 2^31 pixels per call");
     CNUDA_REQUIRE(c.workspace && c.workspace_bytes >= q.fwd_bytes, "cnuda_dcn_v2_forward: workspace too small");
     Carver cv(c.workspace, c.workspace_bytes);
+    const bool col_quads = c.columns && g_columns_layout == CNUDA_DCN_COLS_QUADS;
+    CNUDA_REQUIRE(!col_quads || q.fwd == DcnFwdPath::Window,
+                  "cnuda_dcn_v2_forward: the columns were asked for in quads (cnuda_dcn_set_columns_layout), this call's kernel "
+                  "writes rows (did the offset regime change after cnuda_dcn_v2_columns_layout?)");
     if (q.fwd == DcnFwdPath::Window) {
         const int bm = 64;
         const float* Aw = launch_pack(c.weight, cv.take<float>((size_t)q.Kp * bm), (size_t)q.Kp * bm * sizeof(float), g.Co, g.C,
                                       q.T, PACK_HALO_FWD, q.Kp, bm, 0, st);
-        DcnFwdParams p{g, c.input, c.offset, c.mask, c.bias, c.act_slope, c.output, c.columns, c.stats, 64};
+        DcnFwdParams p{g, c.input, c.offset, c.mask, c.bias, c.act_slope, c.output, c.columns, c.stats, 64, col_quads};
         ProfScope prof(st);
         prof.name("dcnw_fwd_kernel<%d>%s", bm, c.columns ? " (+ column side output)" : "");
         const int tiles_x = g.W / dcnw_tile_cols(g.W), n_tiles = (int)(q.N / IG_BN);
@@ -1750,7 +1828,9 @@
             "cnuda_dcn_v2_backward(weight)", "cnuda_dcn_v2_backward(weight reduce)", [&](ProfScope& wscope, float* slabs, float* bsl) -> int {
                 bool found;
                 if (c.columns) {
-                    DcnColWParams p{g, c.columns, c.grad_output};
+                    const bool col_quads = g_columns_layout == CNUDA_DCN_COLS_QUADS;
+                    CNUDA_REQUIRE(!col_quads || g.C % 16 == 0, "cnuda_dcn_v2_backward: columns in quads need C %% 16 == 0");
+                    DcnColWParams p{g, c.columns, c.grad_output, col_quads};
                     wscope.name(q.colw_ws ? "igemm_wgrad_ws_kernel<%s, 64, %d>" : "igemm_wgrad_kernel<%s, 64, %d>",
                                 q.colw_buf ? "DcnColWBufLoader" : "DcnColWLoader", q.wg.bj);
                     found = q.colw_ws    ? launch_wgrad<DcnColWBufLoader, true, Tile<64, 64>, Tile<64, 128>>(q.wg, p, slabs, bsl, st)
diff --git a/centernet-uda_amd/csrc/dcn_colmap.h b/centernet-uda_amd/csrc/dcn_colmap.h
--- /dev/null
+++ b/centernet-uda_amd/csrc/dcn_colmap.h
@@ -0,0 +1,29 @@
+#pragma once
+
+namespace cnuda {
+
+__host__ __device__ constexpr int dcn_col_quad_row(int q, int e) {
+    return 16 * (q >> 2) + 8 * ((q >> 1) & 1) + (q & 1) + 2 * e;
+}
+__host__ __device__ constexpr int dcn_col_quad_of(int c) {
+    return 4 * (c >> 4) + 2 * ((c >> 3) & 1) + (c & 1);
+}
+
+constexpr bool dcn_col_quad_map_ok() {
+    for (int g = 0; g < 3; ++g)
+        for (int h = 0; h < 2; ++h)
+            for (int kl = 0; kl < 2; ++kl)
+                for (int e = 0; e < 4; ++e) {
+                    const int c = 16 * g + kl + 2 * (4 * h + e), q = 4 * g + 2 * h + kl;
+                    if (dcn_col_quad_row(q, e) != c || dcn_col_quad_of(c) != q) return false;
+                    if (dcn_col_quad_of(16 * g) + dcn_col_quad_of(8 * h) + dcn_col_quad_of(kl) != q) return false;
+                }
+    for (int sub = 0; sub < 8; ++sub)
+        for (int m = 0; m < 4; ++m)
+            for (int e = 0; e < 4; ++e)
+                if (dcn_col_quad_row(sub + 8 * m, e) != dcn_col_quad_row(sub, 0) + dcn_col_quad_row(8 * m, e)) return false;
+    return true;
+}
+static_assert(dcn_col_quad_map_ok(), "dcn_col_quad_row: the lanes of dcnw_fwd_kernel / the stager's row map");
+
+}
diff --git a/centernet-uda_amd/csrc/igemm.cuh b/centernet-uda_amd/csrc/igemm.cuh
--- a/centernet-uda_amd/csrc/igemm.cuh
+++ b/centernet-uda_amd/csrc/igemm.cuh
@@ -752,6 +752,18 @@
     for (int i = 0; i < NV; ++i) v[i] = ig_buf_load(rs, voff, (unsigned)((row0 + STEP * i) * HoWo) * (unsigned)sizeof(float));
 }
 
+template <int NQ>
+__device__ __forceinline__ void ig_buf_quads(buf_rsrc rs, const IgPixelCursor& c, unsigned image_base, int HoWo, int row0,
+                                             int sub, float (&v)[4 * NQ]) {
+    const unsigned voff = c.valid_ ? image_base + (unsigned)ig_mad24(4 * sub, HoWo, 4 * c.pp_) * 4u : IG_BUF_OOB;
+#pragma unroll
+    for (int m = 0; m < NQ; ++m) {
+        const f32x4 q = ig_buf_load4(rs, voff, (unsigned)((row0 + 32 * m) * HoWo) * (unsigned)sizeof(float));
+#pragma unroll
+        for (int e = 0; e < 4; ++e) v[4 * m + e] = q[e];
+    }
+}
+
 template <int NG, int STEP>
 __device__ __forceinline__ void ig_wgrad_store_bias(float (&bs)[NG], float* __restrict__ dst, int pl, int sub) {
     static_assert(WG_BP == 32, "a row group's pixel lanes are one half of a wave");
@@ -773,9 +785,13 @@
     static_assert((BM / 32 / TM) * WJ == 4, "four waves tile the block");
 };
 
+template <class L, class = void> struct IgHasQuadRows : std::false_type {};
+template <class L> struct IgHasQuadRows<L, std::void_t<decltype(std::declval<const L&>().b_quads())>> : std::true_type {};
+
 template <class WLoader, int BM, int BJ>
 struct IgWgradStager {
     using W = IgWgradTile<BM, BJ>;
+    static_assert(W::NB % 4 == 0 && W::STEP == 8, "quad rows: thread `sub` takes quads sub + 8 m of the column tile");
     const int pl, sub, m0, j0;
     WLoader ld;
     const bool do_bias;
@@ -788,14 +804,30 @@
     }
     __device__ __forceinline__ void load() {
         ld.template load_g<W::NG, W::STEP>(m0, sub, rg);
+        if constexpr (IgHasQuadRows<WLoader>::value) {
+            if (ld.b_quads()) { ld.template load_bq<W::NB / 4>(j0, sub, rb); return; }
+        }
         ld.template load_b<W::NB, W::STEP>(j0, sub, rb);
     }
     __device__ __forceinline__ void advance_load() { ld.advance(); load(); }
     __device__ __forceinline__ void store(float* Gs, float* Bs) {
 #pragma unroll
         for (int i = 0; i < W::NG; ++i) Gs[pl * W::GLD + sub + W::STEP * i] = rg[i];
-#pragma unroll
-        for (int i = 0; i < W::NB; ++i) Bs[pl * W::BLD + sub + W::STEP * i] = rb[i];
+        bool plain = true;
+        if constexpr (IgHasQuadRows<WLoader>::value) {
+            if (ld.b_quads()) {
+                float* bq = Bs + pl * W::BLD + WLoader::b_quad_row_base(sub);
+#pragma unroll
+                for (int m = 0; m < W::NB / 4; ++m)
+#pragma unroll
+                    for (int e = 0; e < 4; ++e) bq[WLoader::b_quad_row_imm(m, e)] = rb[4 * m + e];
+                plain = false;
+            }
+        }
+        if (plain) {
+#pragma unroll
+            for (int i = 0; i < W::NB; ++i) Bs[pl * W::BLD + sub + W::STEP * i] = rb[i];
+        }
         if (do_bias) {
 #pragma unroll
             for (int i = 0; i < W::NG; ++i) bs[i] += rg[i];
diff --git a/centernet-uda_amd/hip_runtime/__init__.py b/centernet-uda_amd/hip_runtime/__init__.py
--- a/centernet-uda_amd/hip_runtime/__init__.py
+++ b/centernet-uda_amd/hip_runtime/__init__.py
@@ -63,6 +63,10 @@
     cnuda_dcn_v2_forward_act = (_I, [_P] * 7 + [_F] + [_I] * 14 + _WS)
     cnuda_dcn_v2_forward_stats = (_I, [_P] * 8 + [_I] * 16 + _WS)
     cnuda_dcn_v2_stats_block = (_I, [_I] * 14 + [_P])
+    cnuda_dcn_set_columns_layout = (_I, [_I])
+    cnuda_dcn_v2_columns_layout = (_I, [_I] * 14)
+    cnuda_dcn_set_col_quads_policy = (_I, [_I])
+    cnuda_dcn_column_row = (_I, [_I, _I])
     cnuda_dcn_v2_forward_om = (_I, [_P] * 7 + [_I] * 2 + [_F] + [_I] * 14 + _WS)
     cnuda_dcn_v2_backward_om = (_I, [_P] * 7 + [_I] + [_P] * 3 + [_I] * 14 + _WS)
     cnuda_dcn_v2_backward_cols = (_I, [_P] * 12 + [_I] * 14 + _WS)
@@ -532,6 +536,30 @@
         lib().cnuda_dcn_set_fused_min_tiles(self.prev)
 
 
+class dcn_col_quads:
+
+    def __init__(self, on):
+        self.on = int(bool(on))
+
+    def __enter__(self):
+        self.prev = lib().cnuda_dcn_set_col_quads_policy(self.on)
+
+    def __exit__(self, *exc):
+        lib().cnuda_dcn_set_col_quads_policy(self.prev)
+
+
+class dcn_columns_layout:
+
+    def __init__(self, layout):
+        self.layout = int(layout)
+
+    def __enter__(self):
+        self.prev = lib().cnuda_dcn_set_columns_layout(self.layout)
+
+    def __exit__(self, *exc):
+        lib().cnuda_dcn_set_columns_layout(self.prev)
+
+
 class splitk:
 
     def __init__(self, max_tiles):
diff --git a/centernet-uda_amd/libs/DCNv2/dcn_v2.py b/centernet-uda_amd/libs/DCNv2/dcn_v2.py
--- a/centernet-uda_amd/libs/DCNv2/dcn_v2.py
+++ b/centernet-uda_amd/libs/DCNv2/dcn_v2.py
@@ -27,7 +27,7 @@
     keep = keep and any(ctx.needs_input_grad[:3 + len(sampling)]) and _KEEP_COLUMNS
     with _offset_regime(ctx.regime):
         out = fwd(input, weight, bias, *sampling, *geom, _want_columns=keep, _pack_token=pack_token, _stats_box=stats_box)
-    out, cols = out if isinstance(out, tuple) else (out, None)
+    out, cols, ctx.cols_layout = out if isinstance(out, tuple) else (out, None, 0)
     ctx.save_for_backward(input, *sampling, weight, bias, cols)
     return out
 
@@ -38,7 +38,7 @@
     acc = accumulate_in_place(ctx.slot)
     with _offset_regime(ctx.regime):
         g_in, *g_sampling, g_w, g_b = bwd(input, weight, bias, *sampling, grad_output, *ctx.geom, _columns=cols,
-                                          _grad_weight=sw, _grad_bias=sb, _grad_input=acc)
+                                          _columns_layout=ctx.cols_layout, _grad_weight=sw, _grad_bias=sb, _grad_input=acc)
     if acc is None:
         claim(ctx.slot, g_in)
     return g_in, g_sampling, (None if sw is not None else g_w), (None if sb is not None else g_b)
diff --git a/include/centernet_uda_hip.h b/include/centernet_uda_hip.h
--- a/include/centernet_uda_hip.h
+++ b/include/centernet_uda_hip.h
@@ -119,6 +119,14 @@
                               int B, int C, int H, int W, int Cout, int kh, int kw,
                               int sh, int sw, int ph, int pw, int dh, int dw, int dg,
                               void* workspace, size_t workspace_bytes, cnuda_stream_t stream);
+
+#define CNUDA_DCN_COLS_ROWS 0
+#define CNUDA_DCN_COLS_QUADS 1
+int cnuda_dcn_set_columns_layout(int layout);
+int cnuda_dcn_v2_columns_layout(int B, int C, int H, int W, int Cout, int kh, int kw, int sh, int sw, int ph, int pw, int dh,
+                                int dw, int dg);
+int cnuda_dcn_set_col_quads_policy(int on);
+int cnuda_dcn_column_row(int C, int storage_row);
 
 size_t cnuda_dcn_v2_psroi_pooling_workspace_bytes(int B, int num_rois, int output_dim, int pooled_size);
 int cnuda_dcn_v2_psroi_pooling_forward(const float* input, const float* rois, const float* trans,
```

Result: no change. 220.3 images/sec, median of 2 (+0.2%).
